# MarcKloter/bulletproofs_gadgets

Hardware: AMD Instinct MI355X
Metric: R1CS constraints/sec (prove), 2^20-constraint MiMC-Merkle, 1/2/4/8 GPU (higher is better)
Workload: dtype u32

## Files before the change

bulletproofs_gadgets_amd/csrc/engine.hip:

```cpp
#include <hip/hip_runtime.h>
#include <algorithm>
#include <array>
#include <chrono>
#include <cerrno>
#include <cstdio>
#include <cstdlib>
#include <cstring>
#include <atomic>
#include <condition_variable>
#include <deque>
#include <functional>
#include <map>
#include <memory>
#include <mutex>
#include <thread>
#include <sched.h>
#include <fcntl.h>
#include <sys/stat.h>
#include <unistd.h>
#include "engine.hpp"
#include "host/fe51.hpp"
#include "host/chain.hpp"
#include "hip/kernels.cuh"

// ... 6 lines not shown
#define BPG_LAUNCH_LDS(I, id, kernel, grid, block, lds, ...) do { (I).prof_begin(id); hipLaunchKernelGGL(kernel, grid, block, lds, (I).st, __VA_ARGS__); (I).prof_end(id); } while (0)

namespace {

struct DevBuf {
    void *p = nullptr; size_t cap = 0;
    void ensure(size_t bytes) {
        if (bytes <= cap) return;
        if (p) HIPCHK(hipFree(p));
        p = nullptr; cap = 0;
        HIPCHK(hipMalloc(&p, bytes)); cap = bytes;
    }
    void release() { if (p) { (void)hipFree(p); p = nullptr; cap = 0; } }
    template <class T> T *as() const { return reinterpret_cast<T *>(p); }
};
struct PinBuf {
    void *p = nullptr; size_t cap = 0;
    void ensure(size_t bytes) {
        if (bytes <= cap) return;
        if (p) HIPCHK(hipHostFree(p));
        p = nullptr; cap = 0;
        HIPCHK(hipHostMalloc(&p, bytes, hipHostMallocDefault)); cap = bytes;
    }
    void release() { if (p) { (void)hipHostFree(p); p = nullptr; cap = 0; } }
    template <class T> T *as() const { return reinterpret_cast<T *>(p); }
};

static std::mutex g_table_bytes_mutex;
static std::map<int, uint64_t> g_table_bytes;
static uint64_t table_bytes_held(int device) { std::lock_guard<std::mutex> lk(g_table_bytes_mutex); return g_table_bytes[device]; }
static void table_bytes_add(int device, int64_t delta) { std::lock_guard<std::mutex> lk(g_table_bytes_mutex); g_table_bytes[device] = (uint64_t)((int64_t)g_table_bytes[device] + delta); }
static std::atomic<int> g_proving[64];
struct ProvingGuard {
    std::atomic<int> &c;
    explicit ProvingGuard(int device) : c(g_proving[(unsigned)device & 63u]) { c.fetch_add(1, std::memory_order_relaxed); }
    ~ProvingGuard() { c.fetch_sub(1, std::memory_order_relaxed); }
};
static bool device_shared(int device) { return g_proving[(unsigned)device & 63u].load(std::memory_order_relaxed) > 1; }
struct SharedTables {
    int device = 0; uint64_t cap = 0;
    DevBuf gens;
    std::mutex m;
    std::map<uint32_t, DevBuf> wide;
    std::map<uint32_t, DevBuf> odd;
    std::map<uint64_t, uint64_t> refused;
    ~SharedTables() {
        (void)hipSetDevice(device); gens.release();
        uint64_t held = 0;
        for (auto &kv : odd) { held += kv.second.cap; kv.second.release(); }
        for (auto &kv : wide) { held += kv.second.cap; kv.second.release(); }
        table_bytes_add(device, -(int64_t)held);
    }
};
static std::mutex g_tables_mutex;
static std::map<std::pair<int, uint64_t>, std::weak_ptr<SharedTables>> g_tables;

inline uint32_t cdiv(uint64_t a, uint64_t b) { return (uint32_t)((a + b - 1) / b); }
inline double now_ms() { return std::chrono::duration<double, std::milli>(std::chrono::steady_clock::now().time_since_epoch()).count(); }

const Scalar &R1_plain() { static Scalar r = [] { Scalar s; s.w[0] = 0xd6ec31748d98951dULL; s.w[1] = 0xc6ef5bf4737dcf70ULL; s.w[2] = 0xfffffffffffffffeULL; s.w[3] = 0x0fffffffffffffffULL; return s; }(); return r; }
const Scalar &Rinv_plain() { static Scalar r = R1_plain().invert(); return r; }
scm to_scm(const Scalar &s) { Scalar m = s * R1_plain(); scm o; std::memcpy(o.v, m.w, 32); return o; }
Scalar from_scm(const scm &m) { Scalar s; std::memcpy(s.w, m.v, 32); return s * Rinv_plain(); }

int32_t naf256(const Scalar &s, int8_t d[256]) {
    uint64_t k[5] = {s.w[0], s.w[1], s.w[2], s.w[3], 0};
    std::memset(d, 0, 256);
    int32_t top = -1;
    for (int i = 0; i < 256; i++) {
        if ((k[0] | k[1] | k[2] | k[3] | k[4]) == 0) break;
        if (k[0] & 1) {
            int dig = 2 - (int)(k[0] & 3);
            d[i] = (int8_t)dig; top = i;
            if (dig == 1) k[0] -= 1;
            else { for (int j = 0; j < 5; j++) { if (++k[j] != 0) break; } }
        }
        for (int j = 0; j < 4; j++) k[j] = (k[j] >> 1) | (k[j + 1] << 63);
        k[4] >>= 1;
    }
    return top;
}

int32_t wnaf256(const Scalar &s, uint32_t w, int8_t d[256]) {
    uint64_t k[5] = {s.w[0], s.w[1], s.w[2], s.w[3], 0};
    std::memset(d, 0, 256);
    int32_t top = -1;
    const int64_t full = 1ll << w, half = 1ll << (w - 1);
    for (int i = 0; i < 256; i++) {
        if ((k[0] | k[1] | k[2] | k[3] | k[4]) == 0) break;
        if (k[0] & 1) {
            int64_t dig = (int64_t)(k[0] & (uint64_t)(full - 1));
            if (dig >= half) dig -= full;
            d[i] = (int8_t)dig; top = i;
            if (dig > 0) { k[0] -= (uint64_t)dig; }
            else { uint64_t add = (uint64_t)(-dig); for (int j = 0; j < 5; j++) { uint64_t t = k[j] + add; add = t < add ? 1 : 0; k[j] = t; if (!add) break; } }
        }
        for (int j = 0; j < 4; j++) k[j] = (k[j] >> 1) | (k[j + 1] << 63);
        k[4] >>= 1;
    }
    return top;
}

Scalar scalar_bits(const Scalar &s, uint32_t from, uint32_t count) {
    Scalar r = Scalar::zero();
    for (uint32_t k = 0; k < count && from + k < 256; k++) {
        const uint32_t b = from + k;
        if ((s.w[b >> 6] >> (b & 63)) & 1ull) r.w[k >> 6] |= 1ull << (k & 63);
    }
    return r;
}

uint32_t ceil_log2(uint64_t x) { uint32_t l = 0; while ((1ULL << l) < x) l++; return l; }

struct GensCacheHeader { char magic[8]; uint64_t version, capacity, bytes, checksum; };
static const char kGensMagic[8] = {'B', 'P', 'G', 'G', 'E', 'N', 'S', '1'};
uint64_t gens_checksum(const uint8_t *p, size_t n) {
    uint64_t h[4] = {0x9e3779b97f4a7c15ull, 0xc2b2ae3d27d4eb4full, 0x165667b19e3779f9ull, 0x27d4eb2f165667c5ull};
    size_t i = 0;
    for (; i + 32 <= n; i += 32) for (int k = 0; k < 4; k++) { uint64_t w; std::memcpy(&w, p + i + 8 * k, 8); h[k] = (h[k] ^ w) * 0x100000001b3ull; h[k] = (h[k] << 29) | (h[k] >> 35); }
    for (; i < n; i++) h[0] = (h[0] ^ p[i]) * 0x100000001b3ull;
    return h[0] ^ (h[1] * 3) ^ (h[2] * 5) ^ (h[3] * 7) ^ (uint64_t)n;
}
bool gens_cache_trusted(const std::string &dir, const std::string &file) {
    struct stat st;
    if (::stat(dir.c_str(), &st) != 0 || !S_ISDIR(st.st_mode) || st.st_uid != ::geteuid() || (st.st_mode & (S_IWGRP | S_IWOTH))) return false;
    if (::lstat(file.c_str(), &st) != 0) return true;
    return S_ISREG(st.st_mode) && st.st_uid == ::geteuid() && !(st.st_mode & (S_IWGRP | S_IWOTH));
}
std::string gens_cache_path(const std::string &dir, uint64_t cap) {
    if (dir.empty()) return std::string();
    return dir + "/gens_" + std::to_string(cap) + ".bpg";
}

}

struct DeviceCircuit {
    uint64_t n = 0, m = 0, q = 0, ncols = 0, nnz = 0;
    bool has_witness = false;
    uint64_t const_begin = 0;
    DevBuf aL, aR, aO, col_ptr, ent_row, ent_coef, coef;
    struct MergeSet { uint32_t groups = 0, skipped = 0; DevBuf skipA, skipB, sc, pts; };
    bool merge_tried = false;
    MergeSet mI, mO;
    bool is_template = false;
    DevBuf wit_stream, wit_segs, wit_v;
    std::vector<uint32_t> wit_level_ptr;
    uint64_t n_params = 0, param_first = 0;
};

#define BPG_KERNELS(X) X(k_gens_derive) X(k_normalize_niels) X(k_compress_niels) X(k_pedersen) X(k_sc_from_bytes) \
    X(k_sc_from_wide) X(k_blind_poison) X(k_exp_table) X(k_reduce_partials) X(k_flatten) X(k_flatten_const) X(k_poly_t) X(k_poly_eval) X(k_ipa_prep) \
    X(k_ipa_fold_scalars) X(k_fold_points) X(k_fold_points_reg) X(k_fold_points_split) X(k_fold_points_wnaf) X(k_fold_points_quad) X(k_fold_points_quadw) X(k_fold_points_regw) X(k_odd_start) X(k_odd_start_ext) X(k_dbl_times) X(k_odd_step) X(k_msm_digits) X(k_msm_scatter1) X(k_msm_sort2) X(k_scan_blocksums) \
    X(k_scan_apply) X(k_bucket_chunks) X(k_bucket_combine) X(k_bucket_combine_heavy) X(k_bucket_reduce) X(k_window_sums) X(k_window_sums_quad) X(k_decompress) X(k_ipa_s) X(k_verify_scalars) X(k_verify_scalars_acc) X(k_bench_fe_mul) \
    X(k_tt_bases) X(k_tt_multiples) X(k_tt_bases8) X(k_tt_multiples8) X(k_tt_round8) X(k_tt_factors) X(k_tt_advance) X(k_tt_round) X(k_tt_finish) X(k_blind_expand) X(k_tt_commit3) X(k_tt_commit3_finish) X(k_csc_count) X(k_csc_fill) X(k_csc_colptr) X(k_merge_insert) X(k_merge_plan) X(k_merge_groups) X(k_merge_members) X(k_merge_sum) \
    X(k_bt_commit3) X(k_bt_commit3_finish) X(k_bt_compress) X(k_bt_exp) X(k_bt_poly_t) X(k_bt_poly_eval) X(k_bt_factors) X(k_bt_advance) X(k_bt_round) \
    X(k_bt_finish) X(k_bt_fold_scalars) X(k_witness_eval)
enum KernelId {
#define X(n) KID_##n,
    BPG_KERNELS(X)
#undef X
    KID_COUNT
};
static const char *const kKernelNames[KID_COUNT] = {
#define X(n) #n,
    BPG_KERNELS(X)
#undef X
};

struct Engine::Impl {
    hipStream_t st = nullptr;
    int prof_mode = 0;
    struct ProfRec { int id; hipEvent_t a, b; };
    std::vector<ProfRec> prof_open;
    std::vector<hipEvent_t> prof_pool;
    double prof_ms[KID_COUNT] = {0};
    std::vector<float> prof_wit_ms;
    uint64_t prof_count[KID_COUNT] = {0};
    double prof_alg_bytes[KID_COUNT] = {0}, prof_act_bytes[KID_COUNT] = {0}, prof_fm[KID_COUNT] = {0};
    bool prof_on(int id) const { return prof_mode == 2 || (prof_mode == 1 && (id == KID_k_fold_points || id == KID_k_fold_points_reg || id == KID_k_fold_points_split || id == KID_k_fold_points_wnaf || id == KID_k_fold_points_quad || id == KID_k_fold_points_quadw || id == KID_k_fold_points_regw || id == KID_k_bucket_chunks)); }
    hipEvent_t prof_event() { if (!prof_pool.empty()) { hipEvent_t e = prof_pool.back(); prof_pool.pop_back(); return e; } hipEvent_t e; HIPCHK(hipEventCreate(&e)); return e; }
    void prof_begin(int id) { if (!prof_on(id)) return; ProfRec r{id, prof_event(), prof_event()}; HIPCHK(hipEventRecord(r.a, st)); prof_open.push_back(r); }
    void prof_end(int id) { if (!prof_on(id)) return; HIPCHK(hipEventRecord(prof_open.back().b, st)); }
    void prof_note(int id, double alg_bytes, double act_bytes, double fm) { if (!prof_on(id)) return; prof_alg_bytes[id] += alg_bytes; prof_act_bytes[id] += act_bytes; prof_fm[id] += fm; }
    void prof_collect() {
        if (prof_open.empty()) return;
        HIPCHK(hipStreamSynchronize(st));
        for (ProfRec &r : prof_open) { float ms = 0; HIPCHK(hipEventElapsedTime(&ms, r.a, r.b)); prof_ms[r.id] += ms; prof_count[r.id]++; if (r.id == KID_k_witness_eval && prof_wit_ms.size() < 1024) prof_wit_ms.push_back(ms); prof_pool.push_back(r.a); prof_pool.push_back(r.b); }
        prof_open.clear();
    }
    void prof_reset() { prof_collect(); for (int i = 0; i < KID_COUNT; i++) { prof_ms[i] = 0; prof_count[i] = 0; prof_alg_bytes[i] = prof_act_bytes[i] = prof_fm[i] = 0; } prof_wit_ms.clear(); }
    std::shared_ptr<SharedTables> shared;
    DevBuf gens;
    DevBuf bases, scratch_ext, comp, small_in, small_sc;
    DevBuf arena;
    uint8_t *arena_at(size_t off) const { return arena.as<uint8_t>() + off; }
    bool blocking_waits = false;
    void wait_stream() {
        if (blocking_waits && !shared_now) {
            const double until = now_ms() + 3.0;
            do {
                const hipError_t e = hipStreamQuery(st);
                if (e == hipSuccess) return;
                if (e != hipErrorNotReady) HIPCHK(e);
                for (int k = 0; k < 64; k++) __builtin_ia32_pause();
            } while (now_ms() < until);
        }
        HIPCHK(hipStreamSynchronize(st));
    }
    static size_t al256(size_t x) { return (x + 255) & ~(size_t)255; }
    DevBuf counts, starts, cursor, blocksum, buckets, partial, msm_result, open_keys, medium, wsums, wq_stage, wq_tickets, tile_hist, heavy, plain, starts1;
    uint32_t sweep_blocks_resident = 1024;
    uint32_t msm_cmax = 15;
    uint32_t msm_cmax_shared = 16;
    uint32_t rseg = 8;
    uint32_t lgch = 0;
    bool gens_share = true;
    uint32_t profile = 1;
    bool shared_now = false;
    uint32_t msm_cmin = 2;
    uint32_t wit_waves = 1024;
    uint32_t merge_equal = 1;
    uint32_t merged_last = 0, merged_skipped_last = 0;
    uint32_t msm_skipped_terms = 0;
    uint32_t msm_alg_discount = 0;
    void merge_witness(DeviceCircuit *c, const ge_niels *Gtab, const ge_niels *Htab);
    void merge_build(DeviceCircuit::MergeSet &M, const scm *A, const ge_niels *PA, uint32_t nA, const scm *B, const ge_niels *PB, uint32_t nB);
    double merge_ms_last = 0;
    DevBuf sLR, yinvpow, lv, rv, red_partial, red_out, raw_rng, extras;
    DevBuf stale_flag;
    DevBuf ipa_s, ipa_tabA, ipa_tabB, naf, qsteps, vfy_in, vfy_pts, vfy_ok, vfy_sc, vfy_ch;
    DevBuf vfy_small;
    DevBuf tt_bases, tt_table, tt_f, tt_c, tt_partial, grp_c, ped_table, s_parts;
    uint32_t tt_orig_M0 = 0; const void *tt_orig_gens = nullptr;
    ge_pniels *tt_table_p = nullptr;
    void tt_build(const ge_niels *G, const ge_niels *H, const ge_niels *B, uint32_t M0, bool original) {
        const uint32_t npts = 2 * M0 + 1;
        if (original && tt_orig_M0 == M0 && tt_orig_gens == gens.p) { tt_table_p = tt_table.as<ge_pniels>(); return; }
        const size_t bb = al256((size_t)npts * TT_WINDOWS * sizeof(ge_ext)), tb = (size_t)npts * TT_WINDOWS * TT_MULTS * sizeof(ge_pniels);
        ge_ext *basesp;
        if (original) {
            tt_orig_M0 = 0;
            tt_bases.ensure(bb); tt_table.ensure(tb);
            basesp = tt_bases.as<ge_ext>(); tt_table_p = tt_table.as<ge_pniels>();
        } else {
            arena.ensure(bb + tb);
            basesp = reinterpret_cast<ge_ext *>(arena_at(0)); tt_table_p = reinterpret_cast<ge_pniels *>(arena_at(bb));
        }
        tt_partial.ensure((size_t)3 * cdiv((uint64_t)M0 * 16, 256) * sizeof(ge_ext));
        BPG_LAUNCH((*this), k_tt_bases, dim3(cdiv(npts, 64)), dim3(256), G, H, B, basesp, M0);
        BPG_LAUNCH((*this), k_tt_multiples, dim3(cdiv((uint64_t)npts * TT_WINDOWS, 256)), dim3(256), basesp, tt_table_p, npts * TT_WINDOWS);
        if (original) { tt_orig_M0 = M0; tt_orig_gens = gens.p; }
    }
    uint64_t table_budget = 4ull << 30;
    uint64_t tt_wide_budget = 0;
    std::string gens_cache_dir;
    bool table_reserve(uint64_t key, uint64_t bytes) const {
        std::lock_guard<std::mutex> lk(g_table_bytes_mutex);
        uint64_t &held = g_table_bytes[shared->device];
        auto it = shared->refused.find(key);
        if (it != shared->refused.end() && held >= it->second) return false;
        if (held + bytes > table_budget) return false;
        held += bytes;
        return true;
    }
    const ge_pniels *wide_ensure(uint32_t M0) {
        const uint64_t bytes = (uint64_t)2 * M0 * TT8_WINDOWS * TT8_MULTS * sizeof(ge_pniels);
        if (M0 < 64 || bytes > tt_wide_budget) return nullptr;
        std::lock_guard<std::mutex> lk(shared->m);
        auto it = shared->wide.find(M0);
        if (it != shared->wide.end()) return it->second.as<ge_pniels>();
        const uint64_t key = (1ull << 32) | M0;
        if (!table_reserve(key, bytes)) return nullptr;
        DevBuf table, bases8;
        try { table.ensure(bytes); bases8.ensure((size_t)2 * M0 * TT8_WINDOWS * sizeof(ge_ext)); }
        catch (const std::exception &) {
            (void)hipGetLastError(); table.release(); bases8.release();
            table_bytes_add(shared->device, -(int64_t)bytes); shared->refused[key] = table_bytes_held(shared->device); return nullptr;
        }
        try {
            BPG_LAUNCH((*this), k_tt_bases8, dim3(cdiv(2 * M0, 64)), dim3(256), gens.as<ge_niels>(), gens.as<ge_niels>() + gens_cap, bases8.as<ge_ext>(), M0);
            BPG_LAUNCH((*this), k_tt_multiples8, dim3(cdiv((uint64_t)2 * M0 * TT8_WINDOWS, 256)), dim3(256), bases8.as<ge_ext>(), table.as<ge_pniels>(), 2 * M0 * TT8_WINDOWS);
            HIPCHK(hipGetLastError());
            HIPCHK(hipStreamSynchronize(st));
        } catch (...) {
            (void)hipStreamSynchronize(st); bases8.release(); table.release(); table_bytes_add(shared->device, -(int64_t)bytes);
            throw;
        }
        bases8.release();
        shared->wide[M0] = table;
        return table.as<ge_pniels>();
    }
    PinBuf h_naf, h_qsteps;
    DevBuf gens_odd;
    uint32_t fold_wnaf = 5;
    uint32_t fold_parts = 2;
    uint64_t fold_table_budget = 64ull << 30;
    uint32_t eff_wnaf = 0, eff_parts = 0;
    uint32_t fold_part_bits() const { return (254 + eff_parts - 1) / eff_parts; }
    bool odd_ensure() {
        eff_wnaf = fold_wnaf; eff_parts = fold_parts;
        auto table_bytes = [&](uint32_t w, uint32_t parts) { return ((uint64_t)parts * (1u << (w - 2)) - 1) * 2 * gens_cap * sizeof(ge_niels); };
        auto smaller = [&]() { if (eff_parts > 1) { eff_parts /= 2; return true; } if (eff_wnaf > 3) { eff_wnaf--; return true; } return false; };
        std::lock_guard<std::mutex> lk(shared->m);
        DevBuf odd;
        for (;;) {
            const uint32_t key = eff_wnaf | (eff_parts << 8);
            auto it = shared->odd.find(key);
            if (it != shared->odd.end()) { gens_odd = it->second; return true; }
            const uint64_t bytes = table_bytes(eff_wnaf, eff_parts);
            if (bytes <= fold_table_budget && table_reserve(key, bytes)) {
                try { odd.ensure(bytes); break; }
                catch (const std::exception &) { (void)hipGetLastError(); odd.release(); table_bytes_add(shared->device, -(int64_t)bytes); shared->refused[key] = table_bytes_held(shared->device); }
            }
            if (!smaller()) { gens_odd = DevBuf(); return false; }
        }
        const uint32_t key_built = eff_wnaf | (eff_parts << 8);
        const uint32_t NM = 1u << (eff_wnaf - 2), cnt = (uint32_t)(2 * gens_cap), L = fold_part_bits();
        DevBuf dbl, base;
        try {
        scratch_ext.ensure((size_t)cnt * sizeof(ge_ext));
        dbl.ensure((size_t)cnt * sizeof(ge_ext));
        if (eff_parts > 1) base.ensure((size_t)cnt * sizeof(ge_ext));
        const dim3 grid(cdiv(cnt, 256)), ngrid(cdiv(cdiv(cnt, NORM_K), 256));
        for (uint32_t part = 0; part < eff_parts; part++) {
            ge_niels *tab0 = odd.as<ge_niels>() + ((ptrdiff_t)part * NM - 1) * (ptrdiff_t)cnt;
            if (part == 0) BPG_LAUNCH((*this), k_odd_start, grid, dim3(256), gens.as<ge_niels>(), scratch_ext.as<ge_ext>(), dbl.as<ge_ext>(), cnt);
            else {
                BPG_LAUNCH((*this), k_dbl_times, grid, dim3(256), gens.as<ge_niels>(), base.as<ge_ext>(), cnt, L, part == 1 ? 1u : 0u);
                BPG_LAUNCH((*this), k_normalize_niels, ngrid, dim3(256), base.as<ge_ext>(), tab0, cnt);
                BPG_LAUNCH((*this), k_odd_start_ext, grid, dim3(256), base.as<ge_ext>(), scratch_ext.as<ge_ext>(), dbl.as<ge_ext>(), cnt);
            }
            for (uint32_t m = 1; m < NM; m++) {
                if (m > 1) BPG_LAUNCH((*this), k_odd_step, grid, dim3(256), scratch_ext.as<ge_ext>(), dbl.as<ge_ext>(), cnt);
                BPG_LAUNCH((*this), k_normalize_niels, ngrid, dim3(256), scratch_ext.as<ge_ext>(), tab0 + (size_t)m * cnt, cnt);
            }
        }
        HIPCHK(hipGetLastError());
        HIPCHK(hipStreamSynchronize(st));
        } catch (...) {
            (void)hipStreamSynchronize(st); dbl.release(); base.release();
            const uint64_t held = odd.cap; odd.release(); table_bytes_add(shared->device, -(int64_t)held);
            throw;
        }
        dbl.release(); base.release();
        shared->odd[key_built] = odd;
        gens_odd = odd;
        return true;
    }
    uint32_t fold_split_max = 65536;
    uint32_t fold_adapt = 1;
    bool shared_variants() const { return fold_adapt == 2 || (fold_adapt == 1 && device_shared(shared->device)); }
    bool fold_quad = true;
    bool fold_quad_w = true;
    bool fold_reg_w = true;
    bool window_quad = true;
    uint32_t window_quad_blocks = 288;
    uint32_t fold_group = 3;
    uint32_t tt_lg = 12;
    uint32_t tt_orig_lg = 14;
    uint32_t batch_wave_mb = 512;
    DevBuf bt_dev; PinBuf bt_pin;
    PinBuf h_raw, h_small;
    using BlindStream = bpg::BlindStream;
    using ChainWorker = bpg::ChainWorker;
    std::shared_ptr<ChainWorker> chain;
    uint32_t pool_streams = 0;
    uint32_t chain_workers = 1;
    uint32_t chain_lanes = 1;
    std::deque<std::shared_ptr<BlindStream>> blinds;
    std::vector<std::shared_ptr<BlindStream>> slab_owner;
    std::vector<PinBuf> h_blind;
    struct SlabDev { DevBuf d; hipStream_t copy_st = nullptr; std::vector<hipEvent_t> ev; };
    std::vector<std::unique_ptr<SlabDev>> slab_dev;
    int last_chain_cpu = -1;
    int test_fail_upload = 0;
    static void blind_stop(const std::shared_ptr<BlindStream> &b) {
        b->stop.store(true, std::memory_order_relaxed);
    }
    void blind_retire(const std::shared_ptr<BlindStream> &b) {
        blind_stop(b);
        if (chain) {
            std::unique_lock<std::mutex> lk(chain->mu);
            for (auto it = chain->pending.begin(); it != chain->pending.end(); ++it) if (it->get() == b.get()) { chain->pending.erase(it); b->finished.store(true); break; }
        }
        while (!b->finished.load(std::memory_order_acquire)) std::this_thread::yield();
        const int c = b->cpu.load(std::memory_order_relaxed); if (c >= 0) last_chain_cpu = c;
    }
    void blind_cancel() {
        while (!blinds.empty()) { blind_retire(blinds.front()); blinds.pop_front(); }
    }
    void chain_shutdown() {
        blind_cancel();
        if (!chain) return;
        if (!chain->pool) chain->stop();
        chain.reset(); pool_streams = 0;
    }
    uint64_t gens_cap = 0;
    bool gens_load_cached(const std::string &path, uint64_t cap, DevBuf &out);
    void adopt(const std::shared_ptr<SharedTables> &sp) { shared = sp; gens = sp->gens; gens_cap = sp->cap; gens_odd = DevBuf(); }
    void gens_store_cached(const std::string &path, uint64_t cap);

// ... 5 lines not shown
        MsmPlan P;
        uint32_t nkeys = 0, CH = 0, nchunks = 0, live = 0;
        bool shared = false, per_bucket = false, quad = false;
        uint32_t window_blocks = 0, window_threads = 0;
    } msm_last;
    DevBuf test_skip;
    std::vector<h51::pt> msm_points(const MsmTicket &t) const {
        std::vector<h51::pt> out(t.nmsm);
        const uint32_t *w = reinterpret_cast<const uint32_t *>(h_wsums.as<uint8_t>() + (size_t)t.slot * WS_SLOT_BYTES);
        for (uint32_t m = 0; m < t.nmsm; m++) out[m] = h51::pt_horner(w + (size_t)m * t.W * 32, t.W);
        return out;
    }
    PinBuf stage; hipEvent_t stage_ev[2] = {nullptr, nullptr};
    void h2d(void *dst, const void *src, size_t bytes) {
        const size_t SLOT = 8u << 20;
        stage.ensure(2 * SLOT);
        for (int k = 0; k < 2; k++) if (!stage_ev[k]) HIPCHK(hipEventCreateWithFlags(&stage_ev[k], hipEventDisableTiming));
        const uint8_t *s8 = static_cast<const uint8_t *>(src); uint8_t *d8 = static_cast<uint8_t *>(dst);
        int slot = 0;
        for (size_t off = 0; off < bytes; off += SLOT, slot ^= 1) {
            const size_t len = std::min(SLOT, bytes - off);
            HIPCHK(hipEventSynchronize(stage_ev[slot]));
            std::memcpy(stage.as<uint8_t>() + (size_t)slot * SLOT, s8 + off, len);
            HIPCHK(hipMemcpyAsync(d8 + off, stage.as<uint8_t>() + (size_t)slot * SLOT, len, hipMemcpyHostToDevice, st));
            HIPCHK(hipEventRecord(stage_ev[slot], st));
        }
    }
    void inner_product(Transcript &T, std::vector<uint8_t> &proof, uint64_t n, uint64_t N, const Scalar &yinv, const Scalar &u_ch, const Scalar &w,
                       const ge_niels *Gtab, const ge_niels *Htab, const ge_niels *Bn, ProveTimings *tm, double &t0);
};

namespace {
bool env_present(const char *name) { const char *e = std::getenv(name); return e && *e; }
long env_int_strict(const char *name, long lo, long hi) {
    const char *e = std::getenv(name);
    char *end = nullptr; errno = 0;
    const long v = std::strtol(e, &end, 10);
    if (errno || end == e || *end != '\0' || v < lo || v > hi)
        throw std::invalid_argument(std::string(name) + "=" + e + ": expected an integer in [" + std::to_string(lo) + ", " + std::to_string(hi) + "]");
    return v;
}
double env_double_strict(const char *name, double lo, double hi) {
    const char *e = std::getenv(name);
    char *end = nullptr; errno = 0;
    const double v = std::strtod(e, &end);
    if (errno || end == e || *end != '\0' || !(v >= lo) || !(v <= hi))
        throw std::invalid_argument(std::string(name) + "=" + e + ": expected a number in [" + std::to_string(lo) + ", " + std::to_string(hi) + "]");
    return v;
}
template <class T> void env_set(const char *name, long lo, long hi, T &out) { if (env_present(name)) out = (T)env_int_strict(name, lo, hi); }
}

Engine::Engine(int device, const EngineConfig &cfg) : device_(device) {
    if (cfg.profile > 2) throw std::invalid_argument("bpg_config.profile: 0 (default), 1 (one-shot) or 2 (serving)");
    if (cfg.table_budget_gb < 0 || cfg.table_budget_gb > 4096) throw std::invalid_argument("bpg_config.table_budget_gb: 0 (default) .. 4096");
    if (cfg.chain_workers > 64) throw std::invalid_argument("bpg_config.chain_workers: 0 (default), 1..64");
    if (cfg.chain_lanes > 8) throw std::invalid_argument("bpg_config.chain_lanes: 0 (default), 1..8");
    if (cfg.blocking_sync < -1 || cfg.blocking_sync > 2) throw std::invalid_argument("bpg_config.blocking_sync: -1 (environment, else spin), 0 (spin), 1 (blocking)");
    std::unique_ptr<Impl> K(new Impl());
    int blocking = cfg.blocking_sync == 2 ? 0 : cfg.blocking_sync;
    if (blocking < 0 && env_present("BPG_SYNC_BLOCKING")) blocking = env_int_strict("BPG_SYNC_BLOCKING", 0, 1) ? 1 : 0;
    uint32_t profile = cfg.profile;
    if (profile == 0) { if (const char *e = std::getenv("BPG_PROFILE")) profile = (!std::strcmp(e, "serving") || !std::strcmp(e, "2")) ? 2u : 1u; else profile = 1u; }
    if (profile == 2) { K->fold_wnaf = 8; K->fold_parts = 4; K->tt_wide_budget = 24ull << 30; K->table_budget = 96ull << 30; }
    else { K->fold_wnaf = 5; K->fold_parts = 2; K->tt_wide_budget = 0; K->table_budget = 4ull << 30; }
    K->profile = profile;
    {
        double gb = cfg.table_budget_gb;
        if (!(gb > 0) && env_present("BPG_TABLE_GB")) gb = env_double_strict("BPG_TABLE_GB", 0.0, 4096.0);
        if (gb > 0) K->table_budget = (uint64_t)(gb * (double)(1ull << 30));
    }
    K->chain_workers = cfg.chain_workers ? cfg.chain_workers : 1u; if (!cfg.chain_workers) env_set("BPG_CHAIN_WORKERS", 1, 64, K->chain_workers);
    K->chain_lanes = cfg.chain_lanes ? cfg.chain_lanes : 1u; if (!cfg.chain_lanes) env_set("BPG_CHAIN_LANES", 1, 8, K->chain_lanes);
    K->gens_cache_dir = cfg.gens_cache_dir;
    if (K->gens_cache_dir.empty()) { if (const char *e = std::getenv("BPG_GENS_CACHE_DIR")) K->gens_cache_dir = e; }
    if (env_present("BPG_MSM_CMAX")) K->msm_cmax = K->msm_cmax_shared = (uint32_t)env_int_strict("BPG_MSM_CMAX", 4, 16);
    env_set("BPG_MSM_CMIN", 2, 16, K->msm_cmin);
    env_set("BPG_MERGE", 0, 2, K->merge_equal);
    bool resident_set = false;
    if (env_present("BPG_SWEEP_RESIDENT")) { K->sweep_blocks_resident = (uint32_t)env_int_strict("BPG_SWEEP_RESIDENT", 64, 65536); resident_set = true; }
    if (env_present("BPG_RSEG")) {
        const long v = env_int_strict("BPG_RSEG", 1, 1024);
        if (v & (v - 1)) throw std::invalid_argument("BPG_RSEG: the segment length of the bucket reduction is a power of two in [1, 1024]");
        K->rseg = (uint32_t)v;
    }
    env_set("BPG_LGCH", 2, 10, K->lgch);
    env_set("BPG_FOLD_SPLIT", 0, 1 << 24, K->fold_split_max);
    if (env_present("BPG_FOLD_QUAD")) K->fold_quad = env_int_strict("BPG_FOLD_QUAD", 0, 1) != 0;
    if (env_present("BPG_FOLD_QUAD_W")) K->fold_quad_w = env_int_strict("BPG_FOLD_QUAD_W", 0, 1) != 0;
    if (env_present("BPG_FOLD_REG_W")) K->fold_reg_w = env_int_strict("BPG_FOLD_REG_W", 0, 1) != 0;
    if (env_present("BPG_WINDOW_QUAD")) K->window_quad = env_int_strict("BPG_WINDOW_QUAD", 0, 1) != 0;
    env_set("BPG_WINDOW_QUAD_BLOCKS", 1, 65536, K->window_quad_blocks);
    env_set("BPG_FOLD_ADAPT", 0, 2, K->fold_adapt);
    env_set("BPG_FOLD_GROUP", 1, 5, K->fold_group);
    if (env_present("BPG_TT_WIDE_GB")) K->tt_wide_budget = (uint64_t)(env_double_strict("BPG_TT_WIDE_GB", 0.0, 4096.0) * (double)(1ull << 30));
    if (env_present("BPG_FOLD_TABLE_GB")) K->fold_table_budget = (uint64_t)(env_double_strict("BPG_FOLD_TABLE_GB", 0.0, 4096.0) * (double)(1ull << 30));
    if (env_present("BPG_FOLD_PARTS")) { const long v = env_int_strict("BPG_FOLD_PARTS", 1, 8); if (v & (v - 1)) throw std::invalid_argument("BPG_FOLD_PARTS: 1, 2, 4 or 8"); K->fold_parts = (uint32_t)v; }
    if (env_present("BPG_FOLD_WNAF")) { const long v = env_int_strict("BPG_FOLD_WNAF", 0, 8); if (v == 1 || v == 2) throw std::invalid_argument("BPG_FOLD_WNAF: 0 (register kernels) or 3..8"); K->fold_wnaf = (uint32_t)v; }
    if (env_present("BPG_TT_LG")) K->tt_lg = K->tt_orig_lg = (uint32_t)env_int_strict("BPG_TT_LG", 0, 20);
    env_set("BPG_TT_ORIG_LG", 0, 20, K->tt_orig_lg);
    env_set("BPG_BATCH_WAVE_MB", 0, 1 << 20, K->batch_wave_mb);
    if (env_present("BPG_GENS_SHARE")) K->gens_share = env_int_strict("BPG_GENS_SHARE", 0, 1) != 0;

    int count = 0;
    hipError_t e = hipGetDeviceCount(&count);
    if (e != hipSuccess || count <= 0) throw DeviceError("no HIP device available: the bpg engine has no CPU path");
    if (device < 0 || device >= count) throw DeviceError("invalid device ordinal");
    HIPCHK(hipSetDevice(device));
    if (blocking == 1) { (void)hipSetDeviceFlags(hipDeviceScheduleBlockingSync); (void)hipGetLastError(); K->blocking_waits = true; }
    {
        int cus = 0;
        if (hipDeviceGetAttribute(&cus, hipDeviceAttributeMultiprocessorCount, device) == hipSuccess && cus > 0) {
            if (!resident_set) K->sweep_blocks_resident = (uint32_t)cus * 4u;
            K->wit_waves = (uint32_t)cus * 4u;
            if (!env_present("BPG_WINDOW_QUAD_BLOCKS")) K->window_quad_blocks = (uint32_t)cus + (uint32_t)cus / 8u;
        }
    }
    impl_ = K.release();
    try { init_device(); }
    catch (...) { if (impl_->st) (void)hipStreamDestroy(impl_->st); delete impl_; impl_ = nullptr; throw; }
}

void Engine::init_device() {
    HIPCHK(hipStreamCreate(&impl_->st));
    stream_ = impl_->st;
    static const uint8_t Bc[32] = {0xe2, 0xf2, 0xae, 0x0a, 0x6a, 0xbc, 0x4e, 0x71, 0xa8, 0x84, 0xa9, 0x61, 0xc5, 0x00, 0x51, 0x5f,
                                   0x58, 0xe3, 0x0b, 0x6a, 0xa5, 0x82, 0xdd, 0x8d, 0xb6, 0xa6, 0x59, 0x45, 0xe0, 0x8d, 0x2d, 0x76};
    uint8_t h[64]; sha3_512_host(h, Bc, 32);
    impl_->small_in.ensure(4096); impl_->bases.ensure(3 * sizeof(ge_niels));
    impl_->stale_flag.ensure(64); HIPCHK(hipMemsetAsync(impl_->stale_flag.p, 0, 64, impl_->st));
    HIPCHK(hipMemcpyAsync(impl_->small_in.p, h, 64, hipMemcpyHostToDevice, impl_->st));
    hipLaunchKernelGGL(k_init_bases, dim3(1), dim3(64), 0, impl_->st, impl_->small_in.as<uint32_t>(), impl_->bases.as<ge_niels>());
    HIPCHK(hipGetLastError());
    impl_->tt_bases.ensure((size_t)3 * TT_WINDOWS * sizeof(ge_ext));
    impl_->ped_table.ensure((size_t)3 * TT_WINDOWS * TT_MULTS * sizeof(ge_pniels));
    hipLaunchKernelGGL(k_tt_bases, dim3(1), dim3(256), 0, impl_->st, impl_->bases.as<ge_niels>(), impl_->bases.as<ge_niels>() + 1, impl_->bases.as<ge_niels>(),
                       impl_->tt_bases.as<ge_ext>(), 1u);
    hipLaunchKernelGGL(k_tt_multiples, dim3(cdiv(3 * TT_WINDOWS, 256)), dim3(256), 0, impl_->st, impl_->tt_bases.as<ge_ext>(), impl_->ped_table.as<ge_pniels>(),
                       (uint32_t)(3 * TT_WINDOWS));
    HIPCHK(hipGetLastError());
    HIPCHK(hipStreamSynchronize(impl_->st));
}

Engine::~Engine() {
    if (!impl_) return;
    impl_->chain_shutdown();
    (void)hipSetDevice(device_);
    (void)hipStreamSynchronize(impl_->st);
    for (auto &sd : impl_->slab_dev) if (sd->copy_st) (void)hipStreamSynchronize(sd->copy_st);
    DevBuf *bufs[] = {&impl_->bases, &impl_->scratch_ext, &impl_->comp, &impl_->small_in, &impl_->small_sc, &impl_->counts,
                      &impl_->starts, &impl_->cursor, &impl_->blocksum, &impl_->arena, &impl_->buckets, &impl_->partial, &impl_->msm_result,
                      &impl_->sLR, &impl_->yinvpow, &impl_->lv, &impl_->rv, &impl_->red_partial,
                      &impl_->red_out, &impl_->raw_rng, &impl_->extras, &impl_->ipa_s, &impl_->ipa_tabA, &impl_->ipa_tabB, &impl_->naf, &impl_->qsteps, &impl_->wsums, &impl_->wq_stage, &impl_->wq_tickets, &impl_->vfy_in, &impl_->vfy_pts, &impl_->vfy_ok, &impl_->vfy_sc, &impl_->vfy_ch, &impl_->vfy_small,
                      &impl_->stale_flag, &impl_->tile_hist, &impl_->heavy, &impl_->plain, &impl_->open_keys, &impl_->medium, &impl_->tt_bases, &impl_->tt_table, &impl_->tt_f, &impl_->tt_c, &impl_->tt_partial, &impl_->grp_c, &impl_->ped_table, &impl_->s_parts, &impl_->starts1};
    for (DevBuf *b : bufs) b->release();
    impl_->shared.reset();
    impl_->h_raw.release(); impl_->h_small.release(); impl_->h_naf.release(); impl_->h_qsteps.release(); impl_->stage.release(); for (PinBuf &b : impl_->h_blind) b.release();
    for (auto &sd : impl_->slab_dev) {
        if (sd->copy_st) { (void)hipStreamSynchronize(sd->copy_st); (void)hipStreamDestroy(sd->copy_st); }
        for (hipEvent_t e : sd->ev) (void)hipEventDestroy(e);
        sd->d.release();
    }
    for (int k = 0; k < 2; k++) if (impl_->stage_ev[k]) (void)hipEventDestroy(impl_->stage_ev[k]);
    (void)hipStreamDestroy(impl_->st);
    delete impl_;
}

int Engine::device_count() { int n = 0; if (hipGetDeviceCount(&n) != hipSuccess) { (void)hipGetLastError(); return 0; } return n; }
void Engine::profile_set(int mode) { HIPCHK(hipSetDevice(device_)); impl_->prof_reset(); impl_->prof_mode = mode; }
std::string Engine::profile_report() {
    HIPCHK(hipSetDevice(device_));
    impl_->prof_collect();
    char sch[896];
    std::snprintf(sch, sizeof sch, "{\"_schedule\": {\"profile\": %u, \"tt_lg\": %u, \"tt_orig_lg\": %u, \"fold_group\": %u, \"fold_wnaf\": %u, \"fold_parts\": %u, "
                  "\"eff_wnaf\": %u, \"eff_parts\": %u, \"fold_adapt\": %u, \"fold_split_max\": %u, \"fold_quad\": %u, \"msm_cmax\": %u, \"msm_cmax_shared\": %u, \"msm_cmin\": %u, "
                  "\"rseg\": %u, \"lgch\": %u, \"sweep_blocks_resident\": %u, \"shared_variants_last\": %u, \"merge_equal\": %u, \"merged_last\": %u, \"merged_skipped_last\": %u, \"merge_ms_last\": %.3f, \"table_budget\": %llu, \"table_bytes\": %llu}",
                  impl_->profile, impl_->tt_lg, impl_->tt_orig_lg, impl_->fold_group, impl_->fold_wnaf, impl_->fold_parts, impl_->eff_wnaf, impl_->eff_parts,
                  impl_->fold_adapt, impl_->fold_split_max, (unsigned)impl_->fold_quad, impl_->msm_cmax, impl_->msm_cmax_shared, impl_->msm_cmin, impl_->rseg, impl_->lgch,
                  impl_->sweep_blocks_resident, (unsigned)impl_->shared_now, (unsigned)impl_->merge_equal, impl_->merged_last, impl_->merged_skipped_last, impl_->merge_ms_last, (unsigned long long)impl_->table_budget, (unsigned long long)table_bytes_held(device_));
    std::string out = sch;
    if (!impl_->prof_wit_ms.empty()) {
        out += ", \"_witness_launch_ms\": [";
        for (size_t i = 0; i < impl_->prof_wit_ms.size(); i++) { char b[32]; std::snprintf(b, sizeof b, "%s%.4f", i ? "," : "", impl_->prof_wit_ms[i]); out += b; }
        out += "]";
    }
    bool first = false;
    for (int i = 0; i < KID_COUNT; i++) {
        if (!impl_->prof_count[i]) continue;
        char buf[512];
        std::snprintf(buf, sizeof buf, "%s\"%s\": {\"count\": %llu, \"total_ms\": %.6f, \"alg_bytes\": %.0f, \"device_bytes\": %.0f, \"field_mults\": %.0f}",
                      first ? "" : ", ", kKernelNames[i], (unsigned long long)impl_->prof_count[i], impl_->prof_ms[i], impl_->prof_alg_bytes[i],
                      impl_->prof_act_bytes[i], impl_->prof_fm[i]);
        out += buf; first = false;
    }
    return out + "}";
}
double Engine::bench_fe_mul(uint32_t iters) {
    HIPCHK(hipSetDevice(device_));
    Impl &I = *impl_;
    const uint32_t blocks = 256 * 16, threads = 256;
    I.small_sc.ensure((size_t)blocks * threads * sizeof(fe));
    hipEvent_t a, b; HIPCHK(hipEventCreate(&a)); HIPCHK(hipEventCreate(&b));
    hipLaunchKernelGGL(k_bench_fe_mul, dim3(blocks), dim3(threads), 0, I.st, I.small_sc.as<fe>(), 8u);
    HIPCHK(hipEventRecord(a, I.st));
    hipLaunchKernelGGL(k_bench_fe_mul, dim3(blocks), dim3(threads), 0, I.st, I.small_sc.as<fe>(), iters);
    HIPCHK(hipEventRecord(b, I.st));
    HIPCHK(hipGetLastError());
    HIPCHK(hipEventSynchronize(b));
    float ms = 0; HIPCHK(hipEventElapsedTime(&ms, a, b));
    (void)hipEventDestroy(a); (void)hipEventDestroy(b);
    return (double)blocks * threads * iters * 4.0 / (ms * 1e-3);
}

void Engine::test_fe_ops(int op, size_t n, const uint8_t *a, const uint8_t *b, uint8_t *out) {
    if (!n) return;
    HIPCHK(hipSetDevice(device_));
    Impl &I = *impl_;
    I.small_sc.ensure(2 * n * 32); I.comp.ensure(n * 32);
    HIPCHK(hipMemcpyAsync(I.small_sc.p, a, n * 32, hipMemcpyHostToDevice, I.st));
    HIPCHK(hipMemcpyAsync(I.small_sc.as<uint8_t>() + n * 32, b, n * 32, hipMemcpyHostToDevice, I.st));
    hipLaunchKernelGGL(k_test_fe, dim3(cdiv(n, 64)), dim3(64), 0, I.st, I.small_sc.as<uint32_t>(), I.small_sc.as<uint32_t>() + 8 * n, I.comp.as<uint8_t>(), (uint32_t)n, (uint32_t)op);
    HIPCHK(hipGetLastError());
    HIPCHK(hipMemcpyAsync(out, I.comp.p, n * 32, hipMemcpyDeviceToHost, I.st));
    HIPCHK(hipStreamSynchronize(I.st));
}

void Engine::synchronize() { HIPCHK(hipSetDevice(device_)); HIPCHK(hipStreamSynchronize(impl_->st)); }

void Engine::gens_ensure(uint64_t capacity) {
    if (capacity == 0 || (capacity & (capacity - 1))) throw std::invalid_argument("generator capacity must be a power of two");
    if (capacity > (1ULL << 24)) throw std::invalid_argument("generator capacity above 2^24 is not supported");
    if (capacity <= gens_cap_) return;
    HIPCHK(hipSetDevice(device_));
    Impl &I = *impl_;
    const uint64_t cap = capacity;
    std::lock_guard<std::mutex> tables_lock(g_tables_mutex);
    const bool share = I.gens_share;
    if (share) {
        auto it = g_tables.find({device_, cap});
        if (it != g_tables.end()) {
            if (std::shared_ptr<SharedTables> sp = it->second.lock()) { I.adopt(sp); gens_cap_ = cap; return; }
            g_tables.erase(it);
        }
    }
    auto publish = [&](DevBuf fresh) {
        auto sp = std::make_shared<SharedTables>();
        sp->device = device_; sp->cap = cap; sp->gens = fresh;
        if (share) g_tables[{device_, cap}] = sp;
        I.adopt(sp); gens_cap_ = cap;
    };
    const std::string cache_file = gens_cache_path(I.gens_cache_dir, cap);
    const bool cache_ok = !cache_file.empty() && gens_cache_trusted(I.gens_cache_dir, cache_file);
    if (cache_ok) { DevBuf loaded; if (I.gens_load_cached(cache_file, cap, loaded)) { publish(loaded); return; } }
    I.h_raw.ensure(2 * cap * 64);
    {
        struct Chain { Shake256 sh; std::vector<uint8_t> bytes; bool started = false; };
        static Chain chains[2];
        static std::mutex chain_mutex;
        std::lock_guard<std::mutex> lock(chain_mutex);
        auto extend = [&](int which) {
            Chain &c = chains[which];
            if (!c.started) {
                const uint8_t label[5] = {(uint8_t)(which ? 'H' : 'G'), 0, 0, 0, 0};
                c.sh.absorb(reinterpret_cast<const uint8_t *>("GeneratorsChain"), 15);
                c.sh.absorb(label, 5);
                c.started = true;
            }
            const size_t have = c.bytes.size(), want = (size_t)cap * 64;
            if (want > have) { c.bytes.resize(want); c.sh.squeeze(c.bytes.data() + have, want - have); }
        };
        (void)keccak_impl();
        std::thread th([&] { extend(1); });
        extend(0);
        th.join();
        for (int which = 0; which < 2; which++) std::memcpy(I.h_raw.as<uint8_t>() + (size_t)which * cap * 64, chains[which].bytes.data(), (size_t)cap * 64);
    }
    I.raw_rng.ensure(2 * cap * 64);
    I.scratch_ext.ensure(2 * cap * sizeof(ge_ext));
    DevBuf fresh; fresh.ensure(2 * cap * sizeof(ge_niels));
    HIPCHK(hipMemcpyAsync(I.raw_rng.p, I.h_raw.p, 2 * cap * 64, hipMemcpyHostToDevice, I.st));
    const uint32_t cnt = (uint32_t)(2 * cap);
    BPG_LAUNCH(I, k_gens_derive, dim3(cdiv(cnt, 256)), dim3(256), I.raw_rng.as<uint32_t>(), I.scratch_ext.as<ge_ext>(), cnt);
    BPG_LAUNCH(I, k_normalize_niels, dim3(cdiv(cdiv(cnt, NORM_K), 256)), dim3(256), I.scratch_ext.as<ge_ext>(), fresh.as<ge_niels>(), cnt);
    HIPCHK(hipGetLastError());
    HIPCHK(hipStreamSynchronize(I.st));
    publish(fresh);
    I.raw_rng.release(); I.scratch_ext.release(); I.h_raw.release();
    if (cache_ok) I.gens_store_cached(cache_file, cap);
}

bool Engine::Impl::gens_load_cached(const std::string &path, uint64_t cap, DevBuf &out) {
    const int fd = ::open(path.c_str(), O_RDONLY | O_NOFOLLOW | O_CLOEXEC);
    FILE *f = fd >= 0 ? ::fdopen(fd, "rb") : nullptr;
    if (!f) { if (fd >= 0) ::close(fd); return false; }
    const size_t bytes = (size_t)2 * cap * sizeof(ge_niels);
    GensCacheHeader hd;
    bool ok = std::fread(&hd, sizeof hd, 1, f) == 1 && std::memcmp(hd.magic, kGensMagic, 8) == 0 && hd.version == 2 && hd.capacity == cap && hd.bytes == bytes;
    PinBuf host;
    if (ok) { host.ensure(bytes); ok = std::fread(host.p, 1, bytes, f) == bytes && std::fgetc(f) == EOF; }
    std::fclose(f);
    if (ok) ok = gens_checksum(host.as<uint8_t>(), bytes) == hd.checksum;
    if (!ok) { host.release(); return false; }
    DevBuf fresh; fresh.ensure(bytes);
    HIPCHK(hipMemcpyAsync(fresh.p, host.p, bytes, hipMemcpyHostToDevice, st));
    const uint32_t SAMPLE = (uint32_t)std::min<uint64_t>(64, cap);
    uint8_t raw[2 * 64 * 64];
    for (int which = 0; which < 2; which++) {
// ... 409 lines not shown

void Engine::free_circuit(DeviceCircuit *c) {
    if (!c) return;
    (void)hipSetDevice(device_);
    DevBuf *b[] = {&c->wit_stream, &c->wit_segs, &c->wit_v, &c->aL, &c->aR, &c->aO, &c->col_ptr, &c->ent_row, &c->ent_coef, &c->coef, &c->mI.skipA, &c->mI.skipB, &c->mI.sc, &c->mI.pts, &c->mO.skipA, &c->mO.skipB, &c->mO.sc, &c->mO.pts};
    for (DevBuf *x : b) x->release();
    delete c;
}

TemplatePlan Engine::plan_template(const FlatView &c, const WitnessProgramView &p) {
    check_instance(c);
    check_witness_program(c, p);
    TemplatePlan T;
    T.schedule = build_witness_schedule(c.n, c.m, p);
    T.packed = pack_witness_program(c, p, T.schedule);
    T.slotted = with_parameter_slots(c, p);
    T.n_params = p.n_params; T.param_first = c.ncoef;
    return T;
}
void Engine::template_eval_host(const FlatView &c, const WitnessProgramView &p, const uint8_t *v, uint8_t *aL_out, uint8_t *aR_out, uint8_t *aO_out) {
    const TemplatePlan T = plan_template(c, p);
    const PackedWitnessProgram &P = T.packed;
    auto load = [](const uint8_t *b, size_t count) {
        std::vector<scm> out(count ? count : 1);
        for (size_t i = 0; i < count; i++) { uint32_t w[8]; std::memcpy(w, b + 32 * i, 32); out[i] = sc_from_words(w); }
        return out;
    };
    const std::vector<scm> coef = load(c.coef, c.ncoef), vv = load(v, c.m);
    std::vector<scm> aL(c.n), aR(c.n), aO(c.n);
    for (const WitnessSegment &s : P.segs) witness_eval_segment(s.first, s.count, P.stream.data() + s.stream, coef.data(), vv.data(), aL.data(), aR.data(), aO.data());
    for (size_t i = 0; i < c.n; i++) {
        uint32_t w[8];
        sc_to_words(w, aL[i]); std::memcpy(aL_out + 32 * i, w, 32);
        sc_to_words(w, aR[i]); std::memcpy(aR_out + 32 * i, w, 32);
        sc_to_words(w, aO[i]); std::memcpy(aO_out + 32 * i, w, 32);
    }
}

DeviceCircuit *Engine::upload_template(const FlatView &c, const TemplatePlan &T) {
    const PackedWitnessProgram &P = T.packed;
    FlatView f(T.slotted); f.aL = c.aL; f.aR = c.aR; f.aO = c.aO;
    DeviceCircuit *d = upload(f);
    try {
        Impl &I = *impl_;
        d->is_template = true; d->n_params = T.n_params; d->param_first = T.param_first;
        d->wit_level_ptr = T.schedule.level_ptr;
        d->wit_stream.ensure(P.stream.size() * 4); d->wit_segs.ensure(P.segs.size() * sizeof(WitnessSegment)); d->wit_v.ensure((c.m ? c.m : 1) * sizeof(scm));
        I.h2d(d->wit_stream.p, P.stream.data(), P.stream.size() * 4);
        I.h2d(d->wit_segs.p, P.segs.data(), P.segs.size() * sizeof(WitnessSegment));
        HIPCHK(hipStreamSynchronize(I.st));
    } catch (...) { free_circuit(d); throw; }
    return d;
}

void Engine::assign(DeviceCircuit *d, const uint8_t *v, const uint8_t *param_values) {
    HIPCHK(hipSetDevice(device_));
    Impl &I = *impl_;
    if (!d || !d->is_template) throw std::invalid_argument("assign: the circuit is not a template (bpg_r1cs_upload_template)");
    d->has_witness = false;
    d->merge_tried = false; d->mI.groups = d->mI.skipped = 0; d->mO.groups = d->mO.skipped = 0;
    const uint64_t cnt[2] = {d->m, d->n_params};
    const uint8_t *src[2] = {v, param_values};
    scm *dst[2] = {d->wit_v.as<scm>(), d->coef.as<scm>() + d->param_first};
    I.small_sc.ensure((std::max(cnt[0], cnt[1]) + 1) * 32);
    for (int k = 0; k < 2; k++) {
        if (!cnt[k]) continue;
        I.h2d(I.small_sc.p, src[k], cnt[k] * 32);
        BPG_LAUNCH(I, k_sc_from_bytes, dim3(cdiv(cnt[k], 256)), dim3(256), I.small_sc.as<uint32_t>(), dst[k], (uint32_t)cnt[k]);
        HIPCHK(hipGetLastError());
        HIPCHK(hipStreamSynchronize(I.st));
    }
    for (size_t l = 0; l + 1 < d->wit_level_ptr.size(); l++) {
        const uint32_t s0 = d->wit_level_ptr[l], ns = d->wit_level_ptr[l + 1] - s0;
        const uint32_t lanes = std::min(64u, std::max(1u, cdiv(ns, I.wit_waves)));
        BPG_LAUNCH(I, k_witness_eval, dim3(cdiv(ns, lanes)), dim3(lanes), d->wit_segs.as<uint4>() + s0, ns, d->wit_stream.as<uint32_t>(), d->coef.as<scm>(),
                   d->wit_v.as<scm>(), d->aL.as<scm>(), d->aR.as<scm>(), d->aO.as<scm>());
    }
    HIPCHK(hipGetLastError());
    HIPCHK(hipStreamSynchronize(I.st));
    d->has_witness = true;
}
void Engine::Impl::merge_build(DeviceCircuit::MergeSet &M, const scm *A, const ge_niels *PA, uint32_t nA, const scm *B, const ge_niels *PB, uint32_t nB) {
    const uint32_t nterms = nA + nB;
    M.groups = 0; M.skipped = 0;
    if (nterms < 2) return;
    MergeTerms T; T.A = A; T.B = B; T.PA = PA; T.PB = PB; T.nA = nA; T.nterms = nterms;
    const uint32_t lgslots = ceil_log2((uint64_t)2 * nterms), slots = 1u << lgslots;
    const uint32_t nblk = cdiv(slots, SCAN_CHUNK);
    const size_t words = (size_t)7 * slots + 2 * (size_t)nterms + (size_t)nterms / 2 + 8;
    arena.ensure(words * 4); blocksum.ensure((size_t)(nblk + 1) * 4);
    uint32_t *rep = arena.as<uint32_t>(), *count = rep + slots, *msize = count + slots, *gcount = msize + slots, *moff = gcount + slots, *goff = moff + slots + 1,
             *fill = goff + slots + 1, *slot_of = fill + slots, *members = slot_of + nterms, *gslot = members + nterms;
    const uint32_t wA = (nA + 31) / 32, wB = (nB + 31) / 32;
    M.skipA.ensure((size_t)std::max(wA, 1u) * 4); M.skipB.ensure((size_t)std::max(wB, 1u) * 4);
    HIPCHK(hipMemsetAsync(rep, 0xff, (size_t)slots * 4, st));
    HIPCHK(hipMemsetAsync(count, 0, (size_t)slots * 4, st));
    HIPCHK(hipMemsetAsync(M.skipA.p, 0, (size_t)std::max(wA, 1u) * 4, st)); HIPCHK(hipMemsetAsync(M.skipB.p, 0, (size_t)std::max(wB, 1u) * 4, st));
    BPG_LAUNCH((*this), k_merge_insert, dim3(cdiv(nterms, 256)), dim3(256), T, rep, count, slot_of, lgslots);
    BPG_LAUNCH((*this), k_merge_plan, dim3(cdiv(slots, 256)), dim3(256), count, msize, gcount, slots);
    auto scan = [&](uint32_t *in, uint32_t *out) {
        BPG_LAUNCH((*this), k_scan_blocksums, dim3(nblk), dim3(256), in, slots, blocksum.as<uint32_t>());
        BPG_LAUNCH((*this), k_scan_apply, dim3(nblk), dim3(256), in, slots, blocksum.as<uint32_t>(), out, fill);
    };
    scan(msize, moff); scan(gcount, goff);
    HIPCHK(hipGetLastError());
    uint32_t tot[2] = {0, 0};
    HIPCHK(hipMemcpyAsync(&tot[0], moff + slots, 4, hipMemcpyDeviceToHost, st));
    HIPCHK(hipMemcpyAsync(&tot[1], goff + slots, 4, hipMemcpyDeviceToHost, st));
    HIPCHK(hipStreamSynchronize(st));
    const uint32_t skipped = tot[0], groups = tot[1];
    if (groups == 0 || skipped > nterms || groups > nterms / 2) return;
    HIPCHK(hipMemsetAsync(fill, 0, (size_t)slots * 4, st));
    M.sc.ensure((size_t)groups * sizeof(scm)); M.pts.ensure((size_t)groups * sizeof(ge_niels));
    scratch_ext.ensure((size_t)groups * sizeof(ge_ext));
    BPG_LAUNCH((*this), k_merge_groups, dim3(cdiv(slots, 256)), dim3(256), count, goff, gslot, slots);
    BPG_LAUNCH((*this), k_merge_members, dim3(cdiv(nterms, 256)), dim3(256), T, slot_of, count, moff, fill, members, M.skipA.as<uint32_t>(), M.skipB.as<uint32_t>());
    BPG_LAUNCH((*this), k_merge_sum, dim3(cdiv(groups, 64)), dim3(64), T, count, moff, goff, gslot, members, groups, scratch_ext.as<ge_ext>(), M.sc.as<scm>());
    BPG_LAUNCH((*this), k_normalize_niels, dim3(cdiv(cdiv(groups, NORM_K), 256)), dim3(256), scratch_ext.as<ge_ext>(), M.pts.as<ge_niels>(), groups);
    HIPCHK(hipGetLastError());
    if (merge_equal != 2) HIPCHK(hipStreamSynchronize(st));
    M.groups = groups; M.skipped = skipped;
}
void Engine::Impl::merge_witness(DeviceCircuit *c, const ge_niels *Gtab, const ge_niels *Htab) {
    if (c->merge_tried) return;
    c->merge_tried = true;
    const uint32_t n = (uint32_t)c->n;
    if (!merge_equal || n < 2) return;
    const double t0 = now_ms();
    merge_build(c->mI, c->aL.as<scm>(), Gtab, n, c->aR.as<scm>(), Htab, n);
    merge_build(c->mO, c->aO.as<scm>(), Gtab, n, nullptr, nullptr, 0);
    merge_ms_last = now_ms() - t0;
}

void Engine::Impl::inner_product(Transcript &T, std::vector<uint8_t> &proof, uint64_t n, uint64_t N, const Scalar &yinv, const Scalar &u_ch,
                                 const Scalar &w, const ge_niels *Gtab, const ge_niels *Htab, const ge_niels *Bn, ProveTimings *tm, double &t0) {
    Impl &I = *this;
    const uint32_t lgN = ceil_log2(N);
    auto lap = [&](double *slot) { if (tm) { I.wait_stream(); double t1 = now_ms(); *slot += t1 - t0; t0 = t1; } };
    T.innerproduct_domain_sep(N);
    std::vector<Scalar> yinv_pow2(lgN + 1);
    yinv_pow2[0] = yinv; for (uint32_t k = 1; k <= lgN; k++) yinv_pow2[k] = yinv_pow2[k - 1] * yinv_pow2[k - 1];
    scm *a = I.lv.as<scm>(), *b = I.rv.as<scm>();
    if (lgN) {
        const uint64_t half = N / 2;
        I.ipa_s.ensure(4 * half * sizeof(scm));
        I.ipa_tabA.ensure(2 * half * sizeof(ge_niels)); I.ipa_tabB.ensure((half > 1 ? half : 2) * sizeof(ge_niels));
        I.naf.ensure(4096);
    }
    Scalar Gamma = Scalar::one(), Eta = Scalar::one();
    const ge_niels *Gst = Gtab, *Hst = Htab;
    const scm w_m = to_scm(w), uch_m = to_scm(u_ch);
    uint64_t mcur = N;
    const uint32_t quad_sums = I.shared_now ? 0u : 1u;
    bool tt_on = false; uint32_t tt_j = 0, tt_lgM0 = 0, tt_cur = 0; Scalar tt_u, tt_uinv; const ge_pniels *tt_wide = nullptr;
    const uint32_t GRP_STRIDE = 64;
    uint32_t g_j = 0, g_r = 1, g_cur = 0, g_index = 0; uint64_t g_M = N; bool g_first = true; std::vector<Scalar> g_us;
    for (uint32_t round = 0; round < lgN; round++) {
        const uint64_t h = mcur / 2;
        const bool first = round == 0;
        if (!tt_on && ((I.tt_lg > 0 && mcur <= (1ull << I.tt_lg)) || (first && I.tt_orig_lg > 0 && mcur <= (1ull << I.tt_orig_lg)))) {
            tt_on = true; tt_lgM0 = ceil_log2(mcur); tt_j = 0; tt_cur = 0;
            const uint32_t M0 = (uint32_t)mcur;
            I.tt_f.ensure((size_t)2 * M0 * sizeof(scm)); I.tt_c.ensure((size_t)4 * M0 * sizeof(scm));
            I.tt_build(Gst, Hst, Bn, M0, Gst == Gtab && Hst == Htab);
            tt_wide = (Gst == Gtab && Hst == Htab && Gtab == I.gens.as<ge_niels>()) ? I.wide_ensure(M0) : nullptr;
            BPG_LAUNCH(I, k_tt_factors, dim3(cdiv(M0, 256)), dim3(256), I.yinvpow.as<scm>(), uch_m, (uint32_t)first, (uint32_t)n, M0, to_scm(Gamma), to_scm(Eta),
                       I.tt_f.as<scm>(), I.tt_f.as<scm>() + M0, I.tt_c.as<scm>());
        }
        if (tt_on) {
            const uint32_t M0 = 1u << tt_lgM0;
            scm *c0 = I.tt_c.as<scm>() + (size_t)tt_cur * 2 * M0, *c1 = I.tt_c.as<scm>() + (size_t)(tt_cur ^ 1u) * 2 * M0;
            if (tt_j > 0) {
                BPG_LAUNCH(I, k_tt_advance, dim3(cdiv(std::max<uint64_t>(mcur, 1ull << (tt_j - 1)), 256)), dim3(256), a, b, to_scm(tt_u), to_scm(tt_uinv), (uint32_t)mcur,
                           c0, c1, 1u << (tt_j - 1), M0);
                tt_cur ^= 1u; std::swap(c0, c1);
            }
            const uint32_t nblk = cdiv((uint64_t)M0 * 8, 256);
            if (tt_wide) BPG_LAUNCH(I, k_tt_round8, dim3(nblk, 2), dim3(256), tt_wide, a, b, I.tt_f.as<scm>(), I.tt_f.as<scm>() + M0, c0, tt_lgM0, tt_j, I.tt_partial.as<ge_ext>(), quad_sums);
            else BPG_LAUNCH(I, k_tt_round, dim3(nblk, 2), dim3(256), I.tt_table_p, a, b, I.tt_f.as<scm>(), I.tt_f.as<scm>() + M0, c0, tt_lgM0, tt_j,
                       I.tt_partial.as<ge_ext>(), quad_sums);
            BPG_LAUNCH(I, k_tt_finish, dim3(2), dim3(256), I.tt_partial.as<ge_ext>(), nblk, a, b, (uint32_t)h, w_m,
                       I.tt_table_p + (size_t)2 * M0 * TT_WINDOWS * TT_MULTS, I.msm_result.as<ge_ext>(), quad_sums);
            HIPCHK(hipGetLastError());
            uint8_t lr[64];
            uint32_t *hp = reinterpret_cast<uint32_t *>(I.h_small.as<uint8_t>() + 16384);
            HIPCHK(hipMemcpyAsync(hp, I.msm_result.p, 2 * sizeof(ge_ext), hipMemcpyDeviceToHost, st));
            I.wait_stream();
            h51::pt_compress(lr, h51::pt_from_device(hp)); h51::pt_compress(lr + 32, h51::pt_from_device(hp + 32));
            lap(tm ? &tm->ipa_msm : nullptr);
            T.append_point("L", lr); T.append_point("R", lr + 32);
            proof.insert(proof.end(), lr, lr + 64);
            tt_u = T.challenge_scalar("u"); tt_uinv = tt_u.invert();
            tt_j++;
            mcur = h;
            if (round + 1 == lgN) {
                BPG_LAUNCH(I, k_ipa_fold_scalars, dim3(cdiv(h, 256)), dim3(256), a, b, to_scm(tt_u), to_scm(tt_uinv), (uint32_t)h);
                HIPCHK(hipGetLastError());
            }
            continue;
        }
        if (g_j == 0) {
            g_M = mcur; g_first = first;
            uint32_t left = ceil_log2(mcur);
            if (I.tt_lg > 0 && left > I.tt_lg) left -= I.tt_lg;
            g_r = std::min<uint32_t>(I.fold_group, left);
            g_us.clear();
            I.grp_c.ensure(4 * GRP_STRIDE * sizeof(scm));
            g_cur = 0;
            hipLaunchKernelGGL(k_set2, dim3(1), dim3(64), 0, st, I.grp_c.as<scm>(), (uint32_t)GRP_STRIDE, to_scm(Gamma), to_scm(Eta));
        }
        scm *c0 = I.grp_c.as<scm>() + (size_t)g_cur * 2 * GRP_STRIDE;
        const uint64_t cnt = g_M / 2;
        scm *sLG = I.ipa_s.as<scm>(), *sLH = sLG + cnt, *sRG = sLH + cnt, *sRH = sRG + cnt;
        const uint32_t blocks = std::min<uint32_t>(cdiv(cnt, 256), 1024);
        const uint32_t lgh = ceil_log2(h);
        I.red_partial.ensure((size_t)blocks * 2 * sizeof(scm) + 4096);
        BPG_LAUNCH(I, k_ipa_prep, dim3(blocks), dim3(256), a, b, I.yinvpow.as<scm>(), c0, c0 + GRP_STRIDE, uch_m,
                           (uint32_t)g_first, (uint32_t)n, lgh, g_j, sLG, sLH, sRG, sRH, I.red_partial.as<scm>());
        BPG_LAUNCH_ID(I, KID_k_reduce_partials, k_reduce_partials_scaled, dim3(2), dim3(256), I.red_partial.as<scm>(), blocks, 2u, I.extras.as<scm>() + 3, w_m);
        Impl::MsmTicket tk;
        {
            MsmSegs S = seg_new();
            const uint32_t lgblk = g_j ? lgh : 31u;
            seg_push(S, sLG, Gst + h, (uint32_t)cnt, 0, lgblk);
            seg_push(S, sLH, Hst, (uint32_t)cnt, 0, lgblk);
            seg_push(S, I.extras.as<scm>() + 3, Bn, 1, 0);
            seg_push(S, sRG, Gst, (uint32_t)cnt, 1, lgblk);
            seg_push(S, sRH, Hst + h, (uint32_t)cnt, 1, lgblk);
            seg_push(S, I.extras.as<scm>() + 4, Bn, 1, 1);
            tk = I.msm(S, 2);
        }
        uint8_t lr[64];
        I.wait_stream();
        { const std::vector<h51::pt> LR = I.msm_points(tk); h51::pt_compress(lr, LR[0]); h51::pt_compress(lr + 32, LR[1]); }
        lap(tm ? &tm->ipa_msm : nullptr);
        T.append_point("L", lr); T.append_point("R", lr + 32);
        proof.insert(proof.end(), lr, lr + 64);
        const Scalar u = T.challenge_scalar("u"), uinv = u.invert();
        g_us.push_back(u);
        {
            scm *c1 = I.grp_c.as<scm>() + (size_t)(g_cur ^ 1u) * 2 * GRP_STRIDE;
            BPG_LAUNCH(I, k_tt_advance, dim3(cdiv(std::max<uint64_t>(h, 1ull << g_j), 256)), dim3(256), a, b, to_scm(u), to_scm(uinv), (uint32_t)h,
                       c0, c1, 1u << g_j, (uint32_t)GRP_STRIDE);
            g_cur ^= 1u;
        }
        g_j++;
        if (g_j == g_r) {
            const uint32_t Mr = (uint32_t)(g_M >> g_r), nterms = (1u << g_r) - 1u;
            std::vector<Scalar> fG(g_r), fH(g_r);
            for (uint32_t k = 1; k <= g_r; k++) {
                const Scalar &uk = g_us[k - 1]; const Scalar ukinv = uk.invert();
                fG[k - 1] = uk * uk; fH[k - 1] = ukinv * ukinv * yinv_pow2[ceil_log2(g_M >> k)];
            }
            ge_niels *dst = (g_index & 1) ? I.ipa_tabB.as<ge_niels>() : I.ipa_tabA.as<ge_niels>();
            I.scratch_ext.ensure((size_t)2 * Mr * sizeof(ge_ext));
            const bool use_wnaf = I.fold_wnaf >= 3 && Gst == Gtab && Hst == Htab && Gtab == I.gens.as<ge_niels>() && 2 * Mr > I.fold_split_max
                                  && I.odd_ensure();
            if (use_wnaf) {
                const uint32_t parts = I.eff_parts, L = I.fold_part_bits(), nq = nterms * parts;
                const size_t dbytes = (size_t)4 * nq * 256;
                I.h_naf.ensure(dbytes); I.naf.ensure(dbytes);
                int8_t *hd = I.h_naf.as<int8_t>();
                std::memset(hd, 0, dbytes);
                int32_t top = -1; double adds_fm = 0;
                for (uint32_t q = 0; q < nterms; q++) {
                    const uint32_t t = q + 1;
                    Scalar sg = Scalar::one(), sh = Scalar::one();
                    for (uint32_t k = 1; k <= g_r; k++) if ((t >> (g_r - k)) & 1u) { sg = sg * fG[k - 1]; sh = sh * fH[k - 1]; }
                    const Scalar cls_s[4] = {sg, sg * u_ch, sh, sh * u_ch};
                    const uint64_t lo = (uint64_t)t * Mr, nB = !g_first ? 0 : (lo >= n ? Mr : (lo + Mr > n ? lo + Mr - n : 0));
                    for (int cls = 0; cls < 4; cls++) {
                        if ((cls & 1) && !g_first) continue;
                        for (uint32_t part = 0; part < parts; part++) {
                            int8_t *d = hd + ((size_t)cls * nq + (size_t)part * nterms + q) * 256;
                            const int32_t tp = wnaf256(scalar_bits(cls_s[cls], part * L, L), I.eff_wnaf, d);
                            if (tp > top) top = tp;
                            int adds = 0; for (int k = 0; k < 256; k++) adds += d[k] != 0;
                            adds_fm += 7.0 * adds * ((cls & 1) ? (double)nB : (double)(Mr - nB));
                        }
                    }
                }
                HIPCHK(hipMemcpyAsync(I.naf.p, hd, dbytes, hipMemcpyHostToDevice, st));
                FoldWnaf fw; fw.Mr = Mr; fw.nterms = nterms; fw.first_group = g_first; fw.n = (uint32_t)n; fw.cap = (uint32_t)gens_cap; fw.top = top;
                fw.parts = parts; fw.NM = 1u << (I.eff_wnaf - 2);
                BPG_LAUNCH(I, k_fold_points_wnaf, dim3(cdiv(2 * Mr, 256)), dim3(256), I.gens.as<ge_niels>(), I.gens_odd.as<ge_niels>(), I.scratch_ext.as<ge_ext>(),
                           I.naf.as<uint32_t>(), fw);
                I.prof_note(KID_k_fold_points_wnaf, 32.0 * (2.0 * g_M + 2.0 * Mr), 96.0 * (2.0 * Mr + adds_fm / 7.0) + 128.0 * 2 * Mr, 2.0 * Mr * (8.0 * (top + 1) + 7.0) + adds_fm);
            } else {
            I.h_naf.ensure((size_t)4 * nterms * 16 * 4); I.naf.ensure((size_t)4 * nterms * 16 * 4);
            uint32_t *hn = I.h_naf.as<uint32_t>();
            std::memset(hn, 0, (size_t)4 * nterms * 16 * 4);
            int32_t top = -1; double adds_fm = 0;
            for (uint32_t q = 0; q < nterms; q++) {
                const uint32_t t = q + 1;
                Scalar sg = Scalar::one(), sh = Scalar::one();
                for (uint32_t k = 1; k <= g_r; k++) if ((t >> (g_r - k)) & 1u) { sg = sg * fG[k - 1]; sh = sh * fH[k - 1]; }
                const Scalar cls_s[4] = {sg, sg * u_ch, sh, sh * u_ch};
                const uint64_t lo = (uint64_t)t * Mr, nB = !g_first ? 0 : (lo >= n ? Mr : (lo + Mr > n ? lo + Mr - n : 0));
                for (int cls = 0; cls < 4; cls++) {
                    if ((cls & 1) && !g_first) continue;
                    int8_t dg[256]; const int32_t tp = naf256(cls_s[cls], dg);
                    if (tp > top) top = tp;
                    uint32_t *d = hn + ((size_t)cls * nterms + q) * 16; int adds = 0;
                    for (int k = 0; k < 256; k++) { if (dg[k]) { d[k >> 5] |= 1u << (k & 31); adds++; } if (dg[k] < 0) d[8 + (k >> 5)] |= 1u << (k & 31); }
                    adds_fm += 7.0 * adds * ((cls & 1) ? (double)nB : (double)(Mr - nB));
                }
            }
            HIPCHK(hipMemcpyAsync(I.naf.p, hn, (size_t)4 * nterms * 16 * 4, hipMemcpyHostToDevice, st));
            FoldGroup fg; fg.Mr = Mr; fg.nterms = nterms; fg.first_group = g_first; fg.n = (uint32_t)n; fg.top = top;
            int fold_kid = KID_k_fold_points;
            {
                const dim3 grid(cdiv(2 * Mr, 256)), block(256);
                ge_ext *fo = I.scratch_ext.as<ge_ext>(); const uint32_t *nf = I.naf.as<uint32_t>();
                const bool regs = nterms == 1 || nterms == 3 || nterms == 7 || nterms == 15;
                const uint32_t split_max = (regs && I.shared_now) ? 0 : I.fold_split_max;
                FoldQuadW fq; std::memset(&fq, 0, sizeof fq); fq.Mr = Mr; fq.nterms = nterms;
                auto make_steps = [&]() {
                    I.h_qsteps.ensure((size_t)2 * QW_MAXSTEPS * 4); I.qsteps.ensure((size_t)2 * QW_MAXSTEPS * 4);
                    uint32_t *hs = I.h_qsteps.as<uint32_t>();
                    double adds_w = 0, dbls_w = 0;
                    for (uint32_t cls = 0; cls < 2; cls++) {
                        std::vector<std::array<int8_t, 256>> dg(nterms);
                        int32_t tp = -1;
                        for (uint32_t q = 0; q < nterms; q++) {
                            const uint32_t t = q + 1;
                            Scalar sc1 = Scalar::one();
                            for (uint32_t k = 1; k <= g_r; k++) if ((t >> (g_r - k)) & 1u) sc1 = sc1 * (cls ? fH[k - 1] : fG[k - 1]);
                            tp = std::max(tp, wnaf256(sc1, 4, dg[q].data()));
                        }
                        uint32_t ns = 0, pending = 0;
                        for (int32_t k = tp; k >= 0; k--) {
                            if (ns) pending++;
                            for (uint32_t q = 0; q < nterms; q++) {
                                const int d = dg[q][k];
                                if (!d) continue;
                                if (ns >= QW_MAXSTEPS || pending > 255) throw std::logic_error("fold: step list overflow");
                                const uint32_t mag = (uint32_t)(d < 0 ? -d : d);
                                hs[cls * QW_MAXSTEPS + ns++] = pending | (q << 8) | ((mag >> 1) << 11) | ((d < 0 ? 1u : 0u) << 13);
                                dbls_w += pending; pending = 0;
                            }
                        }
                        fq.nsteps[cls] = ns; fq.tail[cls] = pending; adds_w += ns; dbls_w += pending;
                    }
                    HIPCHK(hipMemcpyAsync(I.qsteps.p, hs, (size_t)2 * QW_MAXSTEPS * 4, hipMemcpyHostToDevice, st));
                    I.arena.ensure((size_t)3 * nterms * 2 * Mr * sizeof(ge_pniels));
                    adds_fm = (adds_w * 8.0 + nterms * 2.0 * (7.0 + 8.0 + 7.0 + 2 * 9.0 + 3.0)) * Mr; top = (int32_t)(dbls_w / 2.0) - 1;
                };
                if (2 * Mr <= split_max && nterms >= 1 && nterms <= 7 && I.fold_quad && I.fold_quad_w && !g_first && Mr % 64 == 0) {
                    fold_kid = KID_k_fold_points_quadw;
                    make_steps();
                    BPG_LAUNCH_ID(I, fold_kid, k_fold_points_quadw, dim3(cdiv(2 * Mr, 64)), block, Gst, Hst, fo, I.qsteps.as<uint32_t>(), reinterpret_cast<fe *>(I.arena_at(0)), fq);
                } else if (2 * Mr <= split_max && nterms >= 1 && nterms <= 7 && I.fold_quad) {
                    fold_kid = KID_k_fold_points_quad;
                    BPG_LAUNCH_ID(I, fold_kid, k_fold_points_quad, dim3(cdiv(2 * Mr, 64)), block, Gst, Hst, fo, nf, fg);
                } else if (2 * Mr <= split_max && nterms >= 3 && nterms <= 15) {
                    fold_kid = KID_k_fold_points_split;
                    BPG_LAUNCH_ID(I, fold_kid, k_fold_points_split, dim3(cdiv(2 * Mr, 64)), block, Gst, Hst, fo, nf, fg);
                } else if (2 * Mr > split_max && I.fold_reg_w && !g_first && nterms >= 1 && nterms <= 7 && Mr % 256 == 0) {
                    fold_kid = KID_k_fold_points_regw;
                    make_steps();
                    BPG_LAUNCH_ID(I, fold_kid, k_fold_points_regw, grid, block, Gst, Hst, fo, I.qsteps.as<uint32_t>(), reinterpret_cast<ge_pniels *>(I.arena_at(0)), fq);
                } else if (regs) {
                    fold_kid = KID_k_fold_points_reg;
                    if (nterms == 1) BPG_LAUNCH_ID(I, fold_kid, k_fold_points_reg<1>, grid, block, Gst, Hst, fo, nf, fg);
                    else if (nterms == 3) BPG_LAUNCH_ID(I, fold_kid, k_fold_points_reg<3>, grid, block, Gst, Hst, fo, nf, fg);
                    else if (nterms == 7) BPG_LAUNCH_ID(I, fold_kid, k_fold_points_reg<7>, grid, block, Gst, Hst, fo, nf, fg);
                    else BPG_LAUNCH_ID(I, fold_kid, k_fold_points_reg<15>, grid, block, Gst, Hst, fo, nf, fg);
                } else BPG_LAUNCH(I, k_fold_points, grid, block, Gst, Hst, fo, nf, fg);
            }
            I.prof_note(fold_kid, 32.0 * (2.0 * g_M + 2.0 * Mr), 96.0 * 2 * g_M + 128.0 * 2 * Mr,
                        2.0 * Mr * (8.0 * (top + 1) * (fold_kid == KID_k_fold_points_split ? (nterms < 4 ? nterms : 4) : 1) + 7.0) + adds_fm);
            }
            BPG_LAUNCH(I, k_normalize_niels, dim3(cdiv(cdiv(2 * Mr, NORM_K), 256)), dim3(256), I.scratch_ext.as<ge_ext>(), dst, 2 * Mr);
            HIPCHK(hipGetLastError());
            I.wait_stream();
            Gst = dst; Hst = dst + Mr;
            for (const Scalar &uk : g_us) { Gamma = uk.invert() * Gamma; Eta = uk * Eta; }
            g_j = 0; g_index++;
        }
        mcur = h;
        lap(tm ? &tm->ipa_fold : nullptr);
    }
    scm ab[2];
    HIPCHK(hipMemcpyAsync(&ab[0], a, sizeof(scm), hipMemcpyDeviceToHost, st));
    HIPCHK(hipMemcpyAsync(&ab[1], b, sizeof(scm), hipMemcpyDeviceToHost, st));
    I.wait_stream();
    { uint8_t o[64]; from_scm(ab[0]).to_bytes(o); from_scm(ab[1]).to_bytes(o + 32); proof.insert(proof.end(), o, o + 64); }
}

void Engine::blinding_begin(const Transcript &after_commitments, const std::vector<Scalar> &v_blinding, const uint8_t seed[32], uint64_t max_multipliers) {
    HIPCHK(hipSetDevice(device_));
    Impl &I = *impl_;
    if (max_multipliers == 0) { I.blind_cancel(); return; }
    if (I.chain && I.chain->pool) {
        bool gone; { std::lock_guard<std::mutex> lk(I.chain->mu); gone = I.chain->quit; }
        if (gone) { I.blind_cancel(); I.chain.reset(); I.pool_streams = 0; }
    }
    using BS = Impl::BlindStream;
    const size_t max_alive = I.pool_streams ? I.pool_streams : (size_t)I.chain_workers * I.chain_lanes + 1;
    while (I.blinds.size() >= max_alive) { I.blind_retire(I.blinds.front()); I.blinds.pop_front(); }
    auto b = std::make_shared<BS>();
    Transcript T = after_commitments;
    T.append_u64("m", v_blinding.size());
    T.export_state(b->state);
    std::memcpy(b->seed, seed, 32); b->vb = v_blinding;
    TranscriptRng rng = T.build_rng(v_blinding, seed);
    for (int k = 0; k < 3; k++) b->first[k] = rng.random_scalar();
    b->max_draws = ((2 * max_multipliers + BS::SNAP - 1) / BS::SNAP) * BS::SNAP;
    b->inject_fail = I.test_fail_upload; I.test_fail_upload = 0;
    if (I.h_blind.size() < max_alive) { I.h_blind.resize(max_alive); I.slab_owner.resize(max_alive); while (I.slab_dev.size() < max_alive) I.slab_dev.emplace_back(std::make_unique<Impl::SlabDev>()); }
    int slot = -1;
    for (size_t k = 0; k < max_alive && slot < 0; k++) {
        bool used = false;
        for (const std::shared_ptr<BS> &x : I.blinds) used |= x->slot == (int)k;
        if (!used) slot = (int)k;
    }
    if (slot < 0) throw std::logic_error("blinding_begin: no free slab");
    b->slot = slot;
    if (I.slab_owner[slot]) { I.blind_retire(I.slab_owner[slot]); I.slab_owner[slot].reset(); }
    Impl::SlabDev &sd = *I.slab_dev[slot];
    if (!sd.copy_st) HIPCHK(hipStreamCreateWithFlags(&sd.copy_st, hipStreamNonBlocking));
    HIPCHK(hipStreamSynchronize(sd.copy_st));
    I.h_blind[slot].ensure(b->max_draws * 64);
    sd.d.ensure(b->max_draws * 64);
    while (sd.ev.size() < b->max_draws / BS::UP + 1) { hipEvent_t e; HIPCHK(hipEventCreateWithFlags(&e, hipEventDisableTiming)); sd.ev.push_back(e); }
    {
        const uint32_t nblk = (uint32_t)((b->max_draws + BS::UP - 1) / BS::UP);
        if (nblk) hipLaunchKernelGGL(k_blind_poison, dim3(cdiv((uint64_t)nblk * 16, 256)), dim3(256), 0, sd.copy_st, sd.d.as<uint32_t>(), nblk, (uint32_t)BS::UP);
        HIPCHK(hipGetLastError());
    }
    b->raw = I.h_blind[slot].as<uint8_t>();
    b->device = device_; b->copy_st = sd.copy_st; b->d_raw = sd.d.as<uint8_t>(); b->ev = &sd.ev;
    b->upload = [](BlindStream &bs, uint64_t from, uint64_t to, uint64_t k) -> int {
        hipError_t e = hipSetDevice(bs.device);
        if (e == hipSuccess && bs.inject_fail != 2) e = hipMemcpyAsync(bs.d_raw + 64 * from, bs.raw + 64 * from, (to - from) * 64, hipMemcpyHostToDevice, static_cast<hipStream_t>(bs.copy_st));
        if (e == hipSuccess) e = hipEventRecord((*static_cast<std::vector<hipEvent_t> *>(bs.ev))[k], static_cast<hipStream_t>(bs.copy_st));
        return (int)e;
    };
    b->snaps.assign(b->max_draws / BS::SNAP + 1, rng);
    I.slab_owner[slot] = b;
    I.blinds.push_back(b);
    if (!I.chain) { I.chain = std::make_shared<Impl::ChainWorker>(); I.chain->lanes = I.chain_lanes; (void)keccak_impl(); }
    if (!I.chain->pool) while (I.chain->th.size() < I.chain_workers) I.chain->th.emplace_back(Impl::ChainWorker::run, I.chain.get(), I.chain->lanes);
    I.chain->push(b);
}
struct ChainPool::Impl { std::shared_ptr<Engine::Impl::ChainWorker> w; };
ChainPool::ChainPool(const std::vector<uint32_t> &lanes_per_thread) : impl_(new Impl()) {
    if (lanes_per_thread.empty() || lanes_per_thread.size() > 256) { delete impl_; throw std::invalid_argument("chain pool: 1..256 threads"); }
    for (uint32_t l : lanes_per_thread) if (l < 1 || l > 8) { delete impl_; throw std::invalid_argument("chain pool: 1..8 lanes per thread"); }
    impl_->w = std::make_shared<Engine::Impl::ChainWorker>();
    impl_->w->pool = true;
    (void)keccak_impl();
    for (uint32_t l : lanes_per_thread) { impl_->w->th.emplace_back(Engine::Impl::ChainWorker::run, impl_->w.get(), l); capacity_ += l; }
}
ChainPool::~ChainPool() { impl_->w->stop(); delete impl_; }
void Engine::attach_chain_pool(ChainPool *pool, uint32_t max_streams) {
    impl_->chain_shutdown();
    if (!pool) return;
    if (max_streams < 1 || max_streams > 64) throw std::invalid_argument("chain pool: 1..64 streams per context");
    impl_->chain = pool->impl_->w; impl_->pool_streams = max_streams;
}
void Engine::set_chain_workers(uint32_t n) {
    if (n < 1 || n > 64) throw std::invalid_argument("chain workers: 1..64");
    impl_->chain_shutdown();
    impl_->chain_workers = n;
}
void Engine::set_chain_lanes(uint32_t n) {
    if (n < 1 || n > 8) throw std::invalid_argument("chain lanes: 1..8");
    impl_->chain_shutdown();
    impl_->chain_lanes = n;
}
void Engine::blinding_cancel() { impl_->blind_cancel(); }
void Engine::test_fail_next_upload() { impl_->test_fail_upload = 1; }
void Engine::test_drop_next_upload() { impl_->test_fail_upload = 2; }
uint64_t Engine::table_bytes() const { return table_bytes_held(device_); }

int Engine::chain_cpu() const { return impl_->last_chain_cpu; }
bool Engine::last_shared_variants() const { return impl_->shared_now; }

std::vector<uint8_t> Engine::prove(DeviceCircuit *c, Transcript &T, const std::vector<Scalar> &v_blinding,
                                   const uint8_t rng_seed[32], uint32_t flags, ProveTimings *tm) {
    HIPCHK(hipSetDevice(device_));
    Impl &I = *impl_;
    hipStream_t st = I.st;
    ProvingGuard in_flight(device_);
    I.shared_now = I.shared_variants();
    if (tm) tm->shared_variants = I.shared_now ? 1u : 0u;
    const uint64_t n = c->n, m = c->m, q = c->q;
    if (v_blinding.size() != m) throw std::invalid_argument("prove: need one blinding factor per committed variable");
    if (!c->has_witness) throw R1CSException(R1CSError::MissingAssignment, "prove: the uploaded circuit carries no assignments (verifier-side instance)");
    uint64_t N = 1; while (N < n) N <<= 1;
    const uint32_t lgN = ceil_log2(N);
    if (gens_cap_ < N) throw R1CSException(R1CSError::InvalidGeneratorsLength, "generator capacity below padded circuit size");
    const bool compact = flags & 1u, no_1phase = flags & 2u;
    const double t_begin = now_ms();
    double t0 = t_begin;
    auto lap = [&](double *slot) { if (tm) { I.wait_stream(); double t1 = now_ms(); *slot += t1 - t0; t0 = t1; } };

    const ge_niels *Gtab = I.gens.as<ge_niels>(), *Htab = I.gens.as<ge_niels>() + gens_cap_;
    const ge_niels *Bn = I.bases.as<ge_niels>(), *Bbn = Bn + 1;

    T.append_u64("m", m);
    const bool expanded = (flags & 4u) != 0;
    std::shared_ptr<Impl::BlindStream> bs;
    if (!I.blinds.empty()) {
        uint8_t now[203]; T.export_state(now);
        for (const std::shared_ptr<Impl::BlindStream> &cand : I.blinds) {
            const Impl::BlindStream &b = *cand;
            bool ok = !expanded && 2 * n <= b.max_draws && std::memcmp(now, b.state, 203) == 0 && std::memcmp(rng_seed, b.seed, 32) == 0 && b.vb.size() == v_blinding.size();
            for (size_t i = 0; ok && i < b.vb.size(); i++) ok = std::memcmp(b.vb[i].as_bytes(), v_blinding[i].as_bytes(), 32) == 0;
            if (ok) { bs = cand; break; }
        }
    }
    TranscriptRng rng = T.build_rng(v_blinding, rng_seed);
    Scalar ib, ob, sb;
    if (bs) { ib = bs->first[0]; ob = bs->first[1]; sb = bs->first[2]; }
    else { ib = rng.random_scalar(); ob = rng.random_scalar(); sb = rng.random_scalar(); }

    I.extras.ensure(16 * sizeof(scm));
    I.h_small.ensure(1 << 16);
    {
        scm *hs = I.h_small.as<scm>();
        hs[0] = to_scm(ib); hs[1] = to_scm(ob); hs[2] = to_scm(sb);
        HIPCHK(hipMemcpyAsync(I.extras.p, hs, 3 * sizeof(scm), hipMemcpyHostToDevice, st));
    }
    I.msm_result.ensure(4 * sizeof(ge_ext)); I.comp.ensure(256);

    const bool tabled = I.tt_orig_lg > 0 && N <= (1ull << I.tt_orig_lg) && n > 0;
    if (tabled) I.tt_build(Gtab, Htab, Bn, (uint32_t)N, true);
    const bool chain_ready = bs && bs->produced.load(std::memory_order_acquire) >= 2 * n;
    const bool merged = expanded || tabled || n < 4096 || chain_ready;
    Impl::MsmTicket tk_aiao{0, 0, 0}, tk_s[3]; uint32_t nparts = 0;
    if (!tabled) { if (I.merge_equal == 2) c->merge_tried = false; I.merge_witness(c, Gtab, Htab); }
    I.merged_last = tabled ? 0u : c->mI.groups + c->mO.groups; I.merged_skipped_last = tabled ? 0u : c->mI.skipped + c->mO.skipped;
    auto push_AI = [&](MsmSegs &S) {
        const bool mg = c->mI.groups != 0;
        seg_push(S, c->aL.as<scm>(), Gtab, (uint32_t)n, 0, 31, mg ? c->mI.skipA.as<uint32_t>() : nullptr);
        seg_push(S, c->aR.as<scm>(), Htab, (uint32_t)n, 0, 31, mg ? c->mI.skipB.as<uint32_t>() : nullptr);
        if (mg) { seg_push(S, c->mI.sc.as<scm>(), c->mI.pts.as<ge_niels>(), c->mI.groups, 0); I.msm_alg_discount += c->mI.groups; I.msm_skipped_terms += c->mI.skipped; }
        seg_push(S, I.extras.as<scm>() + 0, Bbn, 1, 0);
    };
    auto push_AO = [&](MsmSegs &S) {
        const bool mg = c->mO.groups != 0;
        seg_push(S, c->aO.as<scm>(), Gtab, (uint32_t)n, 1, 31, mg ? c->mO.skipA.as<uint32_t>() : nullptr);
        if (mg) { seg_push(S, c->mO.sc.as<scm>(), c->mO.pts.as<ge_niels>(), c->mO.groups, 1); I.msm_alg_discount += c->mO.groups; I.msm_skipped_terms += c->mO.skipped; }
        seg_push(S, I.extras.as<scm>() + 1, Bbn, 1, 1);
    };
    if (!merged) {
        MsmSegs S = seg_new();
        push_AI(S); push_AO(S);
        tk_aiao = I.msm(S, 2);
    }
    const double t_rng0 = now_ms();
    if (!bs && !expanded) { I.h_raw.ensure((2 * n ? 2 * n : 1) * 64); I.raw_rng.ensure((2 * n ? 2 * n : 1) * 64); }
    I.sLR.ensure((2 * n ? 2 * n : 1) * sizeof(scm));
    scm *sL = I.sLR.as<scm>(), *sR = sL + n;
    struct Piece { uint64_t a, b; } pieces[3] = {{0, n}, {n, n + (n - n / 8)}, {n + (n - n / 8), 2 * n}};
    if (n < (1u << 17)) { pieces[0] = {0, 0}; pieces[1] = {0, 0}; pieces[2] = {0, 2 * n}; }
    uint32_t next_piece = 0;
    auto launch_pieces = [&](uint64_t drawn) {
        while (next_piece < 3 && pieces[next_piece].b <= drawn) {
            const Piece pc = pieces[next_piece];
            const bool last = next_piece == 2;
            next_piece++;
            if (pc.b == pc.a && !last) continue;
            MsmSegs S = seg_new();
            if (pc.a < n) seg_push(S, sL + pc.a, Gtab + pc.a, (uint32_t)(std::min<uint64_t>(pc.b, n) - pc.a), 0);
            if (pc.b > n) { const uint64_t a2 = std::max<uint64_t>(pc.a, n) - n; seg_push(S, sR + a2, Htab + a2, (uint32_t)(pc.b - n - a2), 0); }
            if (last) seg_push(S, I.extras.as<scm>() + 2, Bbn, 1, 0);
            tk_s[nparts++] = I.msm(S, 1);
        }
    };
    if (expanded) {
        uint8_t msg[80]; std::memset(msg, 0, sizeof msg);
        std::memcpy(msg, "bpg blinding v1", 15);
        rng.fill_bytes(msg + 15, 64);
        BlindHead head; std::memcpy(head.lane, msg, 80); head.lane[9] &= 0x00ffffffffffffffULL;
        if (n) BPG_LAUNCH(I, k_blind_expand, dim3(cdiv(2 * n, 256)), dim3(256), head, sL, (uint32_t)(2 * n));
    } else
    {
        uint8_t *raw = bs ? bs->raw : I.h_raw.as<uint8_t>();
        const uint64_t slab = 1u << 16;
        if (bs && chain_ready && 2 * n > 0) {
            const uint64_t nblk = (2 * n + Impl::BlindStream::UP - 1) / Impl::BlindStream::UP;
            while (bs->uploaded_blocks.load(std::memory_order_acquire) < nblk) {
                if (bs->finished.load(std::memory_order_acquire) && bs->uploaded_blocks.load(std::memory_order_acquire) < nblk) break;
                std::this_thread::sleep_for(std::chrono::microseconds(40));
            }
            if (const int uerr = bs->err.load(std::memory_order_acquire)) {
                Impl::blind_stop(bs);
                for (auto it = I.blinds.begin(); it != I.blinds.end(); ++it) if (it->get() == bs.get()) { I.blinds.erase(it); break; }
                throw DeviceError(std::string("upload of the blinding draws failed: ") + hipGetErrorString((hipError_t)uerr));
            }
            if (bs->uploaded_blocks.load(std::memory_order_acquire) < nblk) throw DeviceError("the blinding stream ended before its draws were uploaded");
            for (uint64_t k = 0; k < nblk; k++) HIPCHK(hipStreamWaitEvent(st, (*static_cast<std::vector<hipEvent_t> *>(bs->ev))[k], 0));
            BPG_LAUNCH(I, k_sc_from_wide, dim3(cdiv(2 * n, 256)), dim3(256), reinterpret_cast<const uint32_t *>(bs->d_raw), sL, (uint32_t)(2 * n), I.stale_flag.as<uint32_t>());
        } else
        {
        uint64_t conv_from = 0;
        auto convert_to = [&](uint64_t hi) {
            if (hi <= conv_from) return;
            const uint32_t *src = bs ? reinterpret_cast<const uint32_t *>(bs->d_raw) : I.raw_rng.as<uint32_t>();
            BPG_LAUNCH(I, k_sc_from_wide, dim3(cdiv(hi - conv_from, 256)), dim3(256), src + 16 * conv_from, sL + conv_from, (uint32_t)(hi - conv_from), I.stale_flag.as<uint32_t>());
            conv_from = hi;
        };
        for (uint64_t i = 0; i < 2 * n; i += slab) {
            const uint64_t cnt = std::min<uint64_t>(slab, 2 * n - i);
            if (bs) {
                const uint64_t k = i / Impl::BlindStream::UP;
                while (bs->uploaded_blocks.load(std::memory_order_acquire) <= k) std::this_thread::sleep_for(std::chrono::microseconds(40));
                if (const int uerr = bs->err.load(std::memory_order_acquire)) {
                    Impl::blind_stop(bs);
                    for (auto it = I.blinds.begin(); it != I.blinds.end(); ++it) if (it->get() == bs.get()) { I.blinds.erase(it); break; }
                    throw DeviceError(std::string("upload of the blinding draws failed: ") + hipGetErrorString((hipError_t)uerr));
                }
                HIPCHK(hipStreamWaitEvent(st, (*static_cast<std::vector<hipEvent_t> *>(bs->ev))[k], 0));
            } else {
                rng.fill_draws64(raw + 64 * i, cnt);
                HIPCHK(hipMemcpyAsync(I.raw_rng.as<uint8_t>() + 64 * i, raw + 64 * i, cnt * 64, hipMemcpyHostToDevice, st));
            }
            if (!merged && i + cnt < 2 * n && next_piece < 3 && pieces[next_piece].b <= i + cnt) { convert_to(i + cnt); launch_pieces(i + cnt); }
        }
        convert_to(2 * n);
        }
    }
    if (bs) {
        const uint64_t K = (2 * n) / Impl::BlindStream::SNAP, rem = 2 * n - K * Impl::BlindStream::SNAP;
        while (bs->produced.load(std::memory_order_acquire) < K * Impl::BlindStream::SNAP) std::this_thread::sleep_for(std::chrono::microseconds(20));
        rng = bs->snaps[K];
        if (rem) { std::vector<uint8_t> skip(rem * 64); rng.fill_draws64(skip.data(), rem); }
        Impl::blind_stop(bs);
        for (auto it = I.blinds.begin(); it != I.blinds.end(); ++it) if (it->get() == bs.get()) { I.blinds.erase(it); break; }
        { const int c = bs->cpu.load(std::memory_order_relaxed); if (c >= 0) I.last_chain_cpu = c; }
        bs.reset();
    }
    if (tm) tm->rng_host += now_ms() - t_rng0;
    lap(tm ? &tm->msm_aiao : nullptr);
    uint8_t pts[96];
    if (tabled) {
        const uint32_t M0 = (uint32_t)N, nblk = cdiv((uint64_t)M0 * 16, 256);
        BPG_LAUNCH(I, k_tt_commit3, dim3(nblk, 3), dim3(256), I.tt_table_p, c->aL.as<scm>(), c->aR.as<scm>(), c->aO.as<scm>(), sL, sR,
                   (uint32_t)n, M0, I.tt_partial.as<ge_ext>(), I.shared_now ? 0u : 1u);
        BPG_LAUNCH(I, k_tt_commit3_finish, dim3(3), dim3(256), I.tt_partial.as<ge_ext>(), nblk, I.extras.as<scm>(),
                   I.ped_table.as<ge_pniels>() + (size_t)TT_WINDOWS * TT_MULTS, I.msm_result.as<ge_ext>(), I.shared_now ? 0u : 1u);
        HIPCHK(hipGetLastError());
        uint32_t *hp = reinterpret_cast<uint32_t *>(I.h_small.as<uint8_t>() + 16384);
        HIPCHK(hipMemcpyAsync(hp, I.msm_result.p, 3 * sizeof(ge_ext), hipMemcpyDeviceToHost, st));
        I.wait_stream();
        for (int k = 0; k < 3; k++) h51::pt_compress(pts + 32 * k, h51::pt_from_device(hp + 32 * k));
    } else if (merged) {
        MsmSegs S = seg_new();
        push_AI(S); push_AO(S);
        seg_push(S, sL, Gtab, (uint32_t)n, 2);
        seg_push(S, sR, Htab, (uint32_t)n, 2);
        seg_push(S, I.extras.as<scm>() + 2, Bbn, 1, 2);
        const Impl::MsmTicket tk = I.msm(S, 3);
        I.wait_stream();
        const std::vector<h51::pt> P3 = I.msm_points(tk);
        for (int k = 0; k < 3; k++) h51::pt_compress(pts + 32 * k, P3[k]);
    } else {
        launch_pieces(2 * n);
        I.wait_stream();
        const std::vector<h51::pt> AB = I.msm_points(tk_aiao);
        h51::pt Sp = I.msm_points(tk_s[0])[0];
        for (uint32_t k = 1; k < nparts; k++) Sp = h51::pt_add(Sp, I.msm_points(tk_s[k])[0]);
        h51::pt_compress(pts, AB[0]); h51::pt_compress(pts + 32, AB[1]); h51::pt_compress(pts + 64, Sp);
    }
    lap(tm ? &tm->msm_s : nullptr);

    std::vector<uint8_t> proof;
    proof.reserve(14 * 32 + (2 * lgN + 2) * 32 + 1);
    if (compact) proof.push_back(0);
    proof.insert(proof.end(), pts, pts + 96);
    T.append_point("A_I1", pts); T.append_point("A_O1", pts + 32); T.append_point("S1", pts + 64);
    if (!no_1phase) T.r1cs_1phase_domain_sep();
    const uint8_t ident[32] = {0};
    T.append_point("A_I2", ident); T.append_point("A_O2", ident); T.append_point("S2", ident);
    if (!compact) proof.insert(proof.end(), 96, 0);

    const Scalar y = T.challenge_scalar("y"), z = T.challenge_scalar("z");
    const Scalar yinv = y.invert();

    I.yinvpow.ensure(N * sizeof(scm));
    const size_t b_w = Impl::al256((c->ncols ? c->ncols : 1) * sizeof(scm)), b_z = Impl::al256((q + 2) * sizeof(scm)), b_y = Impl::al256(N * sizeof(scm));
    I.arena.ensure(b_w + b_z + b_y);
    scm *const wAll_p = reinterpret_cast<scm *>(I.arena_at(0)), *const zpow_p = reinterpret_cast<scm *>(I.arena_at(b_w)), *const ypow_p = reinterpret_cast<scm *>(I.arena_at(b_w + b_z));
    {
        ExpTables E; std::memset(&E, 0, sizeof E);
        uint32_t k = 0, lgmax = 0;
        auto add = [&](const Scalar &base, scm *out, uint64_t count) {
            uint32_t lgT = ceil_log2(count); if (lgT > 16) lgT = 16;
            E.base[k] = to_scm(base); E.out[k] = out; E.count[k] = (uint32_t)count; E.lgT[k] = lgT; lgmax = std::max(lgmax, lgT); k++;
        };
        add(y, ypow_p, N); add(yinv, I.yinvpow.as<scm>(), N); add(z, zpow_p, q + 1);
        BPG_LAUNCH(I, k_exp_table, dim3(cdiv(1u << lgmax, 256), k), dim3(256), E);
    }
    if (c->ncols > 1)
        BPG_LAUNCH(I, k_flatten, dim3(cdiv(c->ncols - 1, 256)), dim3(256), c->col_ptr.as<uint64_t>(), c->ent_row.as<uint32_t>(),
                           c->ent_coef.as<uint32_t>(), c->coef.as<scm>(), zpow_p, wAll_p, (uint32_t)(c->ncols - 1), (uint32_t)(3 * n));
    scm *wL = wAll_p, *wR = wL + n, *wO = wR + n, *wV = wO + n;
    const uint32_t pblocks = n ? std::min<uint32_t>(cdiv(n, 256), 1024) : 1;
    I.red_partial.ensure((size_t)pblocks * 6 * sizeof(scm) + 4096); I.red_out.ensure(16 * sizeof(scm));
    BPG_LAUNCH(I, k_poly_t, dim3(pblocks), dim3(256), c->aL.as<scm>(), c->aR.as<scm>(), c->aO.as<scm>(), sL, sR, wL, wR, wO,
                       ypow_p, I.yinvpow.as<scm>(), I.red_partial.as<scm>(), (uint32_t)n);
    BPG_LAUNCH(I, k_reduce_partials, dim3(6), dim3(256), I.red_partial.as<scm>(), pblocks, 6u, I.red_out.as<scm>());
    HIPCHK(hipGetLastError());
    scm h_t[6]; std::vector<scm> h_wV(m ? m : 1);
    HIPCHK(hipMemcpyAsync(h_t, I.red_out.p, 6 * sizeof(scm), hipMemcpyDeviceToHost, st));
    if (m) HIPCHK(hipMemcpyAsync(h_wV.data(), wV, m * sizeof(scm), hipMemcpyDeviceToHost, st));
    uint32_t *h_stale = reinterpret_cast<uint32_t *>(I.h_small.as<uint8_t>() + 32768);
    HIPCHK(hipMemcpyAsync(h_stale, I.stale_flag.p, 4, hipMemcpyDeviceToHost, st));
    I.wait_stream();
    if (*h_stale) {
        HIPCHK(hipMemsetAsync(I.stale_flag.p, 0, 4, st));
        throw DeviceError("a blinding draw was read before it was uploaded (stale device slab): proof withheld");
    }
    Scalar t[7], tb[7];
    for (int k = 0; k < 6; k++) t[k + 1] = from_scm(h_t[k]);
    tb[1] = rng.random_scalar(); tb[3] = rng.random_scalar(); tb[4] = rng.random_scalar(); tb[5] = rng.random_scalar(); tb[6] = rng.random_scalar();
    {
        uint8_t vv[5 * 32], rr[5 * 32], out[5 * 32];
        const int idx[5] = {1, 3, 4, 5, 6};
        for (int k = 0; k < 5; k++) { t[idx[k]].to_bytes(vv + 32 * k); tb[idx[k]].to_bytes(rr + 32 * k); }
        pedersen_commit(5, vv, rr, out);
        static const char *labels[5] = {"T_1", "T_3", "T_4", "T_5", "T_6"};
        for (int k = 0; k < 5; k++) T.append_point(labels[k], out + 32 * k);
        proof.insert(proof.end(), out, out + 160);
    }
    const Scalar u_ch = T.challenge_scalar("u"), x = T.challenge_scalar("x");
    for (uint64_t j = 0; j < m; j++) tb[2] += from_scm(h_wV[j]) * v_blinding[j];
    Scalar tx, txb;
    for (int k = 6; k >= 1; k--) { tx = (tx + t[k]) * x; txb = (txb + tb[k]) * x; }
    const Scalar eb = x * (ib + x * (ob + x * sb));
    T.append_scalar("t_x", tx); T.append_scalar("t_x_blinding", txb); T.append_scalar("e_blinding", eb);
    { uint8_t b[96]; tx.to_bytes(b); txb.to_bytes(b + 32); eb.to_bytes(b + 64); proof.insert(proof.end(), b, b + 96); }
    const Scalar w = T.challenge_scalar("w");

    I.lv.ensure(N * sizeof(scm)); I.rv.ensure(N * sizeof(scm));
    BPG_LAUNCH(I, k_poly_eval, dim3(cdiv(N, 256)), dim3(256), c->aL.as<scm>(), c->aR.as<scm>(), c->aO.as<scm>(), sL, sR, wL, wR, wO,
                       ypow_p, I.yinvpow.as<scm>(), to_scm(x), I.lv.as<scm>(), I.rv.as<scm>(), (uint32_t)n, (uint32_t)N);
    HIPCHK(hipGetLastError());
    lap(tm ? &tm->poly : nullptr);

    I.inner_product(T, proof, n, N, yinv, u_ch, w, Gtab, Htab, Bn, tm, t0);
    if (tm) { tm->ipa = tm->ipa_msm + tm->ipa_fold; tm->total += now_ms() - t_begin; }
    return proof;
}

namespace {
uint32_t batch_host_threads() {
    cpu_set_t set; CPU_ZERO(&set);
    long n = sched_getaffinity(0, sizeof set, &set) == 0 ? CPU_COUNT(&set) : 1;
    if (FILE *f = std::fopen("/sys/fs/cgroup/cpu.max", "r")) {
        char quota[32] = {0}; long period = 0;
        if (std::fscanf(f, "%31s %ld", quota, &period) == 2 && std::strcmp(quota, "max") != 0 && period > 0) n = std::min(n, std::max(1L, (std::atol(quota) + period - 1) / period));
        std::fclose(f);
    }
    return (uint32_t)std::max(1L, std::min(n, 16L));
}
class StageThreads {
public:
    explicit StageThreads(uint32_t n) { for (uint32_t t = 1; t < n; t++) th_.emplace_back([this] { loop(); }); }
    ~StageThreads() { { std::lock_guard<std::mutex> lk(mu_); quit_ = true; } cv_.notify_all(); for (std::thread &t : th_) t.join(); }
    void run(size_t count, const std::function<void(size_t, size_t)> &fn) {
        const size_t parts = std::min<size_t>(count, 4 * (th_.size() + 1));
        if (parts <= 1 || th_.empty()) { if (count) fn(0, count); return; }
        { std::lock_guard<std::mutex> lk(mu_); fn_ = &fn; count_ = count; parts_ = parts; next_.store(0); busy_.store((int)th_.size()); gen_++; }
        cv_.notify_all();
        work();
        while (busy_.load(std::memory_order_acquire) != 0) std::this_thread::yield();
        fn_ = nullptr;
        if (err_) { std::exception_ptr e = err_; err_ = nullptr; std::rethrow_exception(e); }
    }
private:
    void work() {
        try {
            for (size_t p; (p = next_.fetch_add(1)) < parts_;) (*fn_)(count_ * p / parts_, count_ * (p + 1) / parts_);
        } catch (...) { std::lock_guard<std::mutex> lk(err_mu_); if (!err_) err_ = std::current_exception(); next_.store(parts_); }
    }
    void loop() {
        uint64_t seen = 0;
        for (;;) {
            { std::unique_lock<std::mutex> lk(mu_); cv_.wait(lk, [&] { return quit_ || gen_ != seen; }); if (quit_) return; seen = gen_; }
            work();
            busy_.fetch_sub(1, std::memory_order_release);
        }
    }
    std::vector<std::thread> th_;
    std::mutex mu_, err_mu_; std::condition_variable cv_;
    bool quit_ = false; uint64_t gen_ = 0;
    const std::function<void(size_t, size_t)> *fn_ = nullptr;
    size_t count_ = 0, parts_ = 0;
    std::atomic<size_t> next_{0}; std::atomic<int> busy_{0};
    std::exception_ptr err_;
};
void batch_invert(Scalar *x, Scalar *out, size_t lo, size_t hi) {
// ... 592 lines not shown
```

bulletproofs_gadgets_amd/csrc/hip/k_ipa.cuh:

```cuda
#pragma once

namespace bpg {

__global__ void __launch_bounds__(256) k_ipa_prep(const scm *__restrict__ a, const scm *__restrict__ b, const scm *__restrict__ yinvpow,
                                                  const scm *__restrict__ cG, const scm *__restrict__ cH, scm u_ch, uint32_t first_group, uint32_t n,
                                                  uint32_t lgh, uint32_t j,
                                                  scm *__restrict__ sLG, scm *__restrict__ sLH, scm *__restrict__ sRG, scm *__restrict__ sRH,
                                                  scm *__restrict__ partial ) {
    __shared__ scm lds[256];
    scm cL = sc_zero(), cR = sc_zero();
    const uint32_t h = 1u << lgh, count = h << j;
    for (uint32_t e = blockIdx.x * blockDim.x + threadIdx.x; e < count; e += gridDim.x * blockDim.x) {
        const uint32_t t = e >> lgh, i = e & (h - 1);
        const uint32_t plo = (t << (lgh + 1)) | i, phi = plo | h;
        const scm alo = a[i], ahi = a[h + i], blo = b[i], bhi = b[h + i];
        const scm g = cG[t], eh = cH[t];
        const bool padlo = first_group && plo >= n, padhi = first_group && phi >= n;
        scm v;
        v = sc_mont_mul(alo, g); if (padhi) v = sc_mont_mul(v, u_ch); sLG[e] = v;
        v = sc_mont_mul(sc_mont_mul(bhi, eh), yinvpow[plo]); if (padlo) v = sc_mont_mul(v, u_ch); sLH[e] = v;
        v = sc_mont_mul(ahi, g); if (padlo) v = sc_mont_mul(v, u_ch); sRG[e] = v;
        v = sc_mont_mul(sc_mont_mul(blo, eh), yinvpow[phi]); if (padhi) v = sc_mont_mul(v, u_ch); sRH[e] = v;
        if (t == 0) { cL = sc_add(cL, sc_mont_mul(alo, bhi)); cR = sc_add(cR, sc_mont_mul(ahi, blo)); }
    }
    scm r;
    r = block_sum_256(cL, lds); if (threadIdx.x == 0) partial[blockIdx.x * 2 + 0] = r;
    r = block_sum_256(cR, lds); if (threadIdx.x == 0) partial[blockIdx.x * 2 + 1] = r;
}
__global__ void k_set2(scm *__restrict__ c, uint32_t stride, scm v0, scm v1) { if (threadIdx.x == 0 && blockIdx.x == 0) { c[0] = v0; c[stride] = v1; } }

__global__ void __launch_bounds__(256) k_ipa_fold_scalars(scm *__restrict__ a, scm *__restrict__ b, scm u, scm uinv, uint32_t h) {
    uint32_t i = blockIdx.x * blockDim.x + threadIdx.x;
    if (i >= h) return;
    a[i] = sc_add(sc_mont_mul(a[i], u), sc_mont_mul(uinv, a[h + i]));
    b[i] = sc_add(sc_mont_mul(b[i], uinv), sc_mont_mul(u, b[h + i]));
}

#define TT_WINDOWS 64
#define TT_MULTS 8

struct CoopLds { uint32_t c[4][8][64]; uint32_t s[4][8][64]; };
__device__ __forceinline__ fe coop_ld(const uint32_t (&a)[8][64], uint32_t lane) { fe r;
#pragma unroll
    for (int j = 0; j < 8; j++) r.v[j] = a[j][lane];
    return r; }
__device__ __forceinline__ void coop_st(uint32_t (&a)[8][64], uint32_t lane, const fe &x) {
#pragma unroll
    for (int j = 0; j < 8; j++) a[j][lane] = x.v[j]; }
__device__ __forceinline__ void coop_dbl(CoopLds &L, uint32_t wv, uint32_t lane) {
    const fe in = (wv == 3) ? fe_add(coop_ld(L.c[0], lane), coop_ld(L.c[1], lane)) : coop_ld(L.c[wv], lane);
    const fe sq = fe_sq(in);
    __syncthreads();
    coop_st(L.s[wv], lane, sq);
    __syncthreads();
    const fe XX = coop_ld(L.s[0], lane), YY = coop_ld(L.s[1], lane);
    const fe YpX = fe_add(YY, XX), YmX = fe_sub(YY, XX);
    fe a, b;
    if (wv == 1) { a = YpX; b = YmX; }
    else {
        const fe ZZ = coop_ld(L.s[2], lane);
        const fe cT = fe_sub(fe_add(ZZ, ZZ), YmX), cX = fe_sub(coop_ld(L.s[3], lane), YpX);
        if (wv == 0) { a = cX; b = cT; }
        else if (wv == 2) { a = YmX; b = cT; }
        else { a = cX; b = YpX; }
    }
    coop_st(L.c[wv], lane, fe_mul(a, b));
    __syncthreads();
}
__global__ void __launch_bounds__(256) k_tt_bases(const ge_niels *__restrict__ G, const ge_niels *__restrict__ H, const ge_niels *__restrict__ B,
                                                  ge_ext *__restrict__ bases, uint32_t M0) {
    __shared__ CoopLds L;
    const uint32_t wv = __builtin_amdgcn_readfirstlane(threadIdx.x >> 6), lane = threadIdx.x & 63u;
    const uint32_t count = 2 * M0 + 1;
    const uint32_t p = blockIdx.x * 64 + lane;
    const bool live = p < count;
    const uint32_t q_idx = live ? p : count - 1;
    if (wv == 0) {
        const ge_niels q = q_idx < M0 ? G[q_idx] : (q_idx < 2 * M0 ? H[q_idx - M0] : B[0]);
        const ge_ext e = ge_madd(ge_identity(), q);
        coop_st(L.c[0], lane, e.X); coop_st(L.c[1], lane, e.Y); coop_st(L.c[2], lane, e.Z); coop_st(L.c[3], lane, e.T);
    }
    __syncthreads();
    fe *dst = reinterpret_cast<fe *>(bases + (size_t)q_idx * TT_WINDOWS) + wv;
    for (uint32_t w = 0; w < TT_WINDOWS; w++) {
        if (live) dst[4 * w] = coop_ld(L.c[wv], lane);
        if (w + 1 < TT_WINDOWS) { coop_dbl(L, wv, lane); coop_dbl(L, wv, lane); coop_dbl(L, wv, lane); coop_dbl(L, wv, lane); }
    }
}
__global__ void __launch_bounds__(256) k_tt_multiples(const ge_ext *__restrict__ bases, ge_pniels *__restrict__ table, uint32_t count) {
    const uint32_t i = blockIdx.x * blockDim.x + threadIdx.x;
    if (i >= count) return;
    ge_pniels *dst = table + (size_t)i * TT_MULTS;
    const ge_ext b1 = bases[i];
    const ge_pniels n1 = ge_to_pniels(b1);
    dst[0] = n1;
    const ge_ext b2 = ge_dbl(b1); dst[1] = ge_to_pniels(b2);
    const ge_ext b3 = ge_add_pniels_signed(b2, n1, 0); dst[2] = ge_to_pniels(b3);
    const ge_ext b4 = ge_dbl(b2); dst[3] = ge_to_pniels(b4);
    const ge_ext b5 = ge_add_pniels_signed(b4, n1, 0); dst[4] = ge_to_pniels(b5);
    const ge_ext b6 = ge_dbl(b3); dst[5] = ge_to_pniels(b6);
    const ge_ext b7 = ge_add_pniels_signed(b6, n1, 0); dst[6] = ge_to_pniels(b7);
    const ge_ext b8 = ge_dbl(b4); dst[7] = ge_to_pniels(b8);
}
__global__ void __launch_bounds__(256) k_tt_factors(const scm *__restrict__ yinvpow, scm u_ch, uint32_t first_round, uint32_t n, uint32_t M0,
                                                    scm Gamma0, scm Eta0, scm *__restrict__ fG, scm *__restrict__ fH, scm *__restrict__ c0) {
    const uint32_t p = blockIdx.x * blockDim.x + threadIdx.x;
    if (p == 0) { c0[0] = Gamma0; c0[M0] = Eta0; }
    if (p >= M0) return;
    const bool pad = first_round && p >= n;
    fG[p] = pad ? u_ch : SC_R1();
    fH[p] = pad ? sc_mont_mul(yinvpow[p], u_ch) : yinvpow[p];
}
__global__ void __launch_bounds__(256) k_tt_advance(scm *__restrict__ a, scm *__restrict__ b, scm u, scm uinv, uint32_t h,
                                                    const scm *__restrict__ cprev, scm *__restrict__ cnext, uint32_t cnt, uint32_t M0) {
    const uint32_t i = blockIdx.x * blockDim.x + threadIdx.x;
    if (i < h) {
        a[i] = sc_add(sc_mont_mul(a[i], u), sc_mont_mul(uinv, a[h + i]));
        b[i] = sc_add(sc_mont_mul(b[i], uinv), sc_mont_mul(u, b[h + i]));
    }
    if (i < cnt) {
        const scm g = cprev[i], e = cprev[M0 + i];
        cnext[2 * i] = sc_mont_mul(g, uinv); cnext[2 * i + 1] = sc_mont_mul(g, u);
        cnext[M0 + 2 * i] = sc_mont_mul(e, u); cnext[M0 + 2 * i + 1] = sc_mont_mul(e, uinv);
    }
}
__device__ __forceinline__ void tt_biased_words(uint32_t w[8], const scm &s) {
    sc_to_words(w, s);
    uint64_t carry = 0;
#pragma unroll
    for (int k = 0; k < 8; k++) { uint64_t t = (uint64_t)w[k] + 0x88888888ull + carry; w[k] = (uint32_t)t; carry = t >> 32; }
}
__global__ void __launch_bounds__(256) k_tt_round(const ge_pniels *__restrict__ table, const scm *__restrict__ a, const scm *__restrict__ b,
                                                  const scm *__restrict__ fG, const scm *__restrict__ fH, const scm *__restrict__ c,
                                                  uint32_t lgM0, uint32_t j, ge_ext *__restrict__ partial , uint32_t quad) {
    __shared__ ge_ext lds[256];
    const uint32_t cls = blockIdx.y, tid = blockIdx.x * blockDim.x + threadIdx.x;
    const uint32_t M0 = 1u << lgM0, e = tid >> 3, g = tid & 7u;
    ge_ext acc = ge_identity();
    if (e < M0) {
        const bool isH = e >= (M0 >> 1);
        const uint32_t e2 = isH ? e - (M0 >> 1) : e;
        const uint32_t lgh = lgM0 - j - 1, h = 1u << lgh;
        const uint32_t t = e2 >> lgh, i = e2 & (h - 1);
        const bool hi = (cls == 0) != isH;
        const uint32_t p = (t << (lgh + 1)) | (hi ? h : 0u) | i;
        const uint32_t sidx = hi ? i : (h | i);
        scm s = isH ? b[sidx] : a[sidx];
        s = sc_mont_mul(s, isH ? fH[p] : fG[p]);
        s = sc_mont_mul(s, c[(isH ? M0 : 0u) + t]);
        uint32_t w[8]; tt_biased_words(w, s);
        const ge_pniels *tbl = table + ((size_t)(isH ? M0 : 0u) + p) * (TT_WINDOWS * TT_MULTS) + (size_t)g * 8 * TT_MULTS;
        const uint32_t word = w[g];
#pragma unroll 1
        for (uint32_t k = 0; k < 8; k++) {
            const int32_t d = (int32_t)((word >> (4 * k)) & 15u) - 8;
            if (d == 0) continue;
            const uint32_t neg = d < 0, mag = neg ? (uint32_t)(-d) : (uint32_t)d;
            acc = ge_add_pniels_signed(acc, tbl[k * TT_MULTS + mag - 1], neg);
        }
    }
    ge_block_sum_store(acc, lds, quad, partial + cls * gridDim.x + blockIdx.x);
}
#define TT8_WINDOWS 32
#define TT8_MULTS 128
__global__ void __launch_bounds__(256) k_tt_bases8(const ge_niels *__restrict__ G, const ge_niels *__restrict__ H, ge_ext *__restrict__ bases, uint32_t M0) {
    __shared__ CoopLds L;
    const uint32_t wv = __builtin_amdgcn_readfirstlane(threadIdx.x >> 6), lane = threadIdx.x & 63u;
    const uint32_t count = 2 * M0;
    const uint32_t p = blockIdx.x * 64 + lane;
    const bool live = p < count;
    const uint32_t q_idx = live ? p : count - 1;
    if (wv == 0) {
        const ge_niels q = q_idx < M0 ? G[q_idx] : H[q_idx - M0];
        const ge_ext e = ge_madd(ge_identity(), q);
        coop_st(L.c[0], lane, e.X); coop_st(L.c[1], lane, e.Y); coop_st(L.c[2], lane, e.Z); coop_st(L.c[3], lane, e.T);
    }
    __syncthreads();
    fe *dst = reinterpret_cast<fe *>(bases + (size_t)q_idx * TT8_WINDOWS) + wv;
    for (uint32_t w = 0; w < TT8_WINDOWS; w++) {
        if (live) dst[4 * w] = coop_ld(L.c[wv], lane);
        if (w + 1 < TT8_WINDOWS) for (int k = 0; k < 8; k++) coop_dbl(L, wv, lane);
    }
}
__global__ void __launch_bounds__(256) k_tt_multiples8(const ge_ext *__restrict__ bases, ge_pniels *__restrict__ table, uint32_t count) {
    const uint32_t i = blockIdx.x * blockDim.x + threadIdx.x;
    if (i >= count) return;
    ge_pniels *dst = table + (size_t)i * TT8_MULTS;
    ge_ext cur = bases[i];
    const ge_pniels n1 = ge_to_pniels(cur);
    dst[0] = n1;
#pragma unroll 1
    for (uint32_t k = 1; k < TT8_MULTS; k++) { cur = ge_add_pniels_signed(cur, n1, 0); dst[k] = ge_to_pniels(cur); }
}
__device__ __forceinline__ void tt8_biased_words(uint32_t w[8], const scm &s) {
    sc_to_words(w, s);
    uint64_t carry = 0;
#pragma unroll
    for (int k = 0; k < 8; k++) { uint64_t t = (uint64_t)w[k] + 0x80808080ull + carry; w[k] = (uint32_t)t; carry = t >> 32; }
}
__global__ void __launch_bounds__(256) k_tt_round8(const ge_pniels *__restrict__ table, const scm *__restrict__ a, const scm *__restrict__ b,
                                                   const scm *__restrict__ fG, const scm *__restrict__ fH, const scm *__restrict__ c,
                                                   uint32_t lgM0, uint32_t j, ge_ext *__restrict__ partial , uint32_t quad) {
    __shared__ ge_ext lds[256];
    const uint32_t cls = blockIdx.y, tid = blockIdx.x * blockDim.x + threadIdx.x;
    const uint32_t M0 = 1u << lgM0, e = tid >> 3, g = tid & 7u;
    ge_ext acc = ge_identity();
    if (e < M0) {
        const bool isH = e >= (M0 >> 1);
        const uint32_t e2 = isH ? e - (M0 >> 1) : e;
        const uint32_t lgh = lgM0 - j - 1, h = 1u << lgh;
        const uint32_t t = e2 >> lgh, i = e2 & (h - 1);
        const bool hi = (cls == 0) != isH;
        const uint32_t p = (t << (lgh + 1)) | (hi ? h : 0u) | i;
        const uint32_t sidx = hi ? i : (h | i);
        scm s = isH ? b[sidx] : a[sidx];
        s = sc_mont_mul(s, isH ? fH[p] : fG[p]);
        s = sc_mont_mul(s, c[(isH ? M0 : 0u) + t]);
        uint32_t w[8]; tt8_biased_words(w, s);
        const ge_pniels *tbl = table + ((size_t)(isH ? M0 : 0u) + p) * (TT8_WINDOWS * TT8_MULTS) + (size_t)g * 4 * TT8_MULTS;
        const uint32_t word = w[g];
#pragma unroll 1
        for (uint32_t k = 0; k < 4; k++) {
            const int32_t d = (int32_t)((word >> (8 * k)) & 255u) - 128;
            if (d == 0) continue;
            const uint32_t neg = d < 0, mag = neg ? (uint32_t)(-d) : (uint32_t)d;
            acc = ge_add_pniels_signed(acc, tbl[k * TT8_MULTS + mag - 1], neg);
        }
    }
    ge_block_sum_store(acc, lds, quad, partial + cls * gridDim.x + blockIdx.x);
}
__global__ void __launch_bounds__(256) k_tt_commit3(const ge_pniels *__restrict__ table, const scm *__restrict__ aL, const scm *__restrict__ aR,
                                                    const scm *__restrict__ aO, const scm *__restrict__ sL, const scm *__restrict__ sR,
                                                    uint32_t n, uint32_t M0, ge_ext *__restrict__ partial, uint32_t quad) {
    __shared__ ge_ext lds[256];
    const uint32_t cls = blockIdx.y, tid = blockIdx.x * blockDim.x + threadIdx.x;
    const uint32_t e = tid >> 3, g = tid & 7u;
    ge_ext acc = ge_identity();
    const bool isH = e >= M0;
    const uint32_t p = isH ? e - M0 : e;
    if (e < 2 * M0 && p < n && !(cls == 1 && isH)) {
        const scm s = cls == 0 ? (isH ? aR[p] : aL[p]) : (cls == 1 ? aO[p] : (isH ? sR[p] : sL[p]));
        uint32_t w[8]; tt_biased_words(w, s);
        const ge_pniels *tbl = table + ((size_t)(isH ? M0 : 0u) + p) * (TT_WINDOWS * TT_MULTS) + (size_t)g * 8 * TT_MULTS;
        const uint32_t word = w[g];
#pragma unroll 1
        for (uint32_t k = 0; k < 8; k++) {
            const int32_t d = (int32_t)((word >> (4 * k)) & 15u) - 8;
            if (d == 0) continue;
            const uint32_t neg = d < 0, mag = neg ? (uint32_t)(-d) : (uint32_t)d;
            acc = ge_add_pniels_signed(acc, tbl[k * TT_MULTS + mag - 1], neg);
        }
    }
    ge_block_sum_store(acc, lds, quad, partial + cls * gridDim.x + blockIdx.x);
}
__global__ void __launch_bounds__(256) k_tt_commit3_finish(const ge_ext *__restrict__ partial, uint32_t nblk, const scm *__restrict__ blind,
                                                           const ge_pniels *__restrict__ tableX, ge_ext *__restrict__ out, uint32_t quad) {
    __shared__ ge_ext lds[256];
    const uint32_t cls = blockIdx.x;
    ge_ext acc = ge_identity();
    uint32_t s0 = threadIdx.x;
    if (s0 < nblk) { acc = partial[cls * nblk + s0]; s0 += 256; }
    for (; s0 < nblk; s0 += 256) acc = ge_add(acc, partial[cls * nblk + s0]);
    const uint32_t win = 255u - threadIdx.x;
    if (win < TT_WINDOWS) {
        uint32_t w[8]; tt_biased_words(w, blind[cls]);
        const int32_t d = (int32_t)((w[win >> 3] >> (4 * (win & 7u))) & 15u) - 8;
        if (d != 0) {
            const uint32_t neg = d < 0, mag = neg ? (uint32_t)(-d) : (uint32_t)d;
            const ge_pniels q = tableX[win * TT_MULTS + mag - 1];
            acc = threadIdx.x >= nblk ? ge_from_pniels_signed(q, neg) : ge_add_pniels_signed(acc, q, neg);
        }
    }
    ge_block_sum_store(acc, lds, quad, out + cls);
}
__global__ void __launch_bounds__(256) k_tt_finish(const ge_ext *__restrict__ partial, uint32_t nblk, const scm *__restrict__ a, const scm *__restrict__ b,
                                                   uint32_t h, scm wq, const ge_pniels *__restrict__ tableB, ge_ext *__restrict__ out, uint32_t quad) {
    __shared__ ge_ext lds[256];
    __shared__ scm slds[256];
    const uint32_t cls = blockIdx.x;
    scm ip = sc_zero();
    for (uint32_t i = threadIdx.x; i < h; i += 256) ip = sc_add(ip, cls == 0 ? sc_mont_mul(a[i], b[h + i]) : sc_mont_mul(a[h + i], b[i]));
    const scm cw = sc_mont_mul(block_sum_256(ip, slds), wq);
    ge_ext acc = ge_identity();
    uint32_t s0 = threadIdx.x;
    if (s0 < nblk) { acc = partial[cls * nblk + s0]; s0 += 256; }
    for (; s0 < nblk; s0 += 256) acc = ge_add(acc, partial[cls * nblk + s0]);
    const uint32_t win = 255u - threadIdx.x;
    if (win < TT_WINDOWS) {
        uint32_t w[8]; tt_biased_words(w, cw);
        const int32_t d = (int32_t)((w[win >> 3] >> (4 * (win & 7u))) & 15u) - 8;
        if (d != 0) {
            const uint32_t neg = d < 0, mag = neg ? (uint32_t)(-d) : (uint32_t)d;
            const ge_pniels q = tableB[win * TT_MULTS + mag - 1];
            acc = threadIdx.x >= nblk ? ge_from_pniels_signed(q, neg) : ge_add_pniels_signed(acc, q, neg);
        }
    }
    ge_block_sum_store(acc, lds, quad, out + cls);
}

__device__ __forceinline__ int32_t ped_digit(const uint32_t w[8], uint32_t win) {
    uint32_t carry = 0; int32_t d = 0;
    for (uint32_t j = 0; j <= win; j++) {
        const uint32_t nib = ((w[j >> 3] >> (4 * (j & 7u))) & 15u) + carry;
        carry = nib > 8u; d = (int32_t)nib - (carry ? 16 : 0);
    }
    return d;
}
__global__ void __launch_bounds__(64) k_pedersen(const uint32_t *__restrict__ v, const uint32_t *__restrict__ r,
                                                 const ge_pniels *__restrict__ table , uint8_t *__restrict__ out, uint32_t count) {
    __shared__ ge_ext lds[64];
    const uint32_t i = blockIdx.x, win = threadIdx.x;
    if (i >= count) return;
    uint32_t vw[8], rw[8];
#pragma unroll
    for (int k = 0; k < 8; k++) { vw[k] = v[8 * (size_t)i + k]; rw[k] = r[8 * (size_t)i + k]; }
    ge_ext acc = ge_identity();
    const int32_t dv = ped_digit(vw, win), dr = ped_digit(rw, win);
    if (dv != 0) acc = ge_add_pniels_signed(acc, table[(size_t)win * TT_MULTS + (dv < 0 ? -dv : dv) - 1], dv < 0);
    if (dr != 0) acc = ge_add_pniels_signed(acc, table[(size_t)(TT_WINDOWS + win) * TT_MULTS + (dr < 0 ? -dr : dr) - 1], dr < 0);
    lds[win] = acc; __syncthreads();
    for (uint32_t d = 32; d > 0; d >>= 1) {
        if (win < d) lds[win] = ge_add(lds[win], lds[win + d]);
        __syncthreads();
    }
    if (win == 0) ge_compress(out + 32 * (size_t)i, lds[0]);
}

struct FoldGroup { uint32_t Mr, nterms, first_group, n; int32_t top; };
__global__ void __launch_bounds__(256) k_fold_points(const ge_niels *__restrict__ G, const ge_niels *__restrict__ H,
                                                     ge_ext *__restrict__ out , const uint32_t *__restrict__ naf, const FoldGroup fg) {
    uint32_t t = blockIdx.x * blockDim.x + threadIdx.x;
    const bool live = t < 2 * fg.Mr;
    if (!live) t = 2 * fg.Mr - 1;
    const bool isH = t >= fg.Mr;
    const uint32_t i = isH ? t - fg.Mr : t;
    const ge_niels *tab = isH ? H : G;
    uint32_t bmask = 0;
    if (fg.first_group) for (uint32_t q = 0; q < fg.nterms; q++) if (i + (q + 1) * fg.Mr >= fg.n) bmask |= 1u << q;
    const uint32_t key = (isH ? 0x80000000u : 0u) | bmask;
    const uint32_t key0 = __builtin_amdgcn_readfirstlane(key);
    ge_ext acc = ge_identity();
    if (__ballot(key != key0) == 0ull) {
        const uint32_t hsel = (key0 >> 31) * 2u;
        for (int k = fg.top; k >= 0; k--) {
            acc = ge_dbl(acc);
            for (uint32_t q = 0; q < fg.nterms; q++) {
                const uint32_t *d = naf + ((size_t)(hsel + ((key0 >> q) & 1u)) * fg.nterms + q) * 16;
                if ((d[k >> 5] >> (k & 31)) & 1u) acc = ge_madd_signed(acc, tab[i + (q + 1) * fg.Mr], (d[8 + (k >> 5)] >> (k & 31)) & 1u);
            }
        }
    } else {
        const uint32_t hsel = isH ? 2u : 0u;
        for (int k = fg.top; k >= 0; k--) {
            acc = ge_dbl(acc);
            for (uint32_t q = 0; q < fg.nterms; q++) {
                const uint32_t *d = naf + ((size_t)(hsel + ((bmask >> q) & 1u)) * fg.nterms + q) * 16;
                if ((d[k >> 5] >> (k & 31)) & 1u) acc = ge_madd_signed(acc, tab[i + (q + 1) * fg.Mr], (d[8 + (k >> 5)] >> (k & 31)) & 1u);
            }
        }
    }
    if (live) out[t] = ge_madd(acc, tab[i]);
}

#define BPG_FOLD_VARS(X) X(1) X(2) X(3) X(4) X(5) X(6) X(7) X(8) X(9) X(10) X(11) X(12) X(13) X(14) X(15)
template <int NT>
__global__ void __launch_bounds__(256) __attribute__((amdgpu_waves_per_eu(2, 2))) k_fold_points_reg(
        const ge_niels *__restrict__ G, const ge_niels *__restrict__ H, ge_ext *__restrict__ out , const uint32_t *__restrict__ naf, const FoldGroup fg) {
    uint32_t t = blockIdx.x * blockDim.x + threadIdx.x;
    const bool live = t < 2 * fg.Mr;
    if (!live) t = 2 * fg.Mr - 1;
    const bool isH = t >= fg.Mr;
    const uint32_t i = isH ? t - fg.Mr : t;
    const ge_niels *tab = isH ? H : G;
#define BPG_FOLD_LOAD(j) ge_niels p##j; if (j <= NT) p##j = tab[i + (size_t)j * fg.Mr];
    BPG_FOLD_VARS(BPG_FOLD_LOAD)
#undef BPG_FOLD_LOAD
    uint32_t bmask = 0;
    if (fg.first_group) for (uint32_t q = 0; q < (uint32_t)NT; q++) if (i + (q + 1) * fg.Mr >= fg.n) bmask |= 1u << q;
    const uint32_t key = (isH ? 0x80000000u : 0u) | bmask;
    const uint32_t key0 = __builtin_amdgcn_readfirstlane(key);
    const bool uniform = __ballot(key != key0) == 0ull;
    const uint32_t hsel = isH ? 2u : 0u;
    ge_ext acc = ge_identity();
    for (int k = fg.top; k >= 0; k--) {
        acc = ge_dbl(acc);
#pragma unroll 1
        for (uint32_t q = 0; q < (uint32_t)NT; q++) {
            const uint32_t cls = uniform ? (uint32_t)__builtin_amdgcn_readfirstlane(hsel + ((bmask >> q) & 1u)) : hsel + ((bmask >> q) & 1u);
            const uint32_t *d = naf + ((size_t)cls * NT + q) * 16;
            const uint32_t nz = (d[k >> 5] >> (k & 31)) & 1u, ng = (d[8 + (k >> 5)] >> (k & 31)) & 1u;
            if (uniform ? (__builtin_amdgcn_readfirstlane(nz) != 0) : (nz != 0)) {
                ge_niels Q = p1;
                switch (q) {
#define BPG_FOLD_PICK(j) case j - 1: if (j <= NT) Q = p##j; break;
                    BPG_FOLD_VARS(BPG_FOLD_PICK)
#undef BPG_FOLD_PICK
                    default: break;
                }
                acc = ge_madd_signed(acc, Q, ng);
            }
        }
    }
    if (live) out[t] = ge_madd(acc, tab[i]);
}

struct FoldWnaf { uint32_t Mr, nterms, first_group, n, cap; int32_t top; uint32_t parts, NM; };
__device__ __forceinline__ int32_t fold_wnaf_digit(const uint32_t *__restrict__ dig32, uint32_t cls, uint32_t nterms, uint32_t q, int k) {
    const uint32_t w = dig32[(cls * nterms + q) * 64u + ((uint32_t)k >> 2)];
    return (int32_t)(int8_t)(w >> (8u * ((uint32_t)k & 3u)));
}
__global__ void __launch_bounds__(256) k_fold_points_wnaf(const ge_niels *__restrict__ gens , const ge_niels *__restrict__ odd ,
                                                          ge_ext *__restrict__ out , const uint32_t *__restrict__ dig32, const FoldWnaf fg) {
    uint32_t t = blockIdx.x * blockDim.x + threadIdx.x;
    const bool live = t < 2 * fg.Mr;
    if (!live) t = 2 * fg.Mr - 1;
    const bool isH = t >= fg.Mr;
    const uint32_t i = isH ? t - fg.Mr : t;
    const uint32_t base = (isH ? fg.cap : 0u) + i;
    const size_t tab = (size_t)2 * fg.cap;
    uint32_t bmask = 0;
    if (fg.first_group) for (uint32_t q = 0; q < fg.nterms; q++) if (i + (q + 1) * fg.Mr >= fg.n) bmask |= 1u << q;
    const uint32_t key = (isH ? 0x80000000u : 0u) | bmask;
    const uint32_t key0 = __builtin_amdgcn_readfirstlane(key);
    const uint32_t hsel = isH ? 2u : 0u;
    ge_ext acc = ge_identity();
    const uint32_t nq = fg.nterms * fg.parts;
    if (__ballot(key != key0) == 0ull) {
        const uint32_t hs = (key0 >> 31) * 2u;
        for (int k = fg.top; k >= 0; k--) {
            acc = ge_dbl(acc);
            for (uint32_t part = 0, e = 0; part < fg.parts; part++) {
                for (uint32_t q = 0; q < fg.nterms; q++, e++) {
                    const int32_t d = __builtin_amdgcn_readfirstlane(fold_wnaf_digit(dig32, hs + ((key0 >> q) & 1u), nq, e, k));
                    if (d != 0) {
                        const uint32_t mag = (uint32_t)(d < 0 ? -d : d), idx = part * fg.NM + (mag >> 1);
                        const ge_niels *T = idx ? odd + (size_t)(idx - 1) * tab : gens;
                        const ge_niels Q = T[base + (q + 1) * fg.Mr];
                        if (d < 0) acc = ge_msub(acc, Q); else acc = ge_madd(acc, Q);
                    }
                }
            }
        }
    } else {
        for (int k = fg.top; k >= 0; k--) {
            acc = ge_dbl(acc);
            for (uint32_t part = 0, e = 0; part < fg.parts; part++) {
                for (uint32_t q = 0; q < fg.nterms; q++, e++) {
                    const int32_t d = fold_wnaf_digit(dig32, hsel + ((bmask >> q) & 1u), nq, e, k);
                    if (d != 0) {
                        const uint32_t mag = (uint32_t)(d < 0 ? -d : d), idx = part * fg.NM + (mag >> 1);
                        const ge_niels *T = idx ? odd + (size_t)(idx - 1) * tab : gens;
                        acc = ge_madd_signed(acc, T[base + (q + 1) * fg.Mr], d < 0);
// ... 225 lines not shown
```

bulletproofs_gadgets_amd/csrc/hip/k_scalars.cuh:

```cuda
#pragma once

namespace bpg {

__global__ void __launch_bounds__(256) k_sc_from_bytes(const uint32_t *__restrict__ in, scm *__restrict__ out, uint32_t count) {
    uint32_t i = blockIdx.x * blockDim.x + threadIdx.x;
    if (i >= count) return;
    uint32_t w[8];
    const uint4 *src = reinterpret_cast<const uint4 *>(in + 8 * (size_t)i);
    uint4 a = src[0], b = src[1];
    w[0] = a.x; w[1] = a.y; w[2] = a.z; w[3] = a.w; w[4] = b.x; w[5] = b.y; w[6] = b.z; w[7] = b.w;
    out[i] = sc_from_words(w);
}
#define BLIND_POISON 0xa5c3a5c3u
__global__ void __launch_bounds__(256) k_blind_poison(uint32_t *__restrict__ raw, uint32_t nblocks, uint32_t draws_per_block) {
    const uint32_t t = blockIdx.x * blockDim.x + threadIdx.x;
    if (t >= nblocks * 16u) return;
    raw[(size_t)(t >> 4) * draws_per_block * 16u + (t & 15u)] = BLIND_POISON;
}
__global__ void __launch_bounds__(256) k_sc_from_wide(const uint32_t *__restrict__ in, scm *__restrict__ out, uint32_t count, uint32_t *__restrict__ stale) {
    uint32_t i = blockIdx.x * blockDim.x + threadIdx.x;
    if (i >= count) return;
    uint32_t w[16];
    const uint4 *src = reinterpret_cast<const uint4 *>(in + 16 * (size_t)i);
#pragma unroll
    for (int k = 0; k < 4; k++) { uint4 q = src[k]; w[4 * k] = q.x; w[4 * k + 1] = q.y; w[4 * k + 2] = q.z; w[4 * k + 3] = q.w; }
    uint32_t diff = 0;
#pragma unroll
    for (int k = 0; k < 16; k++) diff |= w[k] ^ BLIND_POISON;
    if (diff == 0) atomicOr(stale, 1u);
    out[i] = sc_from_wide_words(w);
}
__device__ __forceinline__ uint64_t kk_rol(uint64_t x, int n) { return (x << n) | (x >> (64 - n)); }
struct BlindHead { uint64_t lane[10]; };
__global__ void __launch_bounds__(256) k_blind_expand(const BlindHead head, scm *__restrict__ out, uint32_t count) {
    const uint32_t j = blockIdx.x * blockDim.x + threadIdx.x;
    if (j >= count) return;
    uint64_t a[25];
#pragma unroll
    for (int k = 0; k < 25; k++) a[k] = 0;
#pragma unroll
    for (int k = 0; k < 10; k++) a[k] = head.lane[k];
    a[9] |= (uint64_t)(j & 0xffu) << 56;
    a[10] = (uint64_t)(j >> 8) | (0x1fULL << 56);
    a[16] = 0x80ULL << 56;
    const uint64_t RC[24] = {0x0000000000000001ULL, 0x0000000000008082ULL, 0x800000000000808aULL, 0x8000000080008000ULL, 0x000000000000808bULL,
        0x0000000080000001ULL, 0x8000000080008081ULL, 0x8000000000008009ULL, 0x000000000000008aULL, 0x0000000000000088ULL, 0x0000000080008009ULL,
        0x000000008000000aULL, 0x000000008000808bULL, 0x800000000000008bULL, 0x8000000000008089ULL, 0x8000000000008003ULL, 0x8000000000008002ULL,
        0x8000000000000080ULL, 0x000000000000800aULL, 0x800000008000000aULL, 0x8000000080008081ULL, 0x8000000000008080ULL, 0x0000000080000001ULL,
        0x8000000080008008ULL};
#pragma unroll 1
    for (int r = 0; r < 24; r++) {
        uint64_t c0 = a[0] ^ a[5] ^ a[10] ^ a[15] ^ a[20], c1 = a[1] ^ a[6] ^ a[11] ^ a[16] ^ a[21], c2 = a[2] ^ a[7] ^ a[12] ^ a[17] ^ a[22],
                 c3 = a[3] ^ a[8] ^ a[13] ^ a[18] ^ a[23], c4 = a[4] ^ a[9] ^ a[14] ^ a[19] ^ a[24];
        const uint64_t d0 = c4 ^ kk_rol(c1, 1), d1 = c0 ^ kk_rol(c2, 1), d2 = c1 ^ kk_rol(c3, 1), d3 = c2 ^ kk_rol(c4, 1), d4 = c3 ^ kk_rol(c0, 1);
        const uint64_t b00 = a[0] ^ d0, b01 = kk_rol(a[6] ^ d1, 44), b02 = kk_rol(a[12] ^ d2, 43), b03 = kk_rol(a[18] ^ d3, 21), b04 = kk_rol(a[24] ^ d4, 14);
        const uint64_t b05 = kk_rol(a[3] ^ d3, 28), b06 = kk_rol(a[9] ^ d4, 20), b07 = kk_rol(a[10] ^ d0, 3), b08 = kk_rol(a[16] ^ d1, 45), b09 = kk_rol(a[22] ^ d2, 61);
        const uint64_t b10 = kk_rol(a[1] ^ d1, 1), b11 = kk_rol(a[7] ^ d2, 6), b12 = kk_rol(a[13] ^ d3, 25), b13 = kk_rol(a[19] ^ d4, 8), b14 = kk_rol(a[20] ^ d0, 18);
        const uint64_t b15 = kk_rol(a[4] ^ d4, 27), b16 = kk_rol(a[5] ^ d0, 36), b17 = kk_rol(a[11] ^ d1, 10), b18 = kk_rol(a[17] ^ d2, 15), b19 = kk_rol(a[23] ^ d3, 56);
        const uint64_t b20 = kk_rol(a[2] ^ d2, 62), b21 = kk_rol(a[8] ^ d3, 55), b22 = kk_rol(a[14] ^ d4, 39), b23 = kk_rol(a[15] ^ d0, 41), b24 = kk_rol(a[21] ^ d1, 2);
        a[0] = b00 ^ (~b01 & b02) ^ RC[r]; a[1] = b01 ^ (~b02 & b03); a[2] = b02 ^ (~b03 & b04); a[3] = b03 ^ (~b04 & b00); a[4] = b04 ^ (~b00 & b01);
        a[5] = b05 ^ (~b06 & b07); a[6] = b06 ^ (~b07 & b08); a[7] = b07 ^ (~b08 & b09); a[8] = b08 ^ (~b09 & b05); a[9] = b09 ^ (~b05 & b06);
        a[10] = b10 ^ (~b11 & b12); a[11] = b11 ^ (~b12 & b13); a[12] = b12 ^ (~b13 & b14); a[13] = b13 ^ (~b14 & b10); a[14] = b14 ^ (~b10 & b11);
        a[15] = b15 ^ (~b16 & b17); a[16] = b16 ^ (~b17 & b18); a[17] = b17 ^ (~b18 & b19); a[18] = b18 ^ (~b19 & b15); a[19] = b19 ^ (~b15 & b16);
        a[20] = b20 ^ (~b21 & b22); a[21] = b21 ^ (~b22 & b23); a[22] = b22 ^ (~b23 & b24); a[23] = b23 ^ (~b24 & b20); a[24] = b24 ^ (~b20 & b21);
    }
    uint32_t w[16];
#pragma unroll
    for (int k = 0; k < 8; k++) { w[2 * k] = (uint32_t)a[k]; w[2 * k + 1] = (uint32_t)(a[k] >> 32); }
    out[j] = sc_from_wide_words(w);
}
struct ExpTables { scm base[3]; scm *out[3]; uint32_t count[3], lgT[3]; };
__global__ void __launch_bounds__(256) k_exp_table(ExpTables E) {
    const uint32_t k = blockIdx.y;
    const uint32_t t = blockIdx.x * blockDim.x + threadIdx.x, lgT = E.lgT[k], T = 1u << lgT, count = E.count[k];
    if (t >= T) return;
    scm *__restrict__ out = E.out[k];
    scm cur = SC_R1(), sq = E.base[k];
    for (uint32_t b = 0; b < lgT; b++) {
        if ((t >> b) & 1u) cur = sc_mont_mul(cur, sq);
        sq = sc_mont_mul(sq, sq);
    }
    for (uint32_t i = t; i < count; i += T) { out[i] = cur; cur = sc_mont_mul(cur, sq); }
}

__device__ __forceinline__ scm block_sum_256(scm v, scm *lds) {
    lds[threadIdx.x] = v;
    __syncthreads();
    for (uint32_t s = 128; s > 0; s >>= 1) {
        if (threadIdx.x < s) lds[threadIdx.x] = sc_add(lds[threadIdx.x], lds[threadIdx.x + s]);
        __syncthreads();
    }
    scm r = lds[0];
    __syncthreads();
    return r;
}

__global__ void __launch_bounds__(256) k_reduce_partials(const scm *__restrict__ partial, uint32_t parts, uint32_t stride, scm *__restrict__ out) {
    __shared__ scm lds[256];
    uint32_t k = blockIdx.x;
    scm acc = sc_zero();
    for (uint32_t p = threadIdx.x; p < parts; p += 256) acc = sc_add(acc, partial[(size_t)p * stride + k]);
    scm r = block_sum_256(acc, lds);
    if (threadIdx.x == 0) out[k] = r;
}
__global__ void __launch_bounds__(256) k_reduce_partials_scaled(const scm *__restrict__ partial, uint32_t parts, uint32_t stride, scm *__restrict__ out, scm w) {
    __shared__ scm lds[256];
    uint32_t k = blockIdx.x;
    scm acc = sc_zero();
    for (uint32_t p = threadIdx.x; p < parts; p += 256) acc = sc_add(acc, partial[(size_t)p * stride + k]);
    scm r = block_sum_256(acc, lds);
    if (threadIdx.x == 0) out[k] = sc_mont_mul(r, w);
}

__device__ __forceinline__ uint32_t csc_col(uint32_t pv, uint32_t n, uint32_t m) {
    const uint32_t kind = pv >> 29, idx = pv & 0x1fffffffu;
    return kind <= 2 ? kind * n + idx : (kind == 3 ? 3 * n + idx : 3 * n + m);
}
__global__ void __launch_bounds__(256) k_csc_count(const uint64_t *__restrict__ row_ptr, const uint32_t *__restrict__ term_var, uint32_t q, uint32_t n, uint32_t m,
                                                   uint32_t *__restrict__ counts , uint32_t *__restrict__ rowconst ) {
    const uint32_t r = blockIdx.x * blockDim.x + threadIdx.x;
    if (r >= q) return;
    uint32_t rc = 0;
    for (uint64_t k = row_ptr[r]; k < row_ptr[r + 1]; k++) {
        const uint32_t col = csc_col(term_var[k], n, m);
        if (col == 3 * n + m) rc++; else atomicAdd(&counts[col], 1u);
    }
    rowconst[r] = rc;
}
__global__ void __launch_bounds__(256) k_csc_fill(const uint64_t *__restrict__ row_ptr, const uint32_t *__restrict__ term_var, const uint32_t *__restrict__ term_coef,
                                                  uint32_t q, uint32_t n, uint32_t m, uint32_t *__restrict__ cursor, const uint32_t *__restrict__ rowconst_start,
                                                  const uint32_t *__restrict__ var_total , uint32_t *__restrict__ ent_row, uint32_t *__restrict__ ent_coef) {
    const uint32_t r = blockIdx.x * blockDim.x + threadIdx.x;
    if (r >= q) return;
    uint32_t cpos = *var_total + rowconst_start[r];
    for (uint64_t k = row_ptr[r]; k < row_ptr[r + 1]; k++) {
        const uint32_t col = csc_col(term_var[k], n, m);
        const uint32_t pos = col == 3 * n + m ? cpos++ : atomicAdd(&cursor[col], 1u);
        ent_row[pos] = r; ent_coef[pos] = term_coef[k];
    }
}
__global__ void __launch_bounds__(256) k_csc_colptr(const uint32_t *__restrict__ starts , const uint32_t *__restrict__ rowconst_start ,
                                                    uint32_t nvar, uint32_t q, uint64_t *__restrict__ col_ptr, uint32_t *__restrict__ totals ) {
    const uint32_t c = blockIdx.x * blockDim.x + threadIdx.x;
    if (c <= nvar) col_ptr[c] = starts[c];
    if (c == 0) { const uint32_t all = starts[nvar] + rowconst_start[q]; col_ptr[nvar + 1] = all; totals[0] = starts[nvar]; totals[1] = all; }
}

__global__ void __launch_bounds__(256) k_flatten(const uint64_t *__restrict__ col_ptr, const uint32_t *__restrict__ ent_row,
                                                 const uint32_t *__restrict__ ent_coef, const scm *__restrict__ coef,
                                                 const scm *__restrict__ zpow , scm *__restrict__ w,
                                                 uint32_t ncols, uint32_t first_neg_col) {
    uint32_t c = blockIdx.x * blockDim.x + threadIdx.x;
    if (c >= ncols) return;
    scm acc = sc_zero();
    for (uint64_t e = col_ptr[c]; e < col_ptr[c + 1]; e++) acc = sc_add(acc, sc_mont_mul(coef[ent_coef[e]], zpow[ent_row[e] + 1]));
    w[c] = (c >= first_neg_col) ? sc_neg(acc) : acc;
}

__global__ void __launch_bounds__(256) k_flatten_const(const uint32_t *__restrict__ ent_row, const uint32_t *__restrict__ ent_coef,
                                                       const scm *__restrict__ coef, const scm *__restrict__ zpow, uint64_t e0, uint64_t e1,
                                                       scm *__restrict__ partial) {
    __shared__ scm lds[256];
    scm acc = sc_zero();
    for (uint64_t e = e0 + blockIdx.x * blockDim.x + threadIdx.x; e < e1; e += (uint64_t)gridDim.x * blockDim.x)
        acc = sc_add(acc, sc_mont_mul(coef[ent_coef[e]], zpow[ent_row[e] + 1]));
    scm r = block_sum_256(acc, lds);
    if (threadIdx.x == 0) partial[blockIdx.x] = sc_neg(r);
}

__global__ void __launch_bounds__(256) k_poly_t(const scm *__restrict__ aL, const scm *__restrict__ aR, const scm *__restrict__ aO,
                                                const scm *__restrict__ sL, const scm *__restrict__ sR,
                                                const scm *__restrict__ wL, const scm *__restrict__ wR, const scm *__restrict__ wO,
                                                const scm *__restrict__ ypow, const scm *__restrict__ yinvpow,
                                                scm *__restrict__ partial , uint32_t n) {
    __shared__ scm lds[256];
    scm t1 = sc_zero(), t2 = t1, t3 = t1, t4 = t1, t5 = t1, t6 = t1;
    for (uint32_t i = blockIdx.x * blockDim.x + threadIdx.x; i < n; i += gridDim.x * blockDim.x) {
        scm y = ypow[i];
        scm l1 = sc_add(aL[i], sc_mont_mul(yinvpow[i], wR[i]));
        scm l2 = aO[i], l3 = sL[i];
        scm r0 = sc_sub(wO[i], y);
        scm r1 = sc_add(sc_mont_mul(y, aR[i]), wL[i]);
        scm r3 = sc_mont_mul(y, sR[i]);
        t1 = sc_add(t1, sc_mont_mul(l1, r0));
        t2 = sc_add(t2, sc_add(sc_mont_mul(l1, r1), sc_mont_mul(l2, r0)));
        t3 = sc_add(t3, sc_add(sc_mont_mul(l2, r1), sc_mont_mul(l3, r0)));
        t4 = sc_add(t4, sc_add(sc_mont_mul(l1, r3), sc_mont_mul(l3, r1)));
        t5 = sc_add(t5, sc_mont_mul(l2, r3));
        t6 = sc_add(t6, sc_mont_mul(l3, r3));
    }
    scm r;
    r = block_sum_256(t1, lds); if (threadIdx.x == 0) partial[blockIdx.x * 6 + 0] = r;
    r = block_sum_256(t2, lds); if (threadIdx.x == 0) partial[blockIdx.x * 6 + 1] = r;
    r = block_sum_256(t3, lds); if (threadIdx.x == 0) partial[blockIdx.x * 6 + 2] = r;
    r = block_sum_256(t4, lds); if (threadIdx.x == 0) partial[blockIdx.x * 6 + 3] = r;
    r = block_sum_256(t5, lds); if (threadIdx.x == 0) partial[blockIdx.x * 6 + 4] = r;
    r = block_sum_256(t6, lds); if (threadIdx.x == 0) partial[blockIdx.x * 6 + 5] = r;
}

__global__ void __launch_bounds__(256) k_poly_eval(const scm *__restrict__ aL, const scm *__restrict__ aR, const scm *__restrict__ aO,
                                                   const scm *__restrict__ sL, const scm *__restrict__ sR,
                                                   const scm *__restrict__ wL, const scm *__restrict__ wR, const scm *__restrict__ wO,
                                                   const scm *__restrict__ ypow, const scm *__restrict__ yinvpow, scm x,
                                                   scm *__restrict__ lv, scm *__restrict__ rv, uint32_t n, uint32_t N) {
    uint32_t i = blockIdx.x * blockDim.x + threadIdx.x;
    if (i >= N) return;
    scm y = ypow[i];
    if (i >= n) { lv[i] = sc_zero(); rv[i] = sc_neg(y); return; }
    scm l1 = sc_add(aL[i], sc_mont_mul(yinvpow[i], wR[i]));
    scm r0 = sc_sub(wO[i], y);
    scm r1 = sc_add(sc_mont_mul(y, aR[i]), wL[i]);
    scm r3 = sc_mont_mul(y, sR[i]);
    scm l = sc_mont_mul(x, sc_add(l1, sc_mont_mul(x, sc_add(aO[i], sc_mont_mul(x, sL[i])))));
    scm r = sc_add(r0, sc_mont_mul(x, sc_add(r1, sc_mont_mul(x, sc_mont_mul(x, r3)))));
    lv[i] = l; rv[i] = r;
}

}
```

Measured before the change: 101.4 million.

## Fuse IPA scalar fold and partial reduction into round kernels via last-block tickets

Removes the separate k_tt_advance, k_tt_finish, k_set2 and k_reduce_partials_scaled launches in the inner-product argument. The previous round's challenge fold of a/b and the coefficient vectors is now applied lazily inside the next round's prep/table-round kernel, writing to ping-pong buffers. Cross-block reduction is done by the last block to arrive, using atomic tickets and agent-scope publish stores. This cuts several small launches per IPA round, at the cost of redundant fold arithmetic, atomics and extra ticket state that must stay zeroed.

Measured after the change: 102.7 million (median of 6 runs). 1.01x the previous value.

```diff
diff --git a/bulletproofs_gadgets_amd/csrc/engine.hip b/bulletproofs_gadgets_amd/csrc/engine.hip
--- a/bulletproofs_gadgets_amd/csrc/engine.hip
+++ b/bulletproofs_gadgets_amd/csrc/engine.hip
@@ -182,7 +182,7 @@
     X(k_sc_from_wide) X(k_blind_poison) X(k_exp_table) X(k_reduce_partials) X(k_flatten) X(k_flatten_const) X(k_poly_t) X(k_poly_eval) X(k_ipa_prep) \
     X(k_ipa_fold_scalars) X(k_fold_points) X(k_fold_points_reg) X(k_fold_points_split) X(k_fold_points_wnaf) X(k_fold_points_quad) X(k_fold_points_quadw) X(k_fold_points_regw) X(k_odd_start) X(k_odd_start_ext) X(k_dbl_times) X(k_odd_step) X(k_msm_digits) X(k_msm_scatter1) X(k_msm_sort2) X(k_scan_blocksums) \
     X(k_scan_apply) X(k_bucket_chunks) X(k_bucket_combine) X(k_bucket_combine_heavy) X(k_bucket_reduce) X(k_window_sums) X(k_window_sums_quad) X(k_decompress) X(k_ipa_s) X(k_verify_scalars) X(k_verify_scalars_acc) X(k_bench_fe_mul) \
-    X(k_tt_bases) X(k_tt_multiples) X(k_tt_bases8) X(k_tt_multiples8) X(k_tt_round8) X(k_tt_factors) X(k_tt_advance) X(k_tt_round) X(k_tt_finish) X(k_blind_expand) X(k_tt_commit3) X(k_tt_commit3_finish) X(k_csc_count) X(k_csc_fill) X(k_csc_colptr) X(k_merge_insert) X(k_merge_plan) X(k_merge_groups) X(k_merge_members) X(k_merge_sum) \
+    X(k_tt_bases) X(k_tt_multiples) X(k_tt_bases8) X(k_tt_multiples8) X(k_tt_round8) X(k_tt_factors) X(k_tt_round) X(k_blind_expand) X(k_tt_commit3) X(k_tt_commit3_finish) X(k_csc_count) X(k_csc_fill) X(k_csc_colptr) X(k_merge_insert) X(k_merge_plan) X(k_merge_groups) X(k_merge_members) X(k_merge_sum) \
     X(k_bt_commit3) X(k_bt_commit3_finish) X(k_bt_compress) X(k_bt_exp) X(k_bt_poly_t) X(k_bt_poly_eval) X(k_bt_factors) X(k_bt_advance) X(k_bt_round) \
     X(k_bt_finish) X(k_bt_fold_scalars) X(k_witness_eval)
 enum KernelId {
@@ -260,8 +260,17 @@
     DevBuf stale_flag;
     DevBuf ipa_s, ipa_tabA, ipa_tabB, naf, qsteps, vfy_in, vfy_pts, vfy_ok, vfy_sc, vfy_ch;
     DevBuf vfy_small;
-    DevBuf tt_bases, tt_table, tt_f, tt_c, tt_partial, grp_c, ped_table, s_parts;
+    DevBuf tt_bases, tt_table, tt_f, tt_c, tt_partial, grp_c, ped_table, s_parts, ipa_ab;
     uint32_t tt_orig_M0 = 0; const void *tt_orig_gens = nullptr;
+    static constexpr size_t TT_TICKET_BYTES = 256;
+    enum { TICKET_TT = 0 , TICKET_PREP = 2  };
+    void tt_partial_ensure(size_t bytes) {
+        if (tt_partial.p && bytes + TT_TICKET_BYTES <= tt_partial.cap) return;
+        tt_partial.ensure(bytes + TT_TICKET_BYTES);
+        HIPCHK(hipMemsetAsync(tt_partial.p, 0, TT_TICKET_BYTES, st));
+    }
+    uint32_t *tt_tickets() const { return tt_partial.as<uint32_t>(); }
+    ge_ext *tt_partial_pts() const { return reinterpret_cast<ge_ext *>(tt_partial.as<uint8_t>() + TT_TICKET_BYTES); }
     ge_pniels *tt_table_p = nullptr;
     void tt_build(const ge_niels *G, const ge_niels *H, const ge_niels *B, uint32_t M0, bool original) {
         const uint32_t npts = 2 * M0 + 1;
@@ -276,7 +285,7 @@
             arena.ensure(bb + tb);
             basesp = reinterpret_cast<ge_ext *>(arena_at(0)); tt_table_p = reinterpret_cast<ge_pniels *>(arena_at(bb));
         }
-        tt_partial.ensure((size_t)3 * cdiv((uint64_t)M0 * 16, 256) * sizeof(ge_ext));
+        tt_partial_ensure((size_t)3 * cdiv((uint64_t)M0 * 16, 256) * sizeof(ge_ext));
         BPG_LAUNCH((*this), k_tt_bases, dim3(cdiv(npts, 64)), dim3(256), G, H, B, basesp, M0);
         BPG_LAUNCH((*this), k_tt_multiples, dim3(cdiv((uint64_t)npts * TT_WINDOWS, 256)), dim3(256), basesp, tt_table_p, npts * TT_WINDOWS);
         if (original) { tt_orig_M0 = M0; tt_orig_gens = gens.p; }
@@ -588,7 +597,7 @@
                       &impl_->starts, &impl_->cursor, &impl_->blocksum, &impl_->arena, &impl_->buckets, &impl_->partial, &impl_->msm_result,
                       &impl_->sLR, &impl_->yinvpow, &impl_->lv, &impl_->rv, &impl_->red_partial,
                       &impl_->red_out, &impl_->raw_rng, &impl_->extras, &impl_->ipa_s, &impl_->ipa_tabA, &impl_->ipa_tabB, &impl_->naf, &impl_->qsteps, &impl_->wsums, &impl_->wq_stage, &impl_->wq_tickets, &impl_->vfy_in, &impl_->vfy_pts, &impl_->vfy_ok, &impl_->vfy_sc, &impl_->vfy_ch, &impl_->vfy_small,
-                      &impl_->stale_flag, &impl_->tile_hist, &impl_->heavy, &impl_->plain, &impl_->open_keys, &impl_->medium, &impl_->tt_bases, &impl_->tt_table, &impl_->tt_f, &impl_->tt_c, &impl_->tt_partial, &impl_->grp_c, &impl_->ped_table, &impl_->s_parts, &impl_->starts1};
+                      &impl_->stale_flag, &impl_->tile_hist, &impl_->heavy, &impl_->plain, &impl_->open_keys, &impl_->medium, &impl_->tt_bases, &impl_->tt_table, &impl_->tt_f, &impl_->tt_c, &impl_->tt_partial, &impl_->ipa_ab, &impl_->grp_c, &impl_->ped_table, &impl_->s_parts, &impl_->starts1};
     for (DevBuf *b : bufs) b->release();
     impl_->shared.reset();
     impl_->h_raw.release(); impl_->h_small.release(); impl_->h_naf.release(); impl_->h_qsteps.release(); impl_->stage.release(); for (PinBuf &b : impl_->h_blind) b.release();
@@ -1304,7 +1313,14 @@
     const scm w_m = to_scm(w), uch_m = to_scm(u_ch);
     uint64_t mcur = N;
     const uint32_t quad_sums = I.shared_now ? 0u : 1u;
-    bool tt_on = false; uint32_t tt_j = 0, tt_lgM0 = 0, tt_cur = 0; Scalar tt_u, tt_uinv; const ge_pniels *tt_wide = nullptr;
+    bool tt_on = false; uint32_t tt_j = 0, tt_lgM0 = 0, tt_cur = 0; const ge_pniels *tt_wide = nullptr;
+    IpaPend pend; pend.u = pend.uinv = pend.c0G = pend.c0H = to_scm(Scalar::one()); pend.fold = 0;
+    bool ab_alt = false;
+    auto ab_flip = [&](uint64_t m) {
+        ab_alt = !ab_alt;
+        if (ab_alt) { I.ipa_ab.ensure(2 * m * sizeof(scm)); a = I.ipa_ab.as<scm>(); b = a + m; }
+        else { a = I.lv.as<scm>(); b = I.rv.as<scm>(); }
+    };
     const uint32_t GRP_STRIDE = 64;
     uint32_t g_j = 0, g_r = 1, g_cur = 0, g_index = 0; uint64_t g_M = N; bool g_first = true; std::vector<Scalar> g_us;
     for (uint32_t round = 0; round < lgN; round++) {
@@ -1321,18 +1337,18 @@
         }
         if (tt_on) {
             const uint32_t M0 = 1u << tt_lgM0;
-            scm *c0 = I.tt_c.as<scm>() + (size_t)tt_cur * 2 * M0, *c1 = I.tt_c.as<scm>() + (size_t)(tt_cur ^ 1u) * 2 * M0;
-            if (tt_j > 0) {
-                BPG_LAUNCH(I, k_tt_advance, dim3(cdiv(std::max<uint64_t>(mcur, 1ull << (tt_j - 1)), 256)), dim3(256), a, b, to_scm(tt_u), to_scm(tt_uinv), (uint32_t)mcur,
-                           c0, c1, 1u << (tt_j - 1), M0);
-                tt_cur ^= 1u; std::swap(c0, c1);
-            }
+            const scm *c_in = I.tt_c.as<scm>() + (size_t)tt_cur * 2 * M0; scm *c_out = I.tt_c.as<scm>() + (size_t)(tt_cur ^ 1u) * 2 * M0;
+            if (tt_j > 0) { if (!pend.fold) throw std::logic_error("inner_product: tail round without its challenge"); tt_cur ^= 1u; }
+            const scm *a_in = a, *b_in = b;
+            if (pend.fold) { ab_flip(mcur); }
             const uint32_t nblk = cdiv((uint64_t)M0 * 8, 256);
-            if (tt_wide) BPG_LAUNCH(I, k_tt_round8, dim3(nblk, 2), dim3(256), tt_wide, a, b, I.tt_f.as<scm>(), I.tt_f.as<scm>() + M0, c0, tt_lgM0, tt_j, I.tt_partial.as<ge_ext>(), quad_sums);
-            else BPG_LAUNCH(I, k_tt_round, dim3(nblk, 2), dim3(256), I.tt_table_p, a, b, I.tt_f.as<scm>(), I.tt_f.as<scm>() + M0, c0, tt_lgM0, tt_j,
-                       I.tt_partial.as<ge_ext>(), quad_sums);
-            BPG_LAUNCH(I, k_tt_finish, dim3(2), dim3(256), I.tt_partial.as<ge_ext>(), nblk, a, b, (uint32_t)h, w_m,
-                       I.tt_table_p + (size_t)2 * M0 * TT_WINDOWS * TT_MULTS, I.msm_result.as<ge_ext>(), quad_sums);
+            TtRoundArgs A;
+            A.a_in = a_in; A.b_in = b_in; A.a_out = a; A.b_out = b; A.fG = I.tt_f.as<scm>(); A.fH = I.tt_f.as<scm>() + M0; A.c_in = c_in; A.c_out = c_out;
+            A.partial = I.tt_partial_pts(); A.ticket = I.tt_tickets() + Impl::TICKET_TT; A.tableB = I.tt_table_p + (size_t)2 * M0 * TT_WINDOWS * TT_MULTS;
+            A.out = I.msm_result.as<ge_ext>(); A.lgM0 = tt_lgM0; A.j = tt_j; A.quad = quad_sums;
+            if (tt_wide) BPG_LAUNCH(I, k_tt_round8, dim3(nblk, 2), dim3(256), tt_wide, A, pend, w_m);
+            else BPG_LAUNCH(I, k_tt_round, dim3(nblk, 2), dim3(256), I.tt_table_p, A, pend, w_m);
+            pend.fold = 0;
             HIPCHK(hipGetLastError());
             uint8_t lr[64];
             uint32_t *hp = reinterpret_cast<uint32_t *>(I.h_small.as<uint8_t>() + 16384);
@@ -1342,13 +1358,9 @@
             lap(tm ? &tm->ipa_msm : nullptr);
             T.append_point("L", lr); T.append_point("R", lr + 32);
             proof.insert(proof.end(), lr, lr + 64);
-            tt_u = T.challenge_scalar("u"); tt_uinv = tt_u.invert();
+            { const Scalar u = T.challenge_scalar("u"); pend.u = to_scm(u); pend.uinv = to_scm(u.invert()); pend.fold = 1; }
             tt_j++;
             mcur = h;
-            if (round + 1 == lgN) {
-                BPG_LAUNCH(I, k_ipa_fold_scalars, dim3(cdiv(h, 256)), dim3(256), a, b, to_scm(tt_u), to_scm(tt_uinv), (uint32_t)h);
-                HIPCHK(hipGetLastError());
-            }
             continue;
         }
         if (g_j == 0) {
@@ -1359,17 +1371,21 @@
             g_us.clear();
             I.grp_c.ensure(4 * GRP_STRIDE * sizeof(scm));
             g_cur = 0;
-            hipLaunchKernelGGL(k_set2, dim3(1), dim3(64), 0, st, I.grp_c.as<scm>(), (uint32_t)GRP_STRIDE, to_scm(Gamma), to_scm(Eta));
-        }
-        scm *c0 = I.grp_c.as<scm>() + (size_t)g_cur * 2 * GRP_STRIDE;
+            pend.c0G = to_scm(Gamma); pend.c0H = to_scm(Eta);
+        }
+        if (g_j > 0) { if (!pend.fold) throw std::logic_error("inner_product: sub-round without its challenge"); g_cur ^= 1u; }
+        const scm *c_in = I.grp_c.as<scm>() + (size_t)(g_cur ^ 1u) * 2 * GRP_STRIDE; scm *c_out = I.grp_c.as<scm>() + (size_t)g_cur * 2 * GRP_STRIDE;
+        const scm *a_in = a, *b_in = b;
+        if (pend.fold) ab_flip(mcur);
         const uint64_t cnt = g_M / 2;
         scm *sLG = I.ipa_s.as<scm>(), *sLH = sLG + cnt, *sRG = sLH + cnt, *sRH = sRG + cnt;
         const uint32_t blocks = std::min<uint32_t>(cdiv(cnt, 256), 1024);
         const uint32_t lgh = ceil_log2(h);
         I.red_partial.ensure((size_t)blocks * 2 * sizeof(scm) + 4096);
-        BPG_LAUNCH(I, k_ipa_prep, dim3(blocks), dim3(256), a, b, I.yinvpow.as<scm>(), c0, c0 + GRP_STRIDE, uch_m,
-                           (uint32_t)g_first, (uint32_t)n, lgh, g_j, sLG, sLH, sRG, sRH, I.red_partial.as<scm>());
-        BPG_LAUNCH_ID(I, KID_k_reduce_partials, k_reduce_partials_scaled, dim3(2), dim3(256), I.red_partial.as<scm>(), blocks, 2u, I.extras.as<scm>() + 3, w_m);
+        I.tt_partial_ensure(0);
+        BPG_LAUNCH(I, k_ipa_prep, dim3(blocks), dim3(256), a_in, b_in, a, b, pend, I.yinvpow.as<scm>(), c_in, c_out, (uint32_t)GRP_STRIDE, uch_m,
+                           (uint32_t)g_first, (uint32_t)n, lgh, g_j, sLG, sLH, sRG, sRH, I.red_partial.as<scm>(), I.tt_tickets() + Impl::TICKET_PREP, w_m, I.extras.as<scm>() + 3);
+        pend.fold = 0;
         Impl::MsmTicket tk;
         {
             MsmSegs S = seg_new();
@@ -1390,12 +1406,7 @@
         proof.insert(proof.end(), lr, lr + 64);
         const Scalar u = T.challenge_scalar("u"), uinv = u.invert();
         g_us.push_back(u);
-        {
-            scm *c1 = I.grp_c.as<scm>() + (size_t)(g_cur ^ 1u) * 2 * GRP_STRIDE;
-            BPG_LAUNCH(I, k_tt_advance, dim3(cdiv(std::max<uint64_t>(h, 1ull << g_j), 256)), dim3(256), a, b, to_scm(u), to_scm(uinv), (uint32_t)h,
-                       c0, c1, 1u << g_j, (uint32_t)GRP_STRIDE);
-            g_cur ^= 1u;
-        }
+        pend.u = to_scm(u); pend.uinv = to_scm(uinv); pend.fold = 1;
         g_j++;
         if (g_j == g_r) {
             const uint32_t Mr = (uint32_t)(g_M >> g_r), nterms = (1u << g_r) - 1u;
@@ -1533,6 +1544,10 @@
         mcur = h;
         lap(tm ? &tm->ipa_fold : nullptr);
     }
+    if (pend.fold) {
+        BPG_LAUNCH(I, k_ipa_fold_scalars, dim3(1), dim3(256), a, b, pend.u, pend.uinv, 1u);
+        HIPCHK(hipGetLastError());
+    }
     scm ab[2];
     HIPCHK(hipMemcpyAsync(&ab[0], a, sizeof(scm), hipMemcpyDeviceToHost, st));
     HIPCHK(hipMemcpyAsync(&ab[1], b, sizeof(scm), hipMemcpyDeviceToHost, st));
@@ -1792,8 +1807,8 @@
     if (tabled) {
         const uint32_t M0 = (uint32_t)N, nblk = cdiv((uint64_t)M0 * 16, 256);
         BPG_LAUNCH(I, k_tt_commit3, dim3(nblk, 3), dim3(256), I.tt_table_p, c->aL.as<scm>(), c->aR.as<scm>(), c->aO.as<scm>(), sL, sR,
-                   (uint32_t)n, M0, I.tt_partial.as<ge_ext>(), I.shared_now ? 0u : 1u);
-        BPG_LAUNCH(I, k_tt_commit3_finish, dim3(3), dim3(256), I.tt_partial.as<ge_ext>(), nblk, I.extras.as<scm>(),
+                   (uint32_t)n, M0, I.tt_partial_pts(), I.shared_now ? 0u : 1u);
+        BPG_LAUNCH(I, k_tt_commit3_finish, dim3(3), dim3(256), I.tt_partial_pts(), nblk, I.extras.as<scm>(),
                    I.ped_table.as<ge_pniels>() + (size_t)TT_WINDOWS * TT_MULTS, I.msm_result.as<ge_ext>(), I.shared_now ? 0u : 1u);
         HIPCHK(hipGetLastError());
         uint32_t *hp = reinterpret_cast<uint32_t *>(I.h_small.as<uint8_t>() + 16384);
diff --git a/bulletproofs_gadgets_amd/csrc/hip/k_ipa.cuh b/bulletproofs_gadgets_amd/csrc/hip/k_ipa.cuh
--- a/bulletproofs_gadgets_amd/csrc/hip/k_ipa.cuh
+++ b/bulletproofs_gadgets_amd/csrc/hip/k_ipa.cuh
@@ -2,19 +2,55 @@
 
 namespace bpg {
 
-__global__ void __launch_bounds__(256) k_ipa_prep(const scm *__restrict__ a, const scm *__restrict__ b, const scm *__restrict__ yinvpow,
-                                                  const scm *__restrict__ cG, const scm *__restrict__ cH, scm u_ch, uint32_t first_group, uint32_t n,
-                                                  uint32_t lgh, uint32_t j,
+struct IpaPend { scm u, uinv, c0G, c0H; uint32_t fold; };
+__device__ __forceinline__ scm ipa_fold_a(const scm *a, uint32_t i, uint32_t m, const IpaPend &P) { return sc_add(sc_mont_mul(a[i], P.u), sc_mont_mul(P.uinv, a[m + i])); }
+__device__ __forceinline__ scm ipa_fold_b(const scm *b, uint32_t i, uint32_t m, const IpaPend &P) { return sc_add(sc_mont_mul(b[i], P.uinv), sc_mont_mul(P.u, b[m + i])); }
+template <class T> __device__ __forceinline__ void publish_store(T *dst, const T &v) {
+    static_assert(sizeof(T) % 8 == 0, "64-bit granules");
+    const uint64_t *w = reinterpret_cast<const uint64_t *>(&v);
+#pragma unroll
+    for (uint32_t k = 0; k < sizeof(T) / 8; k++) __hip_atomic_store(reinterpret_cast<uint64_t *>(dst) + k, w[k], __ATOMIC_RELAXED, __HIP_MEMORY_SCOPE_AGENT);
+}
+template <class T> __device__ __forceinline__ T publish_load(const T *src) {
+    T v; uint64_t *w = reinterpret_cast<uint64_t *>(&v);
+#pragma unroll
+    for (uint32_t k = 0; k < sizeof(T) / 8; k++) w[k] = __hip_atomic_load(reinterpret_cast<const uint64_t *>(src) + k, __ATOMIC_RELAXED, __HIP_MEMORY_SCOPE_AGENT);
+    return v;
+}
+__device__ __forceinline__ bool block_is_last(uint32_t *ticket, uint32_t n, uint32_t *flag) {
+    asm volatile("s_waitcnt vmcnt(0)" ::: "memory");
+    __syncthreads();
+    if (threadIdx.x == 0) {
+        const uint32_t prev = __hip_atomic_fetch_add(ticket, 1u, __ATOMIC_RELAXED, __HIP_MEMORY_SCOPE_AGENT);
+        if (prev + 1 == n) __hip_atomic_store(ticket, 0u, __ATOMIC_RELAXED, __HIP_MEMORY_SCOPE_AGENT);
+        *flag = prev + 1 == n ? 1u : 0u;
+    }
+    __syncthreads();
+    const bool last = *reinterpret_cast<volatile uint32_t *>(flag) != 0;
+    __syncthreads();
+    return last;
+}
+__global__ void __launch_bounds__(256) k_ipa_prep(const scm *a_in, const scm *b_in, scm *a_out, scm *b_out, IpaPend P,
+                                                  const scm *__restrict__ yinvpow, const scm *c_in, scm *c_out, uint32_t cstride,
+                                                  scm u_ch, uint32_t first_group, uint32_t n, uint32_t lgh, uint32_t j,
                                                   scm *__restrict__ sLG, scm *__restrict__ sLH, scm *__restrict__ sRG, scm *__restrict__ sRH,
-                                                  scm *__restrict__ partial ) {
+                                                  scm *partial , uint32_t *ticket, scm w, scm *out ) {
     __shared__ scm lds[256];
+    __shared__ uint32_t flag;
     scm cL = sc_zero(), cR = sc_zero();
     const uint32_t h = 1u << lgh, count = h << j;
     for (uint32_t e = blockIdx.x * blockDim.x + threadIdx.x; e < count; e += gridDim.x * blockDim.x) {
         const uint32_t t = e >> lgh, i = e & (h - 1);
         const uint32_t plo = (t << (lgh + 1)) | i, phi = plo | h;
-        const scm alo = a[i], ahi = a[h + i], blo = b[i], bhi = b[h + i];
-        const scm g = cG[t], eh = cH[t];
+        scm alo, ahi, blo, bhi;
+        if (P.fold) {
+            alo = ipa_fold_a(a_in, i, 2 * h, P); ahi = ipa_fold_a(a_in, h + i, 2 * h, P); blo = ipa_fold_b(b_in, i, 2 * h, P); bhi = ipa_fold_b(b_in, h + i, 2 * h, P);
+            if (t == 0) { a_out[i] = alo; a_out[h + i] = ahi; b_out[i] = blo; b_out[h + i] = bhi; }
+        } else { alo = a_in[i]; ahi = a_in[h + i]; blo = b_in[i]; bhi = b_in[h + i]; }
+        scm g, eh;
+        if (j == 0) { g = P.c0G; eh = P.c0H; }
+        else { g = sc_mont_mul(c_in[t >> 1], (t & 1u) ? P.u : P.uinv); eh = sc_mont_mul(c_in[cstride + (t >> 1)], (t & 1u) ? P.uinv : P.u); }
+        if (i == 0) { c_out[t] = g; c_out[cstride + t] = eh; }
         const bool padlo = first_group && plo >= n, padhi = first_group && phi >= n;
         scm v;
         v = sc_mont_mul(alo, g); if (padhi) v = sc_mont_mul(v, u_ch); sLG[e] = v;
@@ -24,10 +60,14 @@
         if (t == 0) { cL = sc_add(cL, sc_mont_mul(alo, bhi)); cR = sc_add(cR, sc_mont_mul(ahi, blo)); }
     }
     scm r;
-    r = block_sum_256(cL, lds); if (threadIdx.x == 0) partial[blockIdx.x * 2 + 0] = r;
-    r = block_sum_256(cR, lds); if (threadIdx.x == 0) partial[blockIdx.x * 2 + 1] = r;
-}
-__global__ void k_set2(scm *__restrict__ c, uint32_t stride, scm v0, scm v1) { if (threadIdx.x == 0 && blockIdx.x == 0) { c[0] = v0; c[stride] = v1; } }
+    r = block_sum_256(cL, lds); if (threadIdx.x == 0) publish_store(partial + blockIdx.x * 2 + 0, r);
+    r = block_sum_256(cR, lds); if (threadIdx.x == 0) publish_store(partial + blockIdx.x * 2 + 1, r);
+    if (!block_is_last(ticket, gridDim.x, &flag)) return;
+    cL = sc_zero(); cR = sc_zero();
+    for (uint32_t p = threadIdx.x; p < gridDim.x; p += 256) { cL = sc_add(cL, publish_load(partial + p * 2 + 0)); cR = sc_add(cR, publish_load(partial + p * 2 + 1)); }
+    r = block_sum_256(cL, lds); if (threadIdx.x == 0) out[0] = sc_mont_mul(r, w);
+    r = block_sum_256(cR, lds); if (threadIdx.x == 0) out[1] = sc_mont_mul(r, w);
+}
 
 __global__ void __launch_bounds__(256) k_ipa_fold_scalars(scm *__restrict__ a, scm *__restrict__ b, scm u, scm uinv, uint32_t h) {
     uint32_t i = blockIdx.x * blockDim.x + threadIdx.x;
@@ -111,43 +151,88 @@
     fG[p] = pad ? u_ch : SC_R1();
     fH[p] = pad ? sc_mont_mul(yinvpow[p], u_ch) : yinvpow[p];
 }
-__global__ void __launch_bounds__(256) k_tt_advance(scm *__restrict__ a, scm *__restrict__ b, scm u, scm uinv, uint32_t h,
-                                                    const scm *__restrict__ cprev, scm *__restrict__ cnext, uint32_t cnt, uint32_t M0) {
-    const uint32_t i = blockIdx.x * blockDim.x + threadIdx.x;
-    if (i < h) {
-        a[i] = sc_add(sc_mont_mul(a[i], u), sc_mont_mul(uinv, a[h + i]));
-        b[i] = sc_add(sc_mont_mul(b[i], uinv), sc_mont_mul(u, b[h + i]));
-    }
-    if (i < cnt) {
-        const scm g = cprev[i], e = cprev[M0 + i];
-        cnext[2 * i] = sc_mont_mul(g, uinv); cnext[2 * i + 1] = sc_mont_mul(g, u);
-        cnext[M0 + 2 * i] = sc_mont_mul(e, u); cnext[M0 + 2 * i + 1] = sc_mont_mul(e, uinv);
-    }
-}
 __device__ __forceinline__ void tt_biased_words(uint32_t w[8], const scm &s) {
     sc_to_words(w, s);
     uint64_t carry = 0;
 #pragma unroll
     for (int k = 0; k < 8; k++) { uint64_t t = (uint64_t)w[k] + 0x88888888ull + carry; w[k] = (uint32_t)t; carry = t >> 32; }
 }
-__global__ void __launch_bounds__(256) k_tt_round(const ge_pniels *__restrict__ table, const scm *__restrict__ a, const scm *__restrict__ b,
-                                                  const scm *__restrict__ fG, const scm *__restrict__ fH, const scm *__restrict__ c,
-                                                  uint32_t lgM0, uint32_t j, ge_ext *__restrict__ partial , uint32_t quad) {
+struct TtRoundArgs {
+    const scm *a_in, *b_in; scm *a_out, *b_out; const scm *fG, *fH, *c_in; scm *c_out;
+    ge_ext *partial ; uint32_t *ticket ; const ge_pniels *tableB; ge_ext *out ;
+    uint32_t lgM0, j, quad;
+};
+__device__ __forceinline__ scm tt_a(const TtRoundArgs &A, const IpaPend &P, uint32_t i, uint32_t m) { return P.fold ? ipa_fold_a(A.a_in, i, m, P) : A.a_in[i]; }
+__device__ __forceinline__ scm tt_b(const TtRoundArgs &A, const IpaPend &P, uint32_t i, uint32_t m) { return P.fold ? ipa_fold_b(A.b_in, i, m, P) : A.b_in[i]; }
+__device__ __forceinline__ scm tt_round_scalar(const TtRoundArgs &A, const IpaPend &P, uint32_t cls, uint32_t tid, uint32_t e, bool &isH, uint32_t &p) {
+    const uint32_t M0 = 1u << A.lgM0, lgh = A.lgM0 - A.j - 1, h = 1u << lgh;
+    if (cls == 0) {
+        if (P.fold && tid < 2 * h) { A.a_out[tid] = tt_a(A, P, tid, 2 * h); A.b_out[tid] = tt_b(A, P, tid, 2 * h); }
+        if (A.j > 0 && tid < (1u << A.j)) {
+            A.c_out[tid] = sc_mont_mul(A.c_in[tid >> 1], (tid & 1u) ? P.u : P.uinv);
+            A.c_out[M0 + tid] = sc_mont_mul(A.c_in[M0 + (tid >> 1)], (tid & 1u) ? P.uinv : P.u);
+        }
+    }
+    isH = e >= (M0 >> 1);
+    const uint32_t e2 = isH ? e - (M0 >> 1) : e;
+    const uint32_t t = e2 >> lgh, i = e2 & (h - 1);
+    const bool hi = (cls == 0) != isH;
+    p = (t << (lgh + 1)) | (hi ? h : 0u) | i;
+    const uint32_t sidx = hi ? i : (h | i);
+    scm s = isH ? tt_b(A, P, sidx, 2 * h) : tt_a(A, P, sidx, 2 * h);
+    s = sc_mont_mul(s, isH ? A.fH[p] : A.fG[p]);
+    scm c;
+    if (A.j == 0) c = A.c_in[isH ? M0 : 0u];
+    else c = sc_mont_mul(A.c_in[(isH ? M0 : 0u) + (t >> 1)], ((t & 1u) != 0) != isH ? P.u : P.uinv);
+    return sc_mont_mul(s, c);
+}
+__device__ __forceinline__ void tt_round_finish(const TtRoundArgs &A, const IpaPend &P, scm wq, const ge_ext &acc_in, ge_ext *lds) {
+    const uint32_t cls = blockIdx.y, nblk = gridDim.x;
+    ge_ext *mine = A.partial + cls * nblk + blockIdx.x;
+    if (A.quad) {
+        const fe sum = ge_block_sum_quad(acc_in, lds);
+        if (threadIdx.x < 4) publish_store(reinterpret_cast<fe *>(mine) + threadIdx.x, sum);
+    } else {
+        lds[threadIdx.x] = acc_in; __syncthreads();
+        for (uint32_t d = 128; d > 0; d >>= 1) {
+            if (threadIdx.x < d) lds[threadIdx.x] = ge_add(lds[threadIdx.x], lds[threadIdx.x + d]);
+            __syncthreads();
+        }
+        if (threadIdx.x == 0) publish_store(mine, lds[0]);
+    }
+    __syncthreads();
+    if (!block_is_last(A.ticket + cls, nblk, reinterpret_cast<uint32_t *>(lds))) return;
+    const uint32_t h = 1u << (A.lgM0 - A.j - 1);
+    scm *slds = reinterpret_cast<scm *>(lds);
+    scm ip = sc_zero();
+    for (uint32_t i = threadIdx.x; i < h; i += 256)
+        ip = sc_add(ip, cls == 0 ? sc_mont_mul(tt_a(A, P, i, 2 * h), tt_b(A, P, h + i, 2 * h)) : sc_mont_mul(tt_a(A, P, h + i, 2 * h), tt_b(A, P, i, 2 * h)));
+    const scm cw = sc_mont_mul(block_sum_256(ip, slds), wq);
+    __syncthreads();
+    ge_ext acc = ge_identity();
+    uint32_t s0 = threadIdx.x;
+    if (s0 < nblk) { acc = publish_load(A.partial + cls * nblk + s0); s0 += 256; }
+    for (; s0 < nblk; s0 += 256) acc = ge_add(acc, publish_load(A.partial + cls * nblk + s0));
+    const uint32_t win = 255u - threadIdx.x;
+    if (win < TT_WINDOWS) {
+        uint32_t w[8]; tt_biased_words(w, cw);
+        const int32_t d = (int32_t)((w[win >> 3] >> (4 * (win & 7u))) & 15u) - 8;
+        if (d != 0) {
+            const uint32_t neg = d < 0, mag = neg ? (uint32_t)(-d) : (uint32_t)d;
+            const ge_pniels q = A.tableB[win * TT_MULTS + mag - 1];
+            acc = threadIdx.x >= nblk ? ge_from_pniels_signed(q, neg) : ge_add_pniels_signed(acc, q, neg);
+        }
+    }
+    ge_block_sum_store(acc, lds, A.quad, A.out + cls);
+}
+__global__ void __launch_bounds__(256) k_tt_round(const ge_pniels *__restrict__ table, TtRoundArgs A, IpaPend P, scm wq) {
     __shared__ ge_ext lds[256];
     const uint32_t cls = blockIdx.y, tid = blockIdx.x * blockDim.x + threadIdx.x;
-    const uint32_t M0 = 1u << lgM0, e = tid >> 3, g = tid & 7u;
+    const uint32_t M0 = 1u << A.lgM0, e = tid >> 3, g = tid & 7u;
     ge_ext acc = ge_identity();
     if (e < M0) {
-        const bool isH = e >= (M0 >> 1);
-        const uint32_t e2 = isH ? e - (M0 >> 1) : e;
-        const uint32_t lgh = lgM0 - j - 1, h = 1u << lgh;
-        const uint32_t t = e2 >> lgh, i = e2 & (h - 1);
-        const bool hi = (cls == 0) != isH;
-        const uint32_t p = (t << (lgh + 1)) | (hi ? h : 0u) | i;
-        const uint32_t sidx = hi ? i : (h | i);
-        scm s = isH ? b[sidx] : a[sidx];
-        s = sc_mont_mul(s, isH ? fH[p] : fG[p]);
-        s = sc_mont_mul(s, c[(isH ? M0 : 0u) + t]);
+        bool isH; uint32_t p;
+        const scm s = tt_round_scalar(A, P, cls, tid, e, isH, p);
         uint32_t w[8]; tt_biased_words(w, s);
         const ge_pniels *tbl = table + ((size_t)(isH ? M0 : 0u) + p) * (TT_WINDOWS * TT_MULTS) + (size_t)g * 8 * TT_MULTS;
         const uint32_t word = w[g];
@@ -159,7 +244,7 @@
             acc = ge_add_pniels_signed(acc, tbl[k * TT_MULTS + mag - 1], neg);
         }
     }
-    ge_block_sum_store(acc, lds, quad, partial + cls * gridDim.x + blockIdx.x);
+    tt_round_finish(A, P, wq, acc, lds);
 }
 #define TT8_WINDOWS 32
 #define TT8_MULTS 128
@@ -198,24 +283,14 @@
 #pragma unroll
     for (int k = 0; k < 8; k++) { uint64_t t = (uint64_t)w[k] + 0x80808080ull + carry; w[k] = (uint32_t)t; carry = t >> 32; }
 }
-__global__ void __launch_bounds__(256) k_tt_round8(const ge_pniels *__restrict__ table, const scm *__restrict__ a, const scm *__restrict__ b,
-                                                   const scm *__restrict__ fG, const scm *__restrict__ fH, const scm *__restrict__ c,
-                                                   uint32_t lgM0, uint32_t j, ge_ext *__restrict__ partial , uint32_t quad) {
+__global__ void __launch_bounds__(256) k_tt_round8(const ge_pniels *__restrict__ table, TtRoundArgs A, IpaPend P, scm wq) {
     __shared__ ge_ext lds[256];
     const uint32_t cls = blockIdx.y, tid = blockIdx.x * blockDim.x + threadIdx.x;
-    const uint32_t M0 = 1u << lgM0, e = tid >> 3, g = tid & 7u;
+    const uint32_t M0 = 1u << A.lgM0, e = tid >> 3, g = tid & 7u;
     ge_ext acc = ge_identity();
     if (e < M0) {
-        const bool isH = e >= (M0 >> 1);
-        const uint32_t e2 = isH ? e - (M0 >> 1) : e;
-        const uint32_t lgh = lgM0 - j - 1, h = 1u << lgh;
-        const uint32_t t = e2 >> lgh, i = e2 & (h - 1);
-        const bool hi = (cls == 0) != isH;
-        const uint32_t p = (t << (lgh + 1)) | (hi ? h : 0u) | i;
-        const uint32_t sidx = hi ? i : (h | i);
-        scm s = isH ? b[sidx] : a[sidx];
-        s = sc_mont_mul(s, isH ? fH[p] : fG[p]);
-        s = sc_mont_mul(s, c[(isH ? M0 : 0u) + t]);
+        bool isH; uint32_t p;
+        const scm s = tt_round_scalar(A, P, cls, tid, e, isH, p);
         uint32_t w[8]; tt8_biased_words(w, s);
         const ge_pniels *tbl = table + ((size_t)(isH ? M0 : 0u) + p) * (TT8_WINDOWS * TT8_MULTS) + (size_t)g * 4 * TT8_MULTS;
         const uint32_t word = w[g];
@@ -227,7 +302,7 @@
             acc = ge_add_pniels_signed(acc, tbl[k * TT8_MULTS + mag - 1], neg);
         }
     }
-    ge_block_sum_store(acc, lds, quad, partial + cls * gridDim.x + blockIdx.x);
+    tt_round_finish(A, P, wq, acc, lds);
 }
 __global__ void __launch_bounds__(256) k_tt_commit3(const ge_pniels *__restrict__ table, const scm *__restrict__ aL, const scm *__restrict__ aR,
                                                     const scm *__restrict__ aO, const scm *__restrict__ sL, const scm *__restrict__ sR,
@@ -273,31 +348,6 @@
     }
     ge_block_sum_store(acc, lds, quad, out + cls);
 }
-__global__ void __launch_bounds__(256) k_tt_finish(const ge_ext *__restrict__ partial, uint32_t nblk, const scm *__restrict__ a, const scm *__restrict__ b,
-                                                   uint32_t h, scm wq, const ge_pniels *__restrict__ tableB, ge_ext *__restrict__ out, uint32_t quad) {
-    __shared__ ge_ext lds[256];
-    __shared__ scm slds[256];
-    const uint32_t cls = blockIdx.x;
-    scm ip = sc_zero();
-    for (uint32_t i = threadIdx.x; i < h; i += 256) ip = sc_add(ip, cls == 0 ? sc_mont_mul(a[i], b[h + i]) : sc_mont_mul(a[h + i], b[i]));
-    const scm cw = sc_mont_mul(block_sum_256(ip, slds), wq);
-    ge_ext acc = ge_identity();
-    uint32_t s0 = threadIdx.x;
-    if (s0 < nblk) { acc = partial[cls * nblk + s0]; s0 += 256; }
-    for (; s0 < nblk; s0 += 256) acc = ge_add(acc, partial[cls * nblk + s0]);
-    const uint32_t win = 255u - threadIdx.x;
-    if (win < TT_WINDOWS) {
-        uint32_t w[8]; tt_biased_words(w, cw);
-        const int32_t d = (int32_t)((w[win >> 3] >> (4 * (win & 7u))) & 15u) - 8;
-        if (d != 0) {
-            const uint32_t neg = d < 0, mag = neg ? (uint32_t)(-d) : (uint32_t)d;
-            const ge_pniels q = tableB[win * TT_MULTS + mag - 1];
-            acc = threadIdx.x >= nblk ? ge_from_pniels_signed(q, neg) : ge_add_pniels_signed(acc, q, neg);
-        }
-    }
-    ge_block_sum_store(acc, lds, quad, out + cls);
-}
-
 __device__ __forceinline__ int32_t ped_digit(const uint32_t w[8], uint32_t win) {
     uint32_t carry = 0; int32_t d = 0;
     for (uint32_t j = 0; j <= win; j++) {
diff --git a/bulletproofs_gadgets_amd/csrc/hip/k_scalars.cuh b/bulletproofs_gadgets_amd/csrc/hip/k_scalars.cuh
--- a/bulletproofs_gadgets_amd/csrc/hip/k_scalars.cuh
+++ b/bulletproofs_gadgets_amd/csrc/hip/k_scalars.cuh
@@ -103,14 +103,6 @@
     scm r = block_sum_256(acc, lds);
     if (threadIdx.x == 0) out[k] = r;
 }
-__global__ void __launch_bounds__(256) k_reduce_partials_scaled(const scm *__restrict__ partial, uint32_t parts, uint32_t stride, scm *__restrict__ out, scm w) {
-    __shared__ scm lds[256];
-    uint32_t k = blockIdx.x;
-    scm acc = sc_zero();
-    for (uint32_t p = threadIdx.x; p < parts; p += 256) acc = sc_add(acc, partial[(size_t)p * stride + k]);
-    scm r = block_sum_256(acc, lds);
-    if (threadIdx.x == 0) out[k] = sc_mont_mul(r, w);
-}
 
 __device__ __forceinline__ uint32_t csc_col(uint32_t pv, uint32_t n, uint32_t m) {
     const uint32_t kind = pv >> 29, idx = pv & 0x1fffffffu;
```
